# amolchanov86/gym_art

Hardware: AMD Instinct MI355X
Metric: env-steps/sec (whole node) at N=2^20 Hummingbird; achieved HBM GB/s (higher is better)
Workload: dtype f64

## Files before the change

### gym_art_amd/csrc/gaq.hip

```cpp
#include "gaq_host.hpp"

#define GAQ_X(FEAT) extern template __global__ GAQ_STEP_SIG(FEAT)
GAQ_STEP_ALL(GAQ_X)
#undef GAQ_X
#define GAQ_X(FEAT) extern template __global__ GAQ_ROLL_SIG(FEAT)
GAQ_ROLL_ALL(GAQ_X)
#undef GAQ_X

namespace {

using namespace gaqk;

__global__ __launch_bounds__(kBlock) void episode_kernel(int64_t n, const float* __restrict__ reward,
                                                          const uint8_t* __restrict__ done, float* __restrict__ ep_ret,
                                                          uint32_t* __restrict__ ep_len, double* __restrict__ acc) {
  const int64_t i = (int64_t)blockIdx.x * kBlock + threadIdx.x;
  float ret = 0.0f; uint32_t len = 0; bool fin = false;
  if (i < n) {
    ret = ep_ret[i] + reward[i];
    len = ep_len[i] + 1u;
    fin = done[i] != 0;
    ep_ret[i] = fin ? 0.0f : ret;
    ep_len[i] = fin ? 0u : len;
  }
  double c = fin ? 1.0 : 0.0, sr = fin ? (double)ret : 0.0, sl = fin ? (double)len : 0.0, sq = fin ? (double)ret * ret : 0.0;
  if (__ballot(fin)) {
#pragma unroll
    for (int o = 32; o > 0; o >>= 1) { c += __shfl_down(c, o); sr += __shfl_down(sr, o); sl += __shfl_down(sl, o); sq += __shfl_down(sq, o); }
    if ((threadIdx.x & 63) == 0) { atomicAdd(acc + 0, c); atomicAdd(acc + 1, sr); atomicAdd(acc + 2, sl); atomicAdd(acc + 3, sq); }
  }
}

__global__ __launch_bounds__(kBlock) void pack_rows_kernel(int64_t n, int D, const float* __restrict__ obs,
                                                            const float* __restrict__ reward, const uint8_t* __restrict__ done,
                                                            float* __restrict__ rows) {
  const int W = D + 2;
  const int64_t total = n * W;
  for (int64_t k = (int64_t)blockIdx.x * kBlock + threadIdx.x; k < total; k += (int64_t)gridDim.x * kBlock) {
    const int64_t i = k / W;
    const int c = (int)(k - i * W);
    rows[k] = c < D ? obs[i * D + c] : c == D ? reward[i] : (float)done[i];
  }
}

__global__ __launch_bounds__(kBlock) void clear_dynamics_kernel(DevPtrs p, const int64_t* __restrict__ idx, int64_t first, int64_t count) {
  const int64_t k = (int64_t)blockIdx.x * kBlock + threadIdx.x;
  if (k >= count) return;
  const int64_t i = idx ? idx[k] : first + k;
  p.ctr[i] &= 0xFFFFu;
  float* ou = p.ou + (i / kTile) * (4 * kTile) + (i % kTile);
#pragma unroll
  for (int j = 0; j < 4; ++j) ou[j * kTile] = 0.0f;
}

__global__ __launch_bounds__(kBlock) void checksum_kernel(const uint32_t* __restrict__ w, int64_t n, uint64_t* __restrict__ out) {
  uint64_t acc = 0;
  for (int64_t i = (int64_t)blockIdx.x * kBlock + threadIdx.x; i < n; i += (int64_t)gridDim.x * kBlock) {
    uint64_t x = ((uint64_t)w[i] << 32) ^ (uint64_t)i * 0x9E3779B97F4A7C15ull;
    x ^= x >> 29; x *= 0xBF58476D1CE4E5B9ull; x ^= x >> 32;
    acc += x;
  }
#pragma unroll
  for (int o = 32; o > 0; o >>= 1) acc += __shfl_down(acc, o);
  if ((threadIdx.x & 63) == 0) atomicAdd(reinterpret_cast<unsigned long long*>(out), (unsigned long long)acc);
}

__device__ __forceinline__ uint32_t* pfull_of(const DevPtrs& p) { return p.traj + 3 * p.ntiles * kTile; }

__device__ __forceinline__ void write_model_planes(const DevPtrs& p, double dt, int64_t i, const gaq::DerivedModel& dm, bool staged = false) {
  double* tp = staged ? p.par_next + i * (int64_t)kPar
                      : const_cast<double*>(p.par) + (i / kTile) * (int64_t)(kPar * kTile) + (i % kTile);
  const int stride = staged ? 1 : kTile;
  auto P = [&](int plane) -> double& { return tp[plane * stride]; };
  P(PP_MASS) = dm.mass; P(PP_INV_MASS) = 1.0 / dm.mass;
#pragma unroll
  for (int j = 0; j < 3; ++j) { P(PP_INERTIA + j) = dm.inertia[j]; P(PP_INV_INERTIA + j) = 1.0 / dm.inertia[j]; }
#pragma unroll
  for (int j = 0; j < 4; ++j) {
    P(PP_THRUST_MAX + j) = dm.thrust_max[j]; P(PP_TORQUE_MAX + j) = dm.torque_max[j];
    P(PP_PROP_X + j) = dm.prop_pos[3 * j]; P(PP_PROP_Y + j) = dm.prop_pos[3 * j + 1]; P(PP_PROP_Z + j) = dm.prop_pos[3 * j + 2];
  }
  P(PP_TAU_UP) = 4 * dt / (dm.damp_time_up + 1e-6); P(PP_TAU_DOWN) = 4 * dt / (dm.damp_time_down + 1e-6);
  P(PP_T_UP) = dm.damp_time_up; P(PP_T_DOWN) = dm.damp_time_down;
  P(PP_LINEARITY) = dm.linearity; P(PP_ARM) = dm.arm; P(PP_VEL_DAMP) = dm.vel_damp; P(PP_DAMP_Q) = dm.damp_omega_quadratic;
  P(PP_C_DRAG) = dm.c_drag; P(PP_C_ROLL) = dm.c_roll;
  if (staged) P(PP_OU_SIGMA) = (double)(float)dm.ou_sigma;
  else reinterpret_cast<float*>(tp - (i % kTile) + PP_OU_SIGMA * kTile)[i % kTile] = (float)dm.ou_sigma;
  P(PP_T2T) = dm.t2t; P(PP_MX) = dm.motor_x; P(PP_MY) = dm.motor_y; P(PP_COMX) = dm.com[0]; P(PP_COMY) = dm.com[1];
  P(PP_COMPACT_OK) = 1.0;
  if (staged) return;
  pfull_of(p)[i] = p.rcount[i];
  p.ctr[i] &= 0xFFFFu;
  float* ou = p.ou + (i / kTile) * (4 * kTile) + (i % kTile);
#pragma unroll
  for (int j = 0; j < 4; ++j) ou[j * kTile] = 0.0f;
}

__global__ __launch_bounds__(kBlock) void rerandomize_kernel(DevPtrs p, StepCfg cfg, Randomizer rz, const uint8_t* __restrict__ sel,
                                                              int mode, double* __restrict__ trees_out, int64_t first, int64_t count) {
  const int64_t k = (int64_t)blockIdx.x * kBlock + threadIdx.x;
  if (mode == 3) {
    if (k >= count) return;
    const int64_t i = first + k;
    const uint32_t rc = p.rcount[i];
    double* row = trees_out + k * (int64_t)kPar;
    if (rc == pfull_of(p)[i]) { row[PP_COMPACT_OK] = -1.0; return; }
    gaq::ParamTree t;
    if (rz.sampler == 2) gaq::random_quad_tree(cfg.seed, cfg.env_offset + (uint64_t)i, rc - 1, t);
    else gaq::perturb_tree(rz.base, rz.ratio, rz.sampler, cfg.seed, cfg.env_offset + (uint64_t)i, rc - 1, t);
    gaq::DerivedModel dm;
    gaq::derive_tree(t, dm, rz.sampler == 2);
    DevPtrs q = p;
    q.par_next = trees_out - first * (int64_t)kPar;
    write_model_planes(q, cfg.dt, i, dm, true);
    return;
  }
  if (trees_out) {
    if (k >= count) return;
    const int64_t i = first + k;
    gaq::ParamTree t;
    const uint32_t rc = p.rcount[i];
    if (rc == 0) { t = rz.base; }
    else if (rz.sampler == 2) { gaq::random_quad_tree(cfg.seed, cfg.env_offset + (uint64_t)i, rc - 1, t); }
    else { gaq::perturb_tree(rz.base, rz.ratio, rz.sampler, cfg.seed, cfg.env_offset + (uint64_t)i, rc - 1, t); }
    for (int j = 0; j < gaq::TL_COUNT; ++j) trees_out[k * gaq::TL_COUNT + j] = t.v[j];
    return;
  }
  if (mode == 0) {
    const int64_t i = k;
    if (i >= p.n) return;
    const uint32_t promoted = p.rz_flag[i];
    if (!promoted) return;
    if (promoted > 1u) atomicAdd(p.rz_overrun, promoted - 1u);
    gaq::ParamTree t;
    const uint32_t rc = p.rcount[i];
    if (rz.sampler == 2) gaq::random_quad_tree(cfg.seed, cfg.env_offset + (uint64_t)i, rc, t);
    else gaq::perturb_tree(rz.base, rz.ratio, rz.sampler, cfg.seed, cfg.env_offset + (uint64_t)i, rc, t);
    gaq::DerivedModel dm;
    gaq::derive_tree(t, dm, rz.sampler == 2);
    write_model_planes(p, cfg.dt, i, dm, true);
    p.rz_flag[i] = 0;
    return;
  }
  const int64_t i = k;
  if (i >= p.n) return;
  if (mode == 2 || mode == 4) {
    const uint32_t rc = p.rcount[i];
    if (mode == 4 && rc == pfull_of(p)[i]) return;
    gaq::ParamTree t;
    if (rc == 0) { t = rz.base; if (rz.sampler == 2) { pfull_of(p)[i] = 0u; return; } }
    else if (rz.sampler == 2) gaq::random_quad_tree(cfg.seed, cfg.env_offset + (uint64_t)i, rc - 1, t);
    else gaq::perturb_tree(rz.base, rz.ratio, rz.sampler, cfg.seed, cfg.env_offset + (uint64_t)i, rc - 1, t);
    gaq::DerivedModel dm;
    gaq::derive_tree(t, dm, rz.sampler == 2);
    const uint32_t keep = p.ctr[i];
    float ou[4];
    float* op = p.ou + (i / kTile) * (4 * kTile) + (i % kTile);
    for (int j = 0; j < 4; ++j) ou[j] = op[j * kTile];
    write_model_planes(p, cfg.dt, i, dm);
    p.ctr[i] = keep;
    for (int j = 0; j < 4; ++j) op[j * kTile] = ou[j];
    if (p.rz_every > 0) p.rz_flag[i] = 1u;
    return;
  }
  if (!(sel == nullptr || sel[i] != 0)) return;
  const uint32_t rc = p.rcount[i];
  p.rcount[i] = rc + 1u;
  gaq::ParamTree t;
  if (rz.sampler == 2) gaq::random_quad_tree(cfg.seed, cfg.env_offset + (uint64_t)i, rc, t);
  else gaq::perturb_tree(rz.base, rz.ratio, rz.sampler, cfg.seed, cfg.env_offset + (uint64_t)i, rc, t);
  gaq::DerivedModel dm;
  gaq::derive_tree(t, dm, rz.sampler == 2);
  write_model_planes(p, cfg.dt, i, dm);
  if (p.rz_every > 0) p.rz_flag[i] = 1u;
}

__global__ __launch_bounds__(kBlock) void jinv_kernel(DevPtrs p, StepCfg cfg, Model<double> um, const uint8_t* __restrict__ done) {
  const int64_t i = (int64_t)blockIdx.x * kBlock + threadIdx.x;
  if (i >= p.n || !p.jinv) return;
  if (done && !done[i]) return;
  Model<double> m;
  load_model<gaq::F_PER_ENV>(p, cfg, i / kTile, (uint32_t)(i % kTile), um, m);
  double J[4][8];
  const double ccw[4] = {-1, 1, -1, 1};
  for (int c = 0; c < 4; ++c) {
    J[0][c] = m.thrust_max[c] * m.inv_mass;
    J[1][c] = m.inv_inertia[0] * (m.thrust_max[c] * m.prop_y[c]);
    J[2][c] = m.inv_inertia[1] * (m.thrust_max[c] * -m.prop_x[c]);
    J[3][c] = m.inv_inertia[2] * (m.torque_max[c] * ccw[c]);
    for (int r = 0; r < 4; ++r) J[r][4 + c] = (r == c) ? 1.0 : 0.0;
  }
  for (int col = 0; col < 4; ++col) {
    int piv = col;
    for (int r = col + 1; r < 4; ++r) if (fabs(J[r][col]) > fabs(J[piv][col])) piv = r;
    for (int c = 0; c < 8; ++c) { const double t = J[col][c]; J[col][c] = J[piv][c]; J[piv][c] = t; }
    const double inv = 1.0 / J[col][col];
    for (int c = 0; c < 8; ++c) J[col][c] *= inv;
    for (int r = 0; r < 4; ++r) if (r != col) {
      const double f = J[r][col];
      for (int c = 0; c < 8; ++c) J[r][c] -= f * J[col][c];
    }
  }
  double* out = const_cast<double*>(p.jinv) + i * 16;
  for (int r = 0; r < 4; ++r) for (int c = 0; c < 4; ++c) out[4 * r + c] = J[r][4 + c];
}

__global__ __launch_bounds__(kBlock) void derive_trees_kernel(DevPtrs p, StepCfg cfg, const double* __restrict__ trees, int by_density,
                                                               int64_t first, int64_t count) {
  const int64_t k = (int64_t)blockIdx.x * kBlock + threadIdx.x;
  if (k >= count) return;
  gaq::ParamTree t;
  for (int j = 0; j < gaq::TL_COUNT; ++j) t.v[j] = trees[k * gaq::TL_COUNT + j];
  gaq::DerivedModel dm;
  gaq::derive_tree(t, dm, by_density != 0);
  write_model_planes(p, cfg.dt, first + k, dm);
}

__global__ __launch_bounds__(kBlock) void hbm_copy_kernel(const u32x4* __restrict__ src, u32x4* __restrict__ dst, size_t n16) {
  size_t i = (size_t)blockIdx.x * kBlock + threadIdx.x;
  const size_t stride = (size_t)gridDim.x * kBlock;
  for (; i < n16; i += stride) dst[i] = src[i];
}

__global__ void bump_kernel(uint64_t* ctr, uint64_t inc) { *ctr += inc; }
__global__ void fold_counter_kernel(uint64_t* ctr) {
  uint64_t sum = 0;
  for (int k = 0; k < kCtrSlots; ++k) { sum += ctr[k * kCtrStride]; ctr[k * kCtrStride] = 0; }
  ctr[0] = sum;
}

struct TileDirect {
  const DevPtrs& p; int64_t tile; uint32_t lane;
  __device__ __forceinline__ double ld64(const double* arr, int planes, int plane) const {
    auto r = __builtin_amdgcn_make_buffer_rsrc(const_cast<double*>(arr + tile * planes * kTile), 0, planes * kTile * 8, 0x00020000);
    return __builtin_bit_cast(double, __builtin_amdgcn_raw_buffer_load_b64(r, lane * 8u, plane * (kTile * 8), 0));
  }
  __device__ __forceinline__ void st64(double* arr, int planes, int plane, double v) const {
    auto r = __builtin_amdgcn_make_buffer_rsrc(arr + tile * planes * kTile, 0, planes * kTile * 8, 0x00020000);
    __builtin_amdgcn_raw_buffer_store_b64(__builtin_bit_cast(u32x2, v), r, lane * 8u, plane * (kTile * 8), 0);
  }
  __device__ __forceinline__ float ld32(const float* arr, int plane) const {
    auto r = __builtin_amdgcn_make_buffer_rsrc(const_cast<float*>(arr + tile * 4 * kTile), 0, kGrpBytes, 0x00020000);
    return __builtin_bit_cast(float, __builtin_amdgcn_raw_buffer_load_b32(r, lane * 4u, plane * (kTile * 4), 0));
  }
  __device__ __forceinline__ void st32(float* arr, int plane, float v) const {
    auto r = __builtin_amdgcn_make_buffer_rsrc(arr + tile * 4 * kTile, 0, kGrpBytes, 0x00020000);
    __builtin_amdgcn_raw_buffer_store_b32(__builtin_bit_cast(unsigned int, v), r, lane * 4u, plane * (kTile * 4), 0);
  }
};

__global__ __launch_bounds__(kBlock) void reset_kernel(DevPtrs p, StepCfg cfg, Model<double> um, const uint8_t* __restrict__ mask,
                                                        int do_reset, float* obs, int alias, uint64_t key_offset, float* hi_out) {
  extern __shared__ __attribute__((aligned(16))) char smem[];
  const int wave = __builtin_amdgcn_readfirstlane(threadIdx.x >> 6);
  const uint32_t lane = threadIdx.x & 63u;
  if (p.step_ctr) cfg.step_index = step_counter_peek(p, lane);
  cfg.step_index += key_offset;
  const int64_t tile = (int64_t)blockIdx.x * (kBlock / kTile) + wave;
  if (tile >= p.ntiles) return;
  const int D = cfg.obs_dim;
  char* rows = smem + wave * (kTile * D * 4);
  const int64_t i = tile * kTile + lane;
  const TileDirect t{p, tile, lane};
  if (i < p.n) {
    EnvState<double> s;
#pragma unroll
    for (int j = 0; j < 3; ++j) { s.goal[j] = (double)t.ld32(p.goal, j); s.gyro_bias[j] = t.ld32(p.gyro, j); }
    if (alias) {
      double v[18];
#pragma unroll
      for (int k = 0; k < 18; ++k) v[k] = lo_decode(alias, p.obs_in, p.lo, i, k);
#pragma unroll
      for (int j = 0; j < 3; ++j) { s.pos[j] = v[j] + s.goal[j]; s.vel[j] = v[3 + j]; s.omega[j] = v[15 + j]; }
#pragma unroll
      for (int j = 0; j < 9; ++j) s.rot[j] = v[6 + j];
    } else {
#pragma unroll
      for (int j = 0; j < 3; ++j) { s.pos[j] = t.ld64(p.core, kCorePlanes, j); s.vel[j] = t.ld64(p.core, kCorePlanes, 3 + j);
                                    s.omega[j] = t.ld64(p.core, kCorePlanes, 15 + j); }
#pragma unroll
      for (int j = 0; j < 9; ++j) s.rot[j] = t.ld64(p.core, kCorePlanes, 6 + j);
    }
#pragma unroll
    for (int j = 0; j < 4; ++j) { s.rot_damp[j] = t.ld64(p.lag, kLagPlanes, j); s.cmds_damp[j] = t.ld32(p.cmds, j);
                                  s.ou[j] = t.ld32(p.ou, j); s.act_prev[j] = t.ld32(p.actp, j); }
    const uint32_t cw = p.ctr[i];
    s.tick = cw & 0xFFFFu; s.svd_ctr = cw >> 16;
    float acc[3] = {0.0f, 0.0f, 9.81f};
    float hist[4] = {s.act_prev[0], s.act_prev[1], s.act_prev[2], s.act_prev[3]};
    if (do_reset && (mask == nullptr || mask[i])) {
      gaq::reset_env<double, gaq::F_GENERIC>(s, cfg, cfg.env_offset + (uint64_t)i, cfg.step_index);
#pragma unroll
      for (int j = 0; j < 3; ++j) t.st32(p.goal, j, (float)s.goal[j]);
      if (!alias) {
#pragma unroll
        for (int j = 0; j < 3; ++j) { t.st64(p.core, kCorePlanes, j, s.pos[j]); t.st64(p.core, kCorePlanes, 3 + j, s.vel[j]);
                                      t.st64(p.core, kCorePlanes, 15 + j, s.omega[j]); }
#pragma unroll
        for (int j = 0; j < 9; ++j) t.st64(p.core, kCorePlanes, 6 + j, s.rot[j]);
      }
#pragma unroll
      for (int j = 0; j < 4; ++j) { t.st64(p.lag, kLagPlanes, j, s.rot_damp[j]); t.st32(p.cmds, j, s.cmds_damp[j]);
                                    t.st32(p.actp, j, s.act_prev[j]); }
      p.ctr[i] = (s.tick & 0xFFFFu) | (s.svd_ctr << 16);
      hist[0] = hist[1] = hist[2] = hist[3] = 0.0f;
    }
    float hi18[18];
#pragma unroll
    for (int k = 0; k < 18; ++k) hi18[k] = 0.0f;
    if (alias) {
      double v[18];
#pragma unroll
      for (int j = 0; j < 3; ++j) { v[j] = s.pos[j] - s.goal[j]; v[3 + j] = s.vel[j]; v[15 + j] = s.omega[j]; }
#pragma unroll
      for (int j = 0; j < 9; ++j) v[6 + j] = s.rot[j];
#pragma unroll
      for (int k = 0; k < 18; ++k) {
        if (alias == 2) { hi18[k] = (float)v[k]; }
        else { lo_encode(alias, p.lo, i, k, v[k]); hi18[k] = split_hi(v[k]); }
      }
      if (hi_out) {
#pragma unroll
        for (int k = 0; k < 18; ++k) hi_out[i * 18 + k] = hi18[k];
      }
    }
    if (obs) {
      float* row = reinterpret_cast<float*>(rows) + lane * D;
      if (alias && !hi_out) {
#pragma unroll
        for (int k = 0; k < 18; ++k) row[k] = hi18[k];
      } else {
        const float* sz = p.sense_in;
        const int64_t n = p.n;
        double t2w = 0.0, t2t = 0.0;
        if (cfg.obs_flags & (gaq::OBS_APPEND_T2W | gaq::OBS_APPEND_T2T)) {
          double th[4], tq0 = um.torque_max[0], im = um.inv_mass;
#pragma unroll
          for (int j = 0; j < 4; ++j) th[j] = um.thrust_max[j];
          if (p.par) {
#pragma unroll
            for (int j = 0; j < 4; ++j) th[j] = t.ld64(p.par, kPar, PP_THRUST_MAX + j);
            tq0 = t.ld64(p.par, kPar, PP_TORQUE_MAX); im = t.ld64(p.par, kPar, PP_INV_MASS);
          }
          t2w = (((th[0] + th[1]) + th[2]) + th[3]) * im / 9.81; t2t = tq0 / th[0];
        }
        gaq::pack_obs<double, gaq::F_GENERIC | gaq::F_DIAG>(s, cfg, acc, hist, [&](int k, float v, int) { row[k] = v; },
                                            cfg.env_offset + (uint64_t)i, cfg.step_index, 1, WaveSwarm{lane, cfg.swarm.agents},
                                            [&](int c, int slot, int j) { return sz ? sz[((int64_t)(c * 12 + slot) * 3 + j) * n + i] : 0.0f; }, t2w, t2t);
        if (cfg.gyro_bias && (!do_reset || mask == nullptr || mask[i])) {
#pragma unroll
          for (int j = 0; j < 3; ++j) t.st32(p.gyro, j, s.gyro_bias[j]);
        }
      }
    }
  }
  if (obs) {
    wave_lds_fence();
    flush_obs(obs, p.n, D, tile, rows, lane);
  }
}

__global__ __launch_bounds__(kBlock) void export_kernel(DevPtrs p, int alias, double* __restrict__ out, float* __restrict__ aux_out = nullptr) {
  const int64_t i = (int64_t)blockIdx.x * kBlock + threadIdx.x;
  if (i >= p.n) return;
  if (aux_out) {
    for (int k = 0; k < gaq::AUX_WORDS; ++k) aux_out[i * gaq::AUX_WORDS + k] = p.aux[i * gaq::AUX_WORDS + k];
  }
  const int64_t n = p.n;
  const int64_t tile = i / kTile;
  const int lane = (int)(i % kTile);
  auto grp = [&](const float* a, int plane) { return (double)a[tile * (4 * kTile) + plane * kTile + lane]; };
  for (int k = 0; k < 3; ++k) out[(34 + k) * n + i] = grp(p.goal, k);
  if (alias) {
    for (int k = 0; k < 18; ++k)
      out[(int64_t)k * n + i] = lo_decode(alias, p.obs_in, p.lo, i, k) + (k < 3 ? grp(p.goal, k) : 0.0);
  } else {
    for (int k = 0; k < kCorePlanes; ++k) out[(int64_t)k * n + i] = p.core[tile * (kCorePlanes * kTile) + k * kTile + lane];
  }
  for (int j = 0; j < 4; ++j) {
    out[(18 + j) * n + i] = p.lag[tile * (kLagPlanes * kTile) + j * kTile + lane];
    out[(22 + j) * n + i] = grp(p.cmds, j);
    out[(26 + j) * n + i] = grp(p.ou, j);
    out[(30 + j) * n + i] = grp(p.actp, j);
  }
  const uint32_t c = p.ctr[i];
  out[37 * n + i] = (double)(c & 0xFFFFu);
  out[38 * n + i] = (double)(c >> 16);
  for (int k = 0; k < 3; ++k) out[(39 + k) * n + i] = grp(p.gyro, k);
}

thread_local std::string g_err;

int svd_period_of(double dt) {
  double t = 0.0; int k = 0;
  while (!(t > 0.5)) { t += dt; ++k; if (k > 1000000) break; }
  return k;
}

}

int fail(int code, const std::string& msg) { g_err = msg; return code; }
int env_override(const char* name) { const char* v = getenv(name); return v ? (v[0] == '1' ? 1 : 0) : -1; }
LaunchRecord& launch_record() { static LaunchRecord r; return r; }

namespace {

void derive_model(const gaq_model& g, double dt, Model<double>& m) {
  m.mass = g.mass; m.inv_mass = 1.0 / g.mass;
  for (int j = 0; j < 3; ++j) { m.inertia[j] = g.inertia[j]; m.inv_inertia[j] = 1.0 / g.inertia[j]; }
  for (int j = 0; j < 4; ++j) {
    m.thrust_max[j] = g.thrust_max[j]; m.torque_max[j] = g.torque_max[j];
    m.prop_x[j] = g.prop_pos[3 * j]; m.prop_y[j] = g.prop_pos[3 * j + 1]; m.prop_z[j] = g.prop_pos[3 * j + 2];
  }
  m.tau_up = 4 * dt / (g.damp_time_up + 1e-6);
  m.tau_down = 4 * dt / (g.damp_time_down + 1e-6);
  m.linearity = g.linearity; m.arm = g.arm; m.vel_damp = g.vel_damp; m.damp_omega_q = g.damp_omega_quadratic;
  m.c_drag = g.c_drag; m.c_roll = g.c_roll; m.ou_sigma = (float)g.ou_sigma;
  m.jinv = nullptr;
}

bool inverse_jacobian(const gaq_model& g, double out[16]) {
  double J[4][8];
  const double ccw[4] = {-1, 1, -1, 1};
  for (int c = 0; c < 4; ++c) {
    J[0][c] = g.thrust_max[c] / g.mass;
    J[1][c] = (1.0 / g.inertia[0]) * (g.thrust_max[c] * g.prop_pos[3 * c + 1]);
    J[2][c] = (1.0 / g.inertia[1]) * (g.thrust_max[c] * -g.prop_pos[3 * c]);
    J[3][c] = (1.0 / g.inertia[2]) * (g.torque_max[c] * ccw[c]);
    for (int r = 0; r < 4; ++r) J[r][4 + c] = (r == c) ? 1.0 : 0.0;
  }
  for (int col = 0; col < 4; ++col) {
    int piv = col;
    for (int r = col + 1; r < 4; ++r) if (std::fabs(J[r][col]) > std::fabs(J[piv][col])) piv = r;
    if (std::fabs(J[piv][col]) < 1e-300) return false;
    for (int c = 0; c < 8; ++c) std::swap(J[col][c], J[piv][c]);
    const double inv = 1.0 / J[col][col];
    for (int c = 0; c < 8; ++c) J[col][c] *= inv;
    for (int r = 0; r < 4; ++r) if (r != col) {
      const double f = J[r][col];
      for (int c = 0; c < 8; ++c) J[r][c] -= f * J[col][c];
    }
  }
  for (int r = 0; r < 4; ++r) for (int c = 0; c < 4; ++c) out[4 * r + c] = J[r][4 + c];
  return true;
}

int check_model(const gaq_model& g) {
  if (!(g.mass > 0) || !(g.inertia[0] > 0) || !(g.inertia[1] > 0) || !(g.inertia[2] > 0))
    return fail(GAQ_ERR_INVALID, "model: mass and inertia must be positive");
  if (g.damp_time_up < 0 || g.damp_time_down < 0) return fail(GAQ_ERR_INVALID, "model: negative motor time constant");
  return GAQ_OK;
}

bool find_construction(const Model<double>& m, double hint[5]) {
  auto same = [](double a, double b) { return std::memcmp(&a, &b, sizeof(double)) == 0 || (a == 0.0 && b == 0.0); };
  auto around = [](double v, double out[3]) { out[0] = v; out[1] = std::nextafter(v, -INFINITY); out[2] = std::nextafter(v, INFINITY); };
  bool ok = false;
  if (m.thrust_max[0] != 0.0) {
    double cand[3]; around(m.torque_max[0] / m.thrust_max[0], cand);
    for (double t : cand) {
      bool all = true;
      for (int j = 0; j < 4; ++j) all = all && same(t * m.thrust_max[j], m.torque_max[j]);
      if (all) { hint[0] = t; ok = true; break; }
    }
  }
  if (!ok) return false;
  const double sx[4] = {1.0, -1.0, -1.0, 1.0}, sy[4] = {-1.0, -1.0, 1.0, 1.0};
  auto axis = [&](const double p[4], const double sgn[4], double& mo, double& co) {
    double a = 0, b = 0;
    for (int j = 0; j < 4; ++j) (sgn[j] > 0 ? a : b) = p[j];
    double mc[3], cc[3]; around((a - b) * 0.5, mc); around(-(a + b) * 0.5, cc);
    for (double mm : mc) for (double c : cc) {
      bool all = true;
      for (int j = 0; j < 4; ++j) all = all && same(sgn[j] * mm - c, p[j]);
      if (all) { mo = mm; co = c; return true; }
    }
    return false;
  };
  return axis(m.prop_x, sx, hint[1], hint[3]) && axis(m.prop_y, sy, hint[2], hint[4]);
}

struct Layout { bool alias, pack, shadow, fp32; };
struct Selection { uint32_t variant; bool generic; int lds_per_wave; };

bool step_instantiated(uint32_t f) {
  switch (f) {
#define GAQ_X(FEAT) case (FEAT):
    GAQ_STEP_ALL(GAQ_X)
#undef GAQ_X
      return true;
    default: return false;
  }
}
bool roll_instantiated(uint32_t f) {
  switch (f) {
#define GAQ_X(FEAT) case (FEAT):
    GAQ_ROLL_ALL(GAQ_X)
#undef GAQ_X
      return true;
    default: return false;
  }
}

const void* step_kernel_ptr(uint32_t f) {
  switch (f) {
#define GAQ_X(FEAT) case (FEAT): return (const void*)&step_kernel<(FEAT)>;
    GAQ_STEP_ALL(GAQ_X)
#undef GAQ_X
    default: return nullptr;
  }
}
uint32_t rollout_variant_of(uint32_t variant, const Layout& L, bool generic) {
  const uint32_t base = variant & ~(gaq::F_PREDRAW | gaq::F_NT | gaq::F_ROWS | gaq::F_CTR);
  if (!L.alias || L.pack || generic || (variant & gaq::F_MELL)) return 0xFFFFFFFFu;
  if ((base >= 16u && base <= 23u) || (variant >= 48u && variant <= 55u)) return base;
  return 0xFFFFFFFFu;
}

uint32_t rows_twin_of(uint32_t variant) { return step_instantiated(variant | gaq::F_ROWS) ? (variant | gaq::F_ROWS) : 0xFFFFFFFFu; }
uint32_t ctr_twin_of(uint32_t variant) { return step_instantiated(variant | gaq::F_CTR) ? (variant | gaq::F_CTR) : 0xFFFFFFFFu; }

int observation_dim(const gaq_config* cfg) {
  int D = (cfg->obs_flags & GAQ_OBS_QUAT) ? 13 : 18;
  if (cfg->obs_flags & GAQ_OBS_APPEND_T2W) D += 1;
  if (cfg->obs_flags & GAQ_OBS_APPEND_T2T) D += 1;
  if (cfg->obs_flags & GAQ_OBS_APPEND_H) D += 1;
  if (cfg->obs_flags & GAQ_OBS_APPEND_ACC) D += 3;
  if (cfg->obs_flags & GAQ_OBS_APPEND_ACT) D += 4;
  if (cfg->swarm.agents > 1) D += 6 * (cfg->swarm.agents - 1);
  return D;
}

int fill_step_cfg(const gaq_config* cfg, StepCfg& sc, int& obs_dim) {
  if (cfg->struct_size != sizeof(gaq_config) || cfg->abi_version != GAQ_ABI_VERSION)
    return fail(GAQ_ERR_INVALID, "gaq_config size/version mismatch (header vs library)");
  if (cfg->num_envs <= 0) return fail(GAQ_ERR_INVALID, "num_envs must be positive");
  if (cfg->num_envs > (int64_t)1 << 27) return fail(GAQ_ERR_INVALID, "num_envs above 2^27 per handle is not supported");
  if (!(cfg->sim_freq > 0) || cfg->sim_steps <= 0) return fail(GAQ_ERR_INVALID, "sim_freq and sim_steps must be positive");
  if (cfg->sim_steps > 64)
    return fail(GAQ_ERR_INVALID, "sim_steps above 64 is not supported (random-stream ids of the sub-steps)");
  if (cfg->ep_len < 0 || cfg->ep_len >= 0xFFFF) return fail(GAQ_ERR_INVALID, "ep_len must be in [0, 65534]");
  if (cfg->control < 0 || cfg->control > 2) return fail(GAQ_ERR_INVALID, "unknown control mode");
  if (cfg->noise < 0 || cfg->noise > 2) return fail(GAQ_ERR_INVALID, "unknown noise mode");
  if (cfg->reward_mode < 0 || cfg->reward_mode > 1) return fail(GAQ_ERR_INVALID, "unknown reward mode");
  if (cfg->obs_flags & ~127) return fail(GAQ_ERR_INVALID, "unknown obs flags");
  if ((cfg->obs_flags & GAQ_OBS_QUAT) && cfg->swarm.agents > 1) return fail(GAQ_ERR_INVALID, "the quaternion observation is not available for swarms");
  if (cfg->swarm.agents > 1) {
    const int a = cfg->swarm.agents;
    if (a > 16 || (a & (a - 1)) != 0) return fail(GAQ_ERR_INVALID, "swarm.agents must be a power of two <= 16");
    if (cfg->num_envs % a != 0 || cfg->env_id_offset % a != 0)
      return fail(GAQ_ERR_INVALID, "num_envs and env_id_offset must be multiples of swarm.agents (whole worlds per handle)");
    if (!(cfg->swarm.prox_dist > 0.0f) || !(cfg->swarm.collision_dist >= 0.0f) || !(cfg->swarm.goal_radius >= 0.0f))
      return fail(GAQ_ERR_INVALID, "swarm distances must be positive");
  }
  const double dt = 1.0 / cfg->sim_freq;
  const int period = svd_period_of(dt);
  if (period >= 0xFFFF) return fail(GAQ_ERR_INVALID, "sim_freq too high for the 16-bit SVD counter");
  if (cfg->sim_freq < 50.0) return fail(GAQ_ERR_INVALID, "sim_freq below 50 Hz is outside the rotation series' range");
  const int D = observation_dim(cfg);
  obs_dim = D;
  std::memset(&sc, 0, sizeof(sc));
  sc.dt = dt; sc.gravity = cfg->gravity;
  sc.room_lo[0] = -cfg->room_size; sc.room_lo[1] = -cfg->room_size; sc.room_lo[2] = 0.0;
  sc.room_hi[0] = cfg->room_size; sc.room_hi[1] = cfg->room_size; sc.room_hi[2] = cfg->room_size;
  sc.goal_default[0] = 0.0; sc.goal_default[1] = 0.0; sc.goal_default[2] = 2.0;
  sc.init_box = 2.0;
  sc.sim_steps = cfg->sim_steps; sc.ep_len = cfg->ep_len; sc.svd_period = period;
  sc.control = cfg->control; sc.noise = cfg->noise; sc.reward_mode = cfg->reward_mode;
  sc.obs_flags = cfg->obs_flags; sc.obs_dim = D;
  static_assert(sizeof(gaq::RewCoeff) == sizeof(gaq_rew_coeff), "reward coefficient layout");
  std::memcpy(&sc.rew, &cfg->rew, sizeof(sc.rew));
  static_assert(sizeof(gaq::SwarmCfg) == sizeof(gaq_swarm), "swarm layout");
  std::memcpy(&sc.swarm, &cfg->swarm, sizeof(sc.swarm));
  if (sc.swarm.agents <= 1) std::memset(&sc.swarm, 0, sizeof(sc.swarm));
  static_assert(sizeof(gaq::SenseNoise) == sizeof(gaq_sense_noise), "sensor noise layout");
  static_assert(gaq::AUX_WORDS == GAQ_AUX_WORDS, "aux row layout");
  std::memcpy(&sc.sense, &cfg->sense, sizeof(sc.sense));
  if (cfg->sense.enabled && cfg->sense.gyro_norm_std != 0.0f) {
    const double tau = cfg->sense.gyro_bias_correlation_time;
    if (!(tau > 0.0)) return fail(GAQ_ERR_INVALID, "gyro_bias_correlation_time must be positive");
    const double sg = (double)cfg->sense.gyro_noise_density / std::sqrt(dt);
    const double sb = std::sqrt(-(sg * sg) * (tau / 2) * (std::exp(-2 * dt / tau) - 1));
    const double pi = std::exp(-dt / tau);
    sc.gyro_bias = 1;
    sc.gyro_pi = (float)pi; sc.gyro_sigma = (float)sb;
    sc.gyro_pi_step = (float)(pi * pi * pi); sc.gyro_sigma_step = (float)(sb * std::sqrt(1.0 + pi * pi + pi * pi * pi * pi));
  }
  sc.need_act_prev = ((cfg->obs_flags & GAQ_OBS_APPEND_ACT) || cfg->rew.action_change != 0.0f) ? 1 : 0;
  sc.resample_goal = cfg->resample_goal ? 1 : 0;
  sc.excite = cfg->excite ? 1 : 0;
  sc.aux = cfg->aux_outputs ? 1 : 0;
  sc.action_f32 = cfg->action_f32 ? 1 : 0;
  sc.sense_input = (cfg->sense_input && (cfg->sense.enabled || (cfg->obs_flags & (GAQ_OBS_APPEND_T2W | GAQ_OBS_APPEND_T2T)))) ? 1 : 0;
  sc.t2w_std = (float)cfg->t2w_std; sc.t2w_min = 1.5f; sc.t2w_max = 10.0f;
  sc.t2t_std = (float)cfg->t2t_std; sc.t2t_min = 0.005f; sc.t2t_max = 1.0f;
  sc.per_env_goal = (sc.resample_goal || sc.excite || sc.swarm.agents > 1) ? 1 : 0;
  sc.auto_reset = cfg->auto_reset ? 1 : 0;
  sc.init_random_state = cfg->init_random_state ? 1 : 0;
  sc.use_acos = (cfg->rew.rot != 0.0f || cfg->rew.attitude != 0.0f) ? 1 : 0;
  sc.seed = cfg->seed; sc.step_index = 0; sc.env_offset = (uint64_t)cfg->env_id_offset;
  return GAQ_OK;
}

bool envx_wanted(const gaq_config& c, const StepCfg& sc) {
  const bool bias_walk = sc.sense.enabled && sc.gyro_bias;
  return (sc.resample_goal || sc.excite || bias_walk) &&
         !((c.per_env_params || c.control == GAQ_CTRL_MELLINGER) && bias_walk);
}
bool auxp_capable(const gaq_config& c, const StepCfg& sc) {
  const bool obs_diag = (c.obs_flags & (GAQ_OBS_QUAT | GAQ_OBS_APPEND_T2W | GAQ_OBS_APPEND_T2T)) != 0;
  return (sc.aux || obs_diag || envx_wanted(c, sc)) && !(c.control == GAQ_CTRL_MELLINGER && c.per_env_params) && c.obs_state_alias != 0 && !c.fp32_state &&
         sc.swarm.agents <= 1 && env_override("GAQ_NO_AUXP") != 1;
}

void generic_tiers(const gaq_config& c, const StepCfg& sc, bool force_generic, bool& generic, bool& heavy, bool& diag) {
  const bool obs_diag = (c.obs_flags & (GAQ_OBS_QUAT | GAQ_OBS_APPEND_T2W | GAQ_OBS_APPEND_T2T)) != 0;
  const bool bias_walk = sc.sense.enabled && sc.gyro_bias;
  const bool mell_packable = (c.obs_flags & ~(GAQ_OBS_BODY_FRAME | GAQ_OBS_APPEND_H | GAQ_OBS_APPEND_ACC | GAQ_OBS_APPEND_ACT)) == 0 &&
                             c.obs_state_alias != 0;
  const bool mell_heads = c.obs_flags == 0 && !c.sense.enabled && !sc.need_act_prev;
  const bool mell_generic = c.control == GAQ_CTRL_MELLINGER && (c.fp32_state || !(mell_heads || mell_packable || auxp_capable(c, sc)));
  const bool swarm_generic = sc.swarm.agents > 1 &&
                             (c.per_env_params || c.control == GAQ_CTRL_MELLINGER || c.obs_state_alias == 0 || c.fp32_state || c.sense.enabled ||
                              (c.obs_flags & ~(GAQ_OBS_BODY_FRAME | GAQ_OBS_APPEND_H | GAQ_OBS_APPEND_ACC | GAQ_OBS_APPEND_ACT)) != 0);
  const bool auxp = auxp_capable(c, sc);
  const bool envx = auxp && envx_wanted(c, sc);
  generic = force_generic || sc.drag || mell_generic || c.noise == GAQ_NOISE_INPUT || ((sc.resample_goal || sc.excite) && !envx) || (sc.aux && !auxp) ||
            sc.sense_input || (obs_diag && !auxp) || (bias_walk && !envx) || swarm_generic;
  heavy = force_generic || sc.drag || c.control == GAQ_CTRL_MELLINGER || c.noise == GAQ_NOISE_INPUT || sc.sense_input ||
          bias_walk || ((sc.aux || obs_diag) && c.per_env_params);
  diag = sc.aux || obs_diag || (heavy && sc.sense_input);
}

Layout decide_layout(const gaq_config& c, const StepCfg& sc, int D, bool generic) {
  Layout L;
  const bool auxp = auxp_capable(c, sc);
  const bool heads_are_obs = D == 18 && !c.sense.enabled && c.obs_flags == 0 && !sc.need_act_prev && !(auxp && (sc.aux || envx_wanted(c, sc)));
  const bool packable = !c.fp32_state &&
                        (c.obs_flags & ~(GAQ_OBS_BODY_FRAME | GAQ_OBS_APPEND_H | GAQ_OBS_APPEND_ACC | GAQ_OBS_APPEND_ACT |
                                         (auxp ? (GAQ_OBS_QUAT | GAQ_OBS_APPEND_T2W | GAQ_OBS_APPEND_T2T) : 0))) == 0;
  L.alias = (c.obs_state_alias != 0 || c.fp32_state != 0) && (heads_are_obs || packable) && !generic;
  L.pack = L.alias && !heads_are_obs;
  L.fp32 = c.fp32_state != 0;
  L.shadow = L.alias && (c.obs_state_alias == 2 || L.pack) && !c.fp32_state;
  return L;
}

Selection select_kernel(const gaq_config& c, const StepCfg& sc, const Layout& L, int obs_dim, bool force_generic, int rz_every,
                        int num_cus, int predraw_env, int nt_env) {
  Selection out;
  bool generic, heavy, diag;
  generic_tiers(c, sc, force_generic, generic, heavy, diag);
  uint32_t f = c.per_env_params ? gaq::F_PER_ENV : 0u;
  if (generic) {
    f |= gaq::F_GENERIC;
    if (!heavy) f |= gaq::F_LITE;
    if (diag) f |= gaq::F_DIAG;
  } else {
    if (sc.motor_lag) f |= gaq::F_LAG;
    if (c.noise == GAQ_NOISE_PHILOX) f |= gaq::F_NOISE;
    if (c.control == GAQ_CTRL_MELLINGER) f |= gaq::F_MELL;
    if (sc.swarm.agents > 1) f |= gaq::F_SWARM;
  }
  if (L.alias && !generic) f |= gaq::F_ALIAS;
  if (L.pack && L.alias && !generic) f |= gaq::F_PACK;
  if (L.pack && L.alias && !generic && auxp_capable(c, sc)) f |= gaq::F_AUXP;
  if ((f & gaq::F_AUXP) && envx_wanted(c, sc)) f |= gaq::F_ENVX | ((sc.sense.enabled && sc.gyro_bias) ? gaq::F_BIAS : 0u);
  if (L.fp32 && L.alias && !generic) f |= gaq::F_FP32;
  if (c.per_env_params && rz_every > 0) f |= gaq::F_RZ;
  if (f == 20u || f == 22u || f == 23u) {
    const int64_t tiles = (c.num_envs + kTile - 1) / kTile;
    const int64_t simds = (int64_t)(num_cus > 0 ? num_cus : 256) * 4;
    bool nt = tiles <= 2 * simds, predraw = tiles > simds;
    if (predraw_env >= 0) predraw = predraw_env != 0;
    if (nt_env >= 0) nt = nt_env != 0;
    if (predraw && sc.sim_steps <= 2) f |= gaq::F_PREDRAW;
    if (nt) f |= gaq::F_NT;
  }
  out.variant = f;
  out.generic = generic;
  const int obs_rows = kTile * obs_dim * 4;
  int lpw;
  if (generic) {
    const int img = tile_image<gaq::F_GENERIC>(sc).total;
    lpw = img > obs_rows ? img : obs_rows;
    if (f & gaq::F_DIAG) {
      const int both = ((obs_rows + 15) & ~15) + kTile * gaq::AUX_WORDS * 4;
      lpw = lpw > both ? lpw : both;
    }
  } else {
    int img = (L.fp32 ? kRowsLds : L.alias ? kRowsLds + kLoRowsLds : kCoreBytes) +
              (sc.motor_lag ? kLagBytes + kGrpBytes : 0) +
              (c.noise == GAQ_NOISE_PHILOX ? kGrpBytes : 0) +
              ((sc.need_act_prev && (!L.alias || L.pack)) ? kGrpBytes : 0) +
              (sc.swarm.agents > 1 ? kGrpBytes : 0) +
              ((f & gaq::F_ENVX) && sc.per_env_goal ? kGrpBytes : 0) +
              ((f & gaq::F_BIAS) && sc.gyro_bias ? kGrpBytes : 0);
    lpw = img > obs_rows ? img : obs_rows;
    if (f & gaq::F_AUXP) {
      const int both = ((obs_rows + 15) & ~15) + kTile * gaq::AUX_WORDS * 4;
      lpw = lpw > both ? lpw : both;
    }
  }
  out.lds_per_wave = (lpw + 15) & ~15;
  return out;
}

void counter_plan(int64_t ntiles, uint64_t& waves, uint32_t& shift, uint32_t& inc0) {
  const int wpb = kBlock / kTile;
  waves = (uint64_t)((ntiles + wpb - 1) / wpb) * wpb;
  shift = 0;
  while (((uint64_t)1 << shift) < waves) ++shift;
  inc0 = (uint32_t)(((uint64_t)1 << shift) - (waves - 1));
}

void refresh_feature_flags(gaq_env* e) {
  StepCfg& sc = e->sc;
  sc.motor_lag = e->any_lag ? 1 : 0;
  sc.drag = e->any_drag ? 1 : 0;
  const Layout L{e->alias, e->pack, e->shadow, e->fp32};
  const Selection sel = select_kernel(e->cfg, sc, L, e->obs_dim, e->force_generic, e->d.rz_every, e->num_cus,
                                      env_override("GAQ_PREDRAW"), env_override("GAQ_NT"));
  e->variant = (int)sel.variant;
  e->needs_generic = sel.generic;
  e->lds_per_wave = sel.lds_per_wave;
}

int alias_mode(const gaq_env* e) { return e->fp32 ? 2 : !e->alias ? 0 : e->lomix ? 3 : 1; }

int record_alias_rows(gaq_env* e, hipStream_t st) {
  if (!e->check_alias || e->shadow) return GAQ_OK;
  HIP_TRY(hipMemsetAsync(e->alias_sum_dev, 0, sizeof(uint64_t), st));
  const int64_t words = e->d.n * 18;
  hipLaunchKernelGGL(checksum_kernel, dim3(1024), dim3(kBlock), 0, st, reinterpret_cast<const uint32_t*>(e->last_obs), words, e->alias_sum_dev);
  HIP_TRY(hipGetLastError());
  HIP_TRY(hipMemcpyAsync(&e->alias_sum, e->alias_sum_dev, sizeof(uint64_t), hipMemcpyDeviceToHost, st));
  HIP_TRY(hipStreamSynchronize(st));
  e->alias_sum_valid = true;
  return GAQ_OK;
}
int verify_alias_rows(gaq_env* e, hipStream_t st) {
  if (!e->check_alias || e->shadow || !e->alias_sum_valid) return GAQ_OK;
  uint64_t now = 0;
  HIP_TRY(hipMemsetAsync(e->alias_sum_dev, 0, sizeof(uint64_t), st));
  const int64_t words = e->d.n * 18;
  hipLaunchKernelGGL(checksum_kernel, dim3(1024), dim3(kBlock), 0, st, reinterpret_cast<const uint32_t*>(e->last_obs), words, e->alias_sum_dev);
  HIP_TRY(hipGetLastError());
  HIP_TRY(hipMemcpyAsync(&now, e->alias_sum_dev, sizeof(uint64_t), hipMemcpyDeviceToHost, st));
  HIP_TRY(hipStreamSynchronize(st));
  if (now != e->alias_sum)
    return fail(GAQ_ERR_STATE, "obs_state_alias: the observation tensor returned by the previous step / reset was modified before "
                               "this call -- it is the integrator state's fp32 head (include/gaq.h gaq_config.obs_state_alias); "
                               "copy it before editing, or create the handle with obs_state_alias = 2 (library-owned heads)");
  return GAQ_OK;
}

int launch_refill(gaq_env* e, hipStream_t st) {
  const dim3 grid((unsigned)((e->d.n + kBlock - 1) / kBlock)), block(kBlock);
  hipLaunchKernelGGL(rerandomize_kernel, grid, block, 0, st, e->d, e->sc, e->rz, (const uint8_t*)nullptr, 0, (double*)nullptr,
                     (int64_t)0, (int64_t)0);
  HIP_TRY(hipGetLastError());
  e->rz_since_refill = 0; e->rz_refill_now = false;
  return GAQ_OK;
}

int launch_jinv(gaq_env* e, hipStream_t st, const uint8_t* done) {
  if (!e->d.jinv || !e->dev_params) return GAQ_OK;
  const dim3 grid((unsigned)((e->d.n + kBlock - 1) / kBlock)), block(kBlock);
  hipLaunchKernelGGL(jinv_kernel, grid, block, 0, st, e->d, e->sc, e->um, done);
  HIP_TRY(hipGetLastError());
  return GAQ_OK;
}

uint32_t launch_variant_of(const gaq_env* e) {
  const uint32_t v = (uint32_t)e->variant;
  if (e->d.rows_out && rows_twin_of(v) != 0xFFFFFFFFu) return rows_twin_of(v);
  if (e->d.step_ctr && ctr_twin_of(v) != 0xFFFFFFFFu) return ctr_twin_of(v);
  return v;
}

}

int launch_step(gaq_env* e, const float* actions, float* obs, float* reward, uint8_t* done, hipStream_t st) {
  e->info_valid = false;
  if ((reinterpret_cast<uintptr_t>(actions) & 15) != 0) return fail(GAQ_ERR_INVALID, "actions must be 16-byte aligned");
  if ((reinterpret_cast<uintptr_t>(obs) & 15) != 0) return fail(GAQ_ERR_INVALID, "obs must be 16-byte aligned");
  if (e->sc.noise == gaq::NOISE_INPUT) {
    if (!e->noise_next) return fail(GAQ_ERR_STATE, "GAQ_NOISE_INPUT: call gaq_set_noise_input_dev before each step");
    e->d.noise_in = e->noise_next;
    e->noise_next = nullptr;
  }
  if (e->sc.sense_input) {
    if (!e->sense_next) return fail(GAQ_ERR_STATE, "sense_input: call gaq_set_sense_input_dev before each step");
    e->d.sense_in = e->sense_next;
    e->sense_next = nullptr;
  }
  const int tiles_per_block = kBlock / kTile;
  const dim3 grid((unsigned)((e->d.ntiles + tiles_per_block - 1) / tiles_per_block)), block(kBlock);
  const size_t lds = (size_t)e->lds_per_wave * tiles_per_block;
  const int lpw = e->lds_per_wave;
  const float* caller_obs = obs;
  if (e->alias) {
    if (e->needs_generic) return fail(GAQ_ERR_STATE, "obs_state_alias: parameters now need the generic kernel (rotor drag); "
                                                     "create the handle without obs_state_alias");
    e->d.obs_in = e->last_obs;
    if (int rc = verify_alias_rows(e, st)) return rc;
    e->d.obs_copy = nullptr;
    if (e->shadow) {
      if (obs != e->own_obs) e->d.obs_copy = obs;
      obs = e->own_obs;
    }
  }
  if (lds > 65536 && e->lds_raised_for != e->variant) {
    const void* fn = step_kernel_ptr((uint32_t)e->variant);
    if (!fn || lds > 160 * 1024) return fail(GAQ_ERR_INVALID, "observation rows too large for the CU's LDS");
    HIP_TRY(hipFuncSetAttribute(fn, hipFuncAttributeMaxDynamicSharedMemorySize, (int)lds));
    e->lds_raised_for = e->variant;
  }
  const uint32_t launch_variant = launch_variant_of(e);
  if (e->d.rz_every > 0 && (launch_variant & gaq::F_RZ) != 0) {
    const bool hot_only = e->sc.compact_params != 0 && e->sc.zero_damp != 0 && (launch_variant & gaq::F_FP32) == 0;
    if (hot_only) e->cold_stale = true;
    else if (e->cold_stale) {
      const dim3 g1((unsigned)((e->d.n + kBlock - 1) / kBlock));
      hipLaunchKernelGGL(rerandomize_kernel, g1, block, 0, st, e->d, e->sc, e->rz, (const uint8_t*)nullptr, 4, (double*)nullptr, (int64_t)0, (int64_t)0);
      HIP_TRY(hipGetLastError());
      e->rz_refill_now = true;
      e->cold_stale = false;
    }
  }
  if (e->d.rz_every > 0 && e->rz_refill_now) { if (int rc = launch_refill(e, st)) return rc; }
  const bool self_counting = (launch_variant & gaq::F_CTR) != 0;
  if (e->d.step_ctr && !self_counting) {
    bool capturing = false;
    hipStreamCaptureStatus cs = hipStreamCaptureStatusNone;
    if (hipStreamIsCapturing(st, &cs) == hipSuccess) capturing = cs == hipStreamCaptureStatusActive; else (void)hipGetLastError();
    if (e->ctr_spread || capturing) {
      hipLaunchKernelGGL(fold_counter_kernel, dim3(1), dim3(1), 0, st, e->d.step_ctr);
      HIP_TRY(hipGetLastError());
      if (!capturing) e->ctr_spread = false;
    }
  }
  if (launch_variant != e->noted_step) { launch_record().note(0, launch_variant); e->noted_step = launch_variant; }
#define GAQ_LAUNCH(FEAT) \
  hipLaunchKernelGGL(step_kernel<(FEAT)>, grid, block, lds, st, e->d, e->sc, e->um, actions, obs, reward, done, lpw)
  switch (launch_variant) {
// ... 91 lines not shown
  HIP_TRY(hipGetLastError());
  if (caller_obs) e->cur_obs = caller_obs;
  if (e->alias) {
    e->last_obs = e->pack ? e->own_obs : obs;
    if (e->shadow && !e->pack && caller_obs != obs)
      HIP_TRY(hipMemcpyAsync(caller_obs, obs, sizeof(float) * (size_t)e->d.n * 18, hipMemcpyDeviceToDevice, st));
    if (int rc = record_alias_rows(e, st)) return rc;
  }
  return GAQ_OK;
}

int read_step_counter(gaq_env* e, uint64_t* step) {
  std::vector<uint64_t> w((size_t)kCtrSlots * kCtrStride);
  HIP_TRY(hipMemcpy(w.data(), e->step_ctr_mem, w.size() * sizeof(uint64_t), hipMemcpyDeviceToHost));
  uint64_t sum = 0;
  for (int k = 0; k < kCtrSlots; ++k) sum += w[k * kCtrStride];
  *step = sum >> e->d.ctr_shift;
  return GAQ_OK;
}
int write_step_counter(gaq_env* e, uint64_t step) {
  std::vector<uint64_t> w((size_t)kCtrSlots * kCtrStride, 0);
  w[0] = step << e->d.ctr_shift;
  HIP_TRY(hipMemcpy(e->step_ctr_mem, w.data(), w.size() * sizeof(uint64_t), hipMemcpyHostToDevice));
  e->ctr_spread = false;
  return GAQ_OK;
}

}

int sync_handle(gaq_env* e) {
  HIP_TRY(hipStreamSynchronize(e->stream));
  if (e->user_stream_used) HIP_TRY(hipStreamSynchronize(e->user_stream));
  return GAQ_OK;
}

int check_overrun(gaq_env* e) {
  if (!e->d.rz_overrun) return GAQ_OK;
  uint32_t o = 0;
  HIP_TRY(hipMemcpy(&o, e->d.rz_overrun, sizeof(uint32_t), hipMemcpyDeviceToHost));
  if (o) return fail(GAQ_ERR_STATE, "internal: an env was re-randomised before its staged parameter planes were refilled");
  return GAQ_OK;
}

namespace {

struct Scratch {
  void* p = nullptr;
  ~Scratch() { if (p) (void)hipFree(p); }
  int alloc(size_t bytes) {
    hipError_t e = hipMalloc(&p, bytes ? bytes : 16);
    return e == hipSuccess ? 0 : fail(GAQ_ERR_DEVICE, std::string("hipMalloc: ") + hipGetErrorString(e));
  }
};

inline size_t tidx(int64_t i, int planes, int plane) {
  return (size_t)(i / kTile) * planes * kTile + (size_t)plane * kTile + (size_t)(i % kTile);
}

}

extern "C" {

int gaq_abi_version(void) { return GAQ_ABI_VERSION; }
const char* gaq_last_error(void) { return g_err.c_str(); }

int gaq_num_devices(void) {
  int n = 0;
  if (hipGetDeviceCount(&n) != hipSuccess) return 0;
  return n;
}

int gaq_create(const gaq_config* cfg, gaq_env** out) {
  if (!cfg || !out) return fail(GAQ_ERR_INVALID, "null argument");
  StepCfg sc0;
  int D = 18;
  if (int rc = fill_step_cfg(cfg, sc0, D)) return rc;
  if (!cfg->per_env_params && check_model(cfg->model) != GAQ_OK) return GAQ_ERR_INVALID;
  int ndev = gaq_num_devices();
  if (ndev <= 0) return fail(GAQ_ERR_DEVICE, "no HIP device visible: libgaq has no CPU fallback");
  if (cfg->device < 0 || cfg->device >= ndev) return fail(GAQ_ERR_INVALID, "device ordinal out of range");
  HIP_TRY(hipSetDevice(cfg->device));
  hipDeviceProp_t prop;
  HIP_TRY(hipGetDeviceProperties(&prop, cfg->device));

  gaq_env* e = new (std::nothrow) gaq_env();
  if (!e) return fail(GAQ_ERR_DEVICE, "out of host memory");
  e->cfg = *cfg;
  e->obs_dim = D;
  e->num_cus = prop.multiProcessorCount > 0 ? prop.multiProcessorCount : 256;
  StepCfg& sc = e->sc;
  sc = sc0;
  const double dt = sc.dt;

  if (!cfg->per_env_params) {
    derive_model(cfg->model, dt, e->um);
    e->um.jinv = nullptr;
    e->any_lag = !(e->um.tau_up >= 1.0 && e->um.tau_down >= 1.0);
    e->any_drag = (cfg->model.c_drag != 0.0 || cfg->model.c_roll != 0.0);
    if (cfg->control == GAQ_CTRL_MELLINGER && !inverse_jacobian(cfg->model, sc.jinv)) {
      delete e;
      return fail(GAQ_ERR_INVALID, "singular quadrotor jacobian");
    }
  } else {
    std::memset(&e->um, 0, sizeof(e->um));
    e->any_lag = true;
    e->any_drag = false;
  }
  { const char* nf = getenv("GAQ_NO_FUSED"); if (nf && nf[0] == '1') e->fused_rollout = false; }
  { const char* fg = getenv("GAQ_FORCE_GENERIC"); if (fg && fg[0] == '1') e->force_generic = true; }
  e->lomix = cfg->per_env_params != 0 || e->any_lag;
  {
    sc.motor_lag = e->any_lag ? 1 : 0; sc.drag = e->any_drag ? 1 : 0;
    bool generic, heavy, diag;
    generic_tiers(*cfg, sc, e->force_generic, generic, heavy, diag);
    const Layout L = decide_layout(*cfg, sc, D, generic);
    e->alias = L.alias; e->pack = L.pack; e->fp32 = L.fp32; e->shadow = L.shadow;
  }
  { const char* ca = getenv("GAQ_CHECK_ALIAS"); e->check_alias = ca && ca[0] == '1'; }
  {
    const char* ab = getenv("GAQ_ABLATE");
    sc.ablate = ab ? atoi(ab) : 0;
    if (sc.ablate != 0 && !kDiagBuild) {
      delete e;
      return fail(GAQ_ERR_INVALID, "GAQ_ABLATE is set but this libgaq is not a measurement build (make EXTRA=-DGAQ_DIAG_BUILD OUT=...): "
                                   "the ablations skip parts of the step and give wrong physics; unset the variable");
    }
    if (sc.ablate != 0) fprintf(stderr, "libgaq: GAQ_ABLATE=%d in a measurement build -- results are WRONG by construction, only timings mean anything\n", sc.ablate);
  }
  refresh_feature_flags(e);
  if (e->fp32 && !e->alias) {
    delete e;
    return fail(GAQ_ERR_INVALID, "fp32_state needs the specialised kernels (18-word world-frame obs, RawControl, default reward terms)");
  }
  if (!step_instantiated((uint32_t)e->variant)) {
    delete e;
    return fail(GAQ_ERR_STATE, "internal: no kernel instantiation for this feature mask");
  }

  DevPtrs& d = e->d;
  std::memset(&d, 0, sizeof(d));
  d.n = cfg->num_envs;
  d.ntiles = (cfg->num_envs + kTile - 1) / kTile;
  {
    uint64_t waves;
    counter_plan(d.ntiles, waves, d.ctr_shift, d.ctr_inc0);
  }
  const size_t nt = (size_t)d.ntiles;
  hipError_t he = hipSuccess;
  auto alloc0 = [&](void** p, size_t bytes) {
    if (he != hipSuccess) return;
    he = hipMalloc(p, bytes);
    if (he == hipSuccess) he = hipMemset(*p, 0, bytes);
  };
  if (e->alias) {
    if (!e->fp32) alloc0((void**)&d.lo, nt * (e->lomix ? (size_t)kMixRowsBytes : (size_t)kLoRowsBytes));
    alloc0((void**)&e->own_obs, nt * kRowsBytes);
  } else {
    alloc0((void**)&d.core, nt * kCoreBytes);
  }
  alloc0((void**)&d.lag, nt * kLagBytes);
  alloc0((void**)&d.ou, nt * kGrpBytes);
  alloc0((void**)&d.cmds, nt * kGrpBytes);
  alloc0((void**)&d.actp, nt * kGrpBytes);
  alloc0((void**)&d.goal, nt * kGrpBytes);
  alloc0((void**)&d.gyro, nt * kGrpBytes);
  alloc0((void**)&e->step_ctr_mem, sizeof(uint64_t) * kCtrSlots * kCtrStride);
  alloc0((void**)&e->alias_sum_dev, sizeof(uint64_t));
  alloc0((void**)&d.ctr, nt * kTile * sizeof(uint32_t));
  alloc0((void**)&d.done_count, sizeof(uint32_t) * 2);
  alloc0((void**)&d.nan_count, sizeof(uint32_t));
  if (cfg->compact_done) alloc0((void**)&d.done_list, nt * kTile * sizeof(uint32_t));
  if (cfg->aux_outputs) alloc0((void**)&d.aux, nt * kTile * gaq::AUX_WORDS * sizeof(float));
  if (cfg->per_env_params) {
    double* par = nullptr;
    double* jinv_dev = nullptr;
    alloc0((void**)&par, nt * kParBytes);
    if (cfg->control == GAQ_CTRL_MELLINGER) alloc0((void**)&jinv_dev, nt * kTile * 16 * sizeof(double));
    d.par = par;
    d.jinv = jinv_dev;
    alloc0((void**)&d.traj, 4 * nt * kTile * sizeof(uint32_t));
    d.rcount = d.traj ? d.traj + nt * kTile : nullptr;
    d.rz_flag = d.traj ? d.traj + 2 * nt * kTile : nullptr;
    e->host_par.assign(nt * kPar * kTile, 1.0);
    for (size_t t = 0; t < nt; ++t)
      for (int pl : {(int)PP_VEL_DAMP, (int)PP_DAMP_Q, (int)PP_C_DRAG, (int)PP_C_ROLL, (int)PP_COMX, (int)PP_COMY, (int)PP_OU_SIGMA})
        std::fill_n(e->host_par.begin() + (t * kPar + pl) * kTile, kTile, 0.0);
    e->pflags.assign((size_t)cfg->num_envs, 0);
  }
  if (he == hipSuccess) he = hipStreamCreateWithFlags(&e->stream, hipStreamNonBlocking);
  if (he == hipSuccess) he = hipEventCreate(&e->ev0);
  if (he == hipSuccess) he = hipEventCreate(&e->ev1);
  if (he != hipSuccess) {
    std::string msg = std::string("device allocation failed: ") + hipGetErrorString(he);
    gaq_destroy(e);
    return fail(GAQ_ERR_DEVICE, msg);
  }
  auto init_state = [&]() -> int {
    std::vector<float> goal(nt * 4 * kTile, 0.0f);
    for (int64_t i = 0; i < d.ntiles * kTile; ++i) {
      goal[tidx(i, 4, 2)] = 2.0f;
      if (sc.swarm.agents > 1) {
        const float ang = 6.2831853071795864769f * (float)(((uint64_t)cfg->env_id_offset + (uint64_t)i) % (uint64_t)sc.swarm.agents) /
                          (float)sc.swarm.agents;
        goal[tidx(i, 4, 0)] = sc.swarm.goal_radius * cosf(ang);
        goal[tidx(i, 4, 1)] = sc.swarm.goal_radius * sinf(ang);
      }
    }
    HIP_TRY(hipMemcpy(d.goal, goal.data(), goal.size() * sizeof(float), hipMemcpyHostToDevice));
    if (e->alias) {
      std::vector<float> rows(nt * kTile * 18, 0.0f);
      for (int64_t i = 0; i < d.ntiles * kTile; ++i) {
        rows[i * 18 + 0] = -goal[tidx(i, 4, 0)]; rows[i * 18 + 1] = -goal[tidx(i, 4, 1)];
        rows[i * 18 + 2] = -2.0f;
        for (int j : {6, 10, 14}) rows[i * 18 + j] = 1.0f;
      }
      HIP_TRY(hipMemcpy(e->own_obs, rows.data(), rows.size() * sizeof(float), hipMemcpyHostToDevice));
      e->last_obs = e->own_obs;
    } else {
      std::vector<double> core(nt * kCorePlanes * kTile, 0.0);
      for (int64_t i = 0; i < d.ntiles * kTile; ++i)
        for (int j : {6, 10, 14}) core[tidx(i, kCorePlanes, j)] = 1.0;
      HIP_TRY(hipMemcpy(d.core, core.data(), core.size() * sizeof(double), hipMemcpyHostToDevice));
    }
    if (cfg->per_env_params)
      HIP_TRY(hipMemcpy(const_cast<double*>(d.par), e->host_par.data(), e->host_par.size() * sizeof(double), hipMemcpyHostToDevice));
    return GAQ_OK;
  };
  if (int rc = init_state()) { gaq_destroy(e); return rc; }
  *out = e;
  return GAQ_OK;
}

int gaq_destroy(gaq_env* e) {
  if (!e) return GAQ_OK;
  (void)hipSetDevice(e->cfg.device);
  if (e->stream) (void)hipStreamSynchronize(e->stream);
  (void)hipDeviceSynchronize();
  (void)hipFree(e->d.core); (void)hipFree(e->d.lo); (void)hipFree(e->own_obs); (void)hipFree(e->d.lag); (void)hipFree(e->d.ou); (void)hipFree(e->d.cmds);
  (void)hipFree(e->d.actp); (void)hipFree(e->d.goal); (void)hipFree(e->d.gyro); (void)hipFree(e->step_ctr_mem); if (e->info_pin) (void)hipHostFree(e->info_pin); (void)hipFree(e->alias_sum_dev); (void)hipFree(e->d.ctr);
  (void)hipFree(e->d.done_count); (void)hipFree(e->d.nan_count); (void)hipFree(e->d.done_list);
  (void)hipFree(e->d.ep_ret); (void)hipFree(e->d.ep_len); (void)hipFree(e->d.ep_acc); (void)hipFree(e->d.aux);
  (void)hipFree(const_cast<double*>(e->d.par)); (void)hipFree(const_cast<double*>(e->d.jinv));
  (void)hipFree(e->d.traj); (void)hipFree(e->d.rz_overrun);
  (void)hipFree(e->stage_dev); (void)hipFree(e->export_dev);
  if (e->stage_pin) (void)hipHostFree(e->stage_pin);
  if (e->ev0) (void)hipEventDestroy(e->ev0);
  if (e->ev1) (void)hipEventDestroy(e->ev1);
  if (e->stream) (void)hipStreamDestroy(e->stream);
  delete e;
  return GAQ_OK;
}

int gaq_is_diag_build(void) { return kDiagBuild ? 1 : 0; }

int gaq_plan(const gaq_config* cfg, int32_t motor_lag, int32_t rotor_drag, int32_t randomize_every, int32_t num_cus, gaq_plan_info* out) {
  if (!cfg || !out) return fail(GAQ_ERR_INVALID, "null argument");
  StepCfg sc;
  int D = 18;
  if (int rc = fill_step_cfg(cfg, sc, D)) return rc;
  bool lag = motor_lag > 0, drag = rotor_drag > 0;
  if (!cfg->per_env_params) {
    if (check_model(cfg->model) != GAQ_OK) return GAQ_ERR_INVALID;
    Model<double> um;
    derive_model(cfg->model, sc.dt, um);
    if (motor_lag < 0) lag = !(um.tau_up >= 1.0 && um.tau_down >= 1.0);
    if (rotor_drag < 0) drag = (cfg->model.c_drag != 0.0 || cfg->model.c_roll != 0.0);
  } else {
    if (motor_lag < 0) lag = true;
    if (rotor_drag < 0) drag = false;
  }
  sc.motor_lag = lag ? 1 : 0; sc.drag = drag ? 1 : 0;
  const bool force_generic = env_override("GAQ_FORCE_GENERIC") == 1;
  bool generic, heavy, diag;
  generic_tiers(*cfg, sc, force_generic, generic, heavy, diag);
  StepCfg sc_create = sc;
  if (cfg->per_env_params) { sc_create.drag = 0; }
  bool g0, h0, d0;
  generic_tiers(*cfg, sc_create, force_generic, g0, h0, d0);
  const Layout L = decide_layout(*cfg, sc_create, D, g0);
  const int rz = (cfg->per_env_params && randomize_every > 0) ? randomize_every : 0;
  const Selection sel = select_kernel(*cfg, sc, L, D, force_generic, rz, num_cus, env_override("GAQ_PREDRAW"), env_override("GAQ_NT"));
  out->obs_dim = D;
  out->state_layout = !L.alias ? 0 : L.shadow ? 2 : 1;
  out->fp32 = (L.fp32 && L.alias) ? 1 : 0;
  out->step_variant = (int32_t)sel.variant;
  out->step_instantiated = step_instantiated(sel.variant) ? 1 : 0;
  out->launchable = (out->step_instantiated && !(L.alias && sel.generic) && !(L.fp32 && !L.alias)) ? 1 : 0;
  const uint32_t rv = (rz > 0) ? 0xFFFFFFFFu : rollout_variant_of(sel.variant, L, sel.generic);
  out->rollout_variant = rv == 0xFFFFFFFFu ? -1 : (int32_t)rv;
  out->rollout_instantiated = rv == 0xFFFFFFFFu ? 0 : (roll_instantiated(rv) ? 1 : 0);
  out->lds_per_wave = sel.lds_per_wave;
  const uint32_t rt = rows_twin_of(sel.variant), ct = ctr_twin_of(sel.variant);
  out->rows_variant = rt == 0xFFFFFFFFu ? -1 : (int32_t)rt;
  out->ctr_variant = ct == 0xFFFFFFFFu ? -1 : (int32_t)ct;
  {
    uint64_t waves; uint32_t sh, inc0;
    counter_plan((cfg->num_envs + kTile - 1) / kTile, waves, sh, inc0);
    out->ctr_waves = (int32_t)waves; out->ctr_shift = (int32_t)sh; out->ctr_inc0 = (int32_t)inc0;
  }
  return GAQ_OK;
}

int gaq_kernel_variant(const gaq_env* e) { return e ? e->variant : GAQ_ERR_INVALID; }
int gaq_launch_variant(const gaq_env* e) { return e ? (int)launch_variant_of(e) : GAQ_ERR_INVALID; }
int gaq_launched_variants(int kind, uint32_t* out, int capacity) {
  if (kind < 0 || kind > 2 || capacity < 0 || (capacity > 0 && !out)) return GAQ_ERR_INVALID;
  LaunchRecord& r = launch_record();
  std::lock_guard<std::mutex> g(r.mu);
  int k = 0;
  for (uint32_t f : r.seen[kind]) { if (k < capacity) out[k] = f; ++k; }
  return k;
}
int gaq_obs_dim(const gaq_env* e) { return e ? e->obs_dim : GAQ_ERR_INVALID; }
int gaq_obs_is_state(const gaq_env* e) { return (e && e->alias && !e->shadow) ? 1 : 0; }
int gaq_state_layout(const gaq_env* e) { return !e ? GAQ_ERR_INVALID : !e->alias ? 0 : e->shadow ? 2 : 1; }
int64_t gaq_num_envs(const gaq_env* e) { return e ? e->d.n : GAQ_ERR_INVALID; }

static void set_env_flags(gaq_env* e, int64_t i, uint8_t nf) {
  const uint8_t of = e->pflags[(size_t)i];
  e->cnt_lag += (nf & 1) - (of & 1); e->cnt_drag += ((nf >> 1) & 1) - ((of >> 1) & 1);
  e->cnt_noncompact += ((nf >> 2) & 1) - ((of >> 2) & 1); e->cnt_damp += ((nf >> 3) & 1) - ((of >> 3) & 1);
  e->pflags[(size_t)i] = nf;
}
static void flags_from_counts(gaq_env* e) {
  e->any_lag = e->cnt_lag > 0; e->any_drag = e->cnt_drag > 0;
  e->sc.compact_params = (e->cnt_noncompact == 0 && !getenv("GAQ_NO_COMPACT")) ? 1 : 0;
  e->sc.zero_damp = (e->cnt_damp == 0 && !getenv("GAQ_NO_COMPACT")) ? 1 : 0;
  refresh_feature_flags(e);
}
static uint8_t tree_flags(const gaq_quad_params& t, double dt) {
  const double tu = 4 * dt / (t.motor[9] + 1e-6), td = 4 * dt / (t.motor[10] + 1e-6);
  return (uint8_t)((!(tu >= 1.0 && td >= 1.0) ? 1 : 0) | ((t.motor[7] != 0.0 || t.motor[8] != 0.0) ? 2 : 0) |
                   ((t.damp[0] != 0.0 || t.damp[1] != 0.0) ? 8 : 0));
}

static int set_params_impl(gaq_env* e, const gaq_model* models, const int64_t* idx, int64_t first, int64_t count) {
  if (!e || !models) return fail(GAQ_ERR_INVALID, "null argument");
  e->info_valid = false;
  if (!e->cfg.per_env_params) return fail(GAQ_ERR_STATE, "handle was created with per_env_params = 0");
  if (e->dev_params) return fail(GAQ_ERR_STATE, "this handle's parameters are managed on the device (gaq_set_randomizer / "
                                                "gaq_set_param_trees): gaq_set_params is not available");
  if (count < 0) return fail(GAQ_ERR_INVALID, "negative count");
  if (count == 0) return GAQ_OK;
  auto env_of = [&](int64_t k) { return idx ? idx[k] : first + k; };
  int64_t lo = e->d.n, hi = -1;
  for (int64_t k = 0; k < count; ++k) {
    const int64_t i = env_of(k);
    if (i < 0 || i >= e->d.n) return fail(GAQ_ERR_INVALID, "env index out of bounds");
    lo = i < lo ? i : lo; hi = i > hi ? i : hi;
  }
  HIP_TRY(hipSetDevice(e->cfg.device));
  double* hp = e->host_par.data();
  std::vector<double> ji(e->d.jinv ? (size_t)count * 16 : 0);
  for (int64_t k = 0; k < count; ++k) {
    if (check_model(models[k]) != GAQ_OK) return GAQ_ERR_INVALID;
    if (e->d.jinv && !inverse_jacobian(models[k], ji.data() + (size_t)k * 16)) return fail(GAQ_ERR_INVALID, "singular quadrotor jacobian");
  }
  for (int64_t k = 0; k < count; ++k) {
    Model<double> m;
    derive_model(models[k], e->sc.dt, m);
    const int64_t i = env_of(k);
    auto P = [&](int plane) -> double& { return hp[tidx(i, kPar, plane)]; };
    P(PP_MASS) = m.mass; P(PP_INV_MASS) = m.inv_mass;
    for (int j = 0; j < 3; ++j) { P(PP_INERTIA + j) = m.inertia[j]; P(PP_INV_INERTIA + j) = m.inv_inertia[j]; }
    for (int j = 0; j < 4; ++j) {
      P(PP_THRUST_MAX + j) = m.thrust_max[j]; P(PP_TORQUE_MAX + j) = m.torque_max[j];
      P(PP_PROP_X + j) = m.prop_x[j]; P(PP_PROP_Y + j) = m.prop_y[j]; P(PP_PROP_Z + j) = m.prop_z[j];
    }
    P(PP_TAU_UP) = m.tau_up; P(PP_TAU_DOWN) = m.tau_down; P(PP_LINEARITY) = m.linearity;
    P(PP_T_UP) = models[k].damp_time_up; P(PP_T_DOWN) = models[k].damp_time_down;
    P(PP_ARM) = m.arm; P(PP_VEL_DAMP) = m.vel_damp; P(PP_DAMP_Q) = m.damp_omega_q;
    P(PP_C_DRAG) = m.c_drag; P(PP_C_ROLL) = m.c_roll;
    reinterpret_cast<float*>(hp + tidx(i - i % kTile, kPar, PP_OU_SIGMA))[i % kTile] = (float)models[k].ou_sigma;
    double hint[5] = {0, 0, 0, 0, 0};
    const bool compact_ok = find_construction(m, hint);
    P(PP_COMPACT_OK) = compact_ok ? 1.0 : 0.0;
    for (int j = 0; j < 5; ++j) P(PP_T2T + j) = hint[j];
    set_env_flags(e, i, (uint8_t)((!(m.tau_up >= 1.0 && m.tau_down >= 1.0) ? 1 : 0) | ((m.c_drag != 0.0 || m.c_roll != 0.0) ? 2 : 0) |
                                  (!compact_ok ? 4 : 0) | ((m.vel_damp != 0.0 || m.damp_omega_q != 0.0) ? 8 : 0)));
  }
  HIP_TRY(hipStreamSynchronize(e->stream));
  if (int rc_ = sync_handle(e)) return rc_;
  if (e->d.jinv) {
    if (!idx) {
      HIP_TRY(hipMemcpy(const_cast<double*>(e->d.jinv) + (size_t)first * 16, ji.data(), ji.size() * sizeof(double), hipMemcpyHostToDevice));
    } else {
      for (int64_t k = 0; k < count; ++k)
        HIP_TRY(hipMemcpy(const_cast<double*>(e->d.jinv) + (size_t)idx[k] * 16, ji.data() + (size_t)k * 16, 16 * sizeof(double), hipMemcpyHostToDevice));
    }
  }
  {
    std::vector<int64_t> tiles((size_t)count);
// ... 314 lines not shown
  }
  char* dv = e->stage_dev;
  char* pin = e->stage_pin;
  if (pin && e->stage_map) {
    char* mp = e->stage_map;
    const bool heads_in_obs = e->alias && !e->pack && !e->shadow;
    float* obs_arg = heads_in_obs ? e->own_obs : reinterpret_cast<float*>(mp + e->off_obs);
    std::memcpy(pin, actions, 16 * n);
    int rc = gaq_step_dev(e, reinterpret_cast<const float*>(mp), obs_arg, reinterpret_cast<float*>(mp + e->off_rew),
                          reinterpret_cast<uint8_t*>(mp + e->off_done), e->stream);
    if (rc) return rc;
    if (heads_in_obs) HIP_TRY(hipMemcpyAsync(pin + e->off_obs, e->own_obs, 4 * D * n, hipMemcpyDeviceToHost, e->stream));
    if (e->d.aux) {
      const size_t sbytes = sizeof(double) * GAQ_STATE_PLANES * n, abytes = sizeof(float) * gaq::AUX_WORDS * n;
      if (!e->info_pin) {
        HIP_TRY(hipHostMalloc((void**)&e->info_pin, sbytes + abytes, hipHostMallocMapped));
        void* dp = nullptr;
        if (hipHostGetDevicePointer(&dp, e->info_pin, 0) == hipSuccess && dp) e->info_map = static_cast<char*>(dp);
        else (void)hipGetLastError();
      }
      if (e->alias) e->d.obs_in = e->last_obs;
      const dim3 grid((unsigned)((n + kBlock - 1) / kBlock)), block(kBlock);
      if (e->info_map) {
        hipLaunchKernelGGL(export_kernel, grid, block, 0, e->stream, e->d, alias_mode(e), reinterpret_cast<double*>(e->info_map),
                           reinterpret_cast<float*>(e->info_map + sbytes));
        HIP_TRY(hipGetLastError());
      } else {
        if (!e->export_dev) HIP_TRY(hipMalloc((void**)&e->export_dev, sbytes));
        hipLaunchKernelGGL(export_kernel, grid, block, 0, e->stream, e->d, alias_mode(e), e->export_dev, (float*)nullptr);
        HIP_TRY(hipGetLastError());
        HIP_TRY(hipMemcpyAsync(e->info_pin, e->export_dev, sbytes, hipMemcpyDeviceToHost, e->stream));
        HIP_TRY(hipMemcpyAsync(e->info_pin + sbytes, e->d.aux, abytes, hipMemcpyDeviceToHost, e->stream));
      }
    }
    HIP_TRY(hipStreamSynchronize(e->stream));
    e->info_valid = e->d.aux != nullptr;
    std::memcpy(reward, pin + e->off_rew, 4 * n);
    std::memcpy(done, pin + e->off_done, n);
    std::memcpy(obs, pin + e->off_obs, 4 * D * n);
    if (int rc_ = check_overrun(e)) return rc_;
    for (size_t i = 0; i < n; ++i) {
      if (!std::isfinite(reward[i])) {
        HIP_TRY(hipMemset(e->d.nan_count, 0, sizeof(uint32_t)));
        return fail(GAQ_ERR_NAN, "QuadEnv: reward is Nan");
      }
    }
    return GAQ_OK;
  }
  float* dev_obs = (e->alias && !e->pack) ? e->own_obs : reinterpret_cast<float*>(dv + e->off_obs);
  if (pin) std::memcpy(pin, actions, 16 * n);
  HIP_TRY(hipMemcpyAsync(dv, pin ? (const void*)pin : (const void*)actions, 16 * n, hipMemcpyHostToDevice, e->stream));
  int rc = gaq_step_dev(e, reinterpret_cast<const float*>(dv), dev_obs, reinterpret_cast<float*>(dv + e->off_rew),
                        reinterpret_cast<uint8_t*>(dv + e->off_done), e->stream);
  if (rc) return rc;
  if (pin) {
    if (e->alias && !e->pack) {
      HIP_TRY(hipMemcpyAsync(pin + e->off_rew, dv + e->off_rew, e->off_obs - e->off_rew, hipMemcpyDeviceToHost, e->stream));
      HIP_TRY(hipMemcpyAsync(pin + e->off_obs, dev_obs, 4 * D * n, hipMemcpyDeviceToHost, e->stream));
    } else {
      HIP_TRY(hipMemcpyAsync(pin + e->off_rew, dv + e->off_rew, e->stage_bytes - e->off_rew, hipMemcpyDeviceToHost, e->stream));
    }
    if (e->d.aux) {
      const size_t sbytes = sizeof(double) * GAQ_STATE_PLANES * n, abytes = sizeof(float) * gaq::AUX_WORDS * n;
      if (!e->info_pin) HIP_TRY(hipHostMalloc((void**)&e->info_pin, sbytes + abytes, hipHostMallocDefault));
      if (!e->export_dev) HIP_TRY(hipMalloc((void**)&e->export_dev, sbytes));
      if (e->alias) e->d.obs_in = e->last_obs;
      const dim3 grid((unsigned)((n + kBlock - 1) / kBlock)), block(kBlock);
      hipLaunchKernelGGL(export_kernel, grid, block, 0, e->stream, e->d, alias_mode(e), e->export_dev, (float*)nullptr);
      HIP_TRY(hipGetLastError());
      HIP_TRY(hipMemcpyAsync(e->info_pin, e->export_dev, sbytes, hipMemcpyDeviceToHost, e->stream));
      HIP_TRY(hipMemcpyAsync(e->info_pin + sbytes, e->d.aux, abytes, hipMemcpyDeviceToHost, e->stream));
    }
    HIP_TRY(hipStreamSynchronize(e->stream));
    e->info_valid = e->d.aux != nullptr;
    std::memcpy(reward, pin + e->off_rew, 4 * n);
    std::memcpy(done, pin + e->off_done, n);
    std::memcpy(obs, pin + e->off_obs, 4 * D * n);
  } else {
    HIP_TRY(hipMemcpyAsync(obs, dev_obs, 4 * D * n, hipMemcpyDeviceToHost, e->stream));
    HIP_TRY(hipMemcpyAsync(reward, dv + e->off_rew, 4 * n, hipMemcpyDeviceToHost, e->stream));
    HIP_TRY(hipMemcpyAsync(done, dv + e->off_done, n, hipMemcpyDeviceToHost, e->stream));
    HIP_TRY(hipStreamSynchronize(e->stream));
  }
  if (int rc_ = check_overrun(e)) return rc_;
  for (size_t i = 0; i < n; ++i) {
    if (!std::isfinite(reward[i])) {
      HIP_TRY(hipMemset(e->d.nan_count, 0, sizeof(uint32_t)));
      return fail(GAQ_ERR_NAN, "QuadEnv: reward is Nan");
    }
  }
  return GAQ_OK;
}

int gaq_set_noise_input_dev(gaq_env* e, const float* normals_dev) {
  if (!e || !normals_dev) return fail(GAQ_ERR_INVALID, "null argument");
  if (e->sc.noise != gaq::NOISE_INPUT) return fail(GAQ_ERR_STATE, "handle was not created with GAQ_NOISE_INPUT");
  e->noise_next = normals_dev;
  return GAQ_OK;
}

int gaq_set_sense_input_dev(gaq_env* e, const float* draws_dev) {
  if (!e || !draws_dev) return fail(GAQ_ERR_INVALID, "null argument");
  if (!e->sc.sense_input) return fail(GAQ_ERR_STATE, "handle was not created with sense_input (and sensor noise or a t2w / t2t observation)");
  e->sense_next = draws_dev;
  return GAQ_OK;
}

int gaq_set_action_dtype(gaq_env* e, int32_t is_float32) {
  if (!e) return fail(GAQ_ERR_INVALID, "null handle");
  e->sc.action_f32 = is_float32 ? 1 : 0;
  return GAQ_OK;
}

int gaq_get_aux(gaq_env* e, float* host_out) {
  if (!e || !host_out) return fail(GAQ_ERR_INVALID, "null argument");
  if (!e->d.aux) return fail(GAQ_ERR_STATE, "handle was created with aux_outputs = 0");
  if (e->info_valid) {
    std::memcpy(host_out, e->info_pin + sizeof(double) * GAQ_STATE_PLANES * (size_t)e->d.n, sizeof(float) * (size_t)e->d.n * gaq::AUX_WORDS);
    return GAQ_OK;
  }
  HIP_TRY(hipSetDevice(e->cfg.device));
  if (int rc_ = sync_handle(e)) return rc_;
  HIP_TRY(hipMemcpy(host_out, e->d.aux, sizeof(float) * (size_t)e->d.n * gaq::AUX_WORDS, hipMemcpyDeviceToHost));
  return GAQ_OK;
}

int gaq_get_state(gaq_env* e, double* hp) {
  if (!e || !hp) return fail(GAQ_ERR_INVALID, "null argument");
  if (e->info_valid) { std::memcpy(hp, e->info_pin, sizeof(double) * GAQ_STATE_PLANES * (size_t)e->d.n); return GAQ_OK; }
  HIP_TRY(hipSetDevice(e->cfg.device));
  if (int rc_ = sync_handle(e)) return rc_;
  const size_t n = (size_t)e->d.n;
  const size_t bytes = sizeof(double) * GAQ_STATE_PLANES * n;
  if (!e->export_dev) HIP_TRY(hipMalloc((void**)&e->export_dev, bytes));
  if (e->alias) e->d.obs_in = e->last_obs;
  const dim3 grid((unsigned)((n + kBlock - 1) / kBlock)), block(kBlock);
  hipLaunchKernelGGL(export_kernel, grid, block, 0, e->stream, e->d, alias_mode(e), e->export_dev, (float*)nullptr);
  HIP_TRY(hipGetLastError());
  HIP_TRY(hipMemcpyAsync(hp, e->export_dev, bytes, hipMemcpyDeviceToHost, e->stream));
  HIP_TRY(hipStreamSynchronize(e->stream));
  return GAQ_OK;
}

int gaq_set_state(gaq_env* e, const double* hp) {
  if (!e || !hp) return fail(GAQ_ERR_INVALID, "null argument");
  e->info_valid = false;
  e->cur_obs = nullptr;
  HIP_TRY(hipSetDevice(e->cfg.device));
  HIP_TRY(hipStreamSynchronize(e->stream));
  if (int rc_ = sync_handle(e)) return rc_;
  const int64_t n = e->d.n;
  const size_t nt = (size_t)e->d.ntiles;
  std::vector<double> core(nt * kCorePlanes * kTile, 0.0), lag(nt * kLagPlanes * kTile, 0.0);
  std::vector<float> ou(nt * 4 * kTile, 0.f), cmds(nt * 4 * kTile, 0.f), actp(nt * 4 * kTile, 0.f), goal(nt * 4 * kTile, 0.f),
      gyro(nt * 4 * kTile, 0.f);
  std::vector<uint32_t> c(nt * kTile, 0u);
  for (int64_t i = n; i < (int64_t)(nt * kTile); ++i) { for (int j : {6, 10, 14}) core[tidx(i, kCorePlanes, j)] = 1.0; }
  for (int64_t i = 0; i < n; ++i) {
    for (int pl = 0; pl < kCorePlanes; ++pl) core[tidx(i, kCorePlanes, pl)] = hp[(size_t)pl * n + i];
    for (int j = 0; j < 4; ++j) {
      lag[tidx(i, kLagPlanes, j)] = hp[(size_t)(18 + j) * n + i];
      cmds[tidx(i, 4, j)] = (float)hp[(size_t)(22 + j) * n + i];
      ou[tidx(i, 4, j)] = (float)hp[(size_t)(26 + j) * n + i];
      actp[tidx(i, 4, j)] = (float)hp[(size_t)(30 + j) * n + i];
    }
    for (int j = 0; j < 3; ++j) goal[tidx(i, 4, j)] = (float)hp[(size_t)(34 + j) * n + i];
    for (int j = 0; j < 3; ++j) gyro[tidx(i, 4, j)] = (float)hp[(size_t)(39 + j) * n + i];
    const double t = hp[(size_t)37 * n + i], s = hp[(size_t)38 * n + i];
    if (!(t >= 0 && t <= 65535 && s >= 0 && s <= 65535)) return fail(GAQ_ERR_INVALID, "tick / SVD counter out of range");
    c[i] = ((uint32_t)t & 0xFFFFu) | ((uint32_t)s << 16);
  }
  if (e->alias) {
    std::vector<float> hi(nt * kTile * 18, 0.0f);
    const int mode = alias_mode(e);
    std::vector<unsigned char> lo(nt * (size_t)(e->lomix ? kMixRowsBytes : kLoRowsBytes), 0);
    for (int64_t i = 0; i < n; ++i)
      for (int k = 0; k < 18; ++k) {
        const double v = core[tidx(i, kCorePlanes, k)] - (k < 3 ? (double)goal[tidx(i, 4, k)] : 0.0);
        hi[i * 18 + k] = e->fp32 ? (float)v : split_hi(v);
        lo_encode(mode, lo.data(), i, k, v);
      }
    HIP_TRY(hipMemcpy(e->own_obs, hi.data(), hi.size() * 4, hipMemcpyHostToDevice));
    if (!e->fp32) HIP_TRY(hipMemcpy(e->d.lo, lo.data(), lo.size(), hipMemcpyHostToDevice));
    e->last_obs = e->own_obs;
  } else {
    HIP_TRY(hipMemcpy(e->d.core, core.data(), core.size() * 8, hipMemcpyHostToDevice));
  }
  HIP_TRY(hipMemcpy(e->d.lag, lag.data(), lag.size() * 8, hipMemcpyHostToDevice));
  HIP_TRY(hipMemcpy(e->d.ou, ou.data(), ou.size() * 4, hipMemcpyHostToDevice));
  HIP_TRY(hipMemcpy(e->d.cmds, cmds.data(), cmds.size() * 4, hipMemcpyHostToDevice));
  HIP_TRY(hipMemcpy(e->d.actp, actp.data(), actp.size() * 4, hipMemcpyHostToDevice));
  HIP_TRY(hipMemcpy(e->d.goal, goal.data(), goal.size() * 4, hipMemcpyHostToDevice));
  HIP_TRY(hipMemcpy(e->d.gyro, gyro.data(), gyro.size() * 4, hipMemcpyHostToDevice));
  HIP_TRY(hipMemcpy(e->d.ctr, c.data(), c.size() * 4, hipMemcpyHostToDevice));
  e->rz_refill_now = true;
  return GAQ_OK;
}

int gaq_done_list(gaq_env* e, uint32_t* idx_out, int64_t capacity, int64_t* count_out) {
  if (!e || !count_out) return fail(GAQ_ERR_INVALID, "null argument");
  if (!e->d.done_list) return fail(GAQ_ERR_STATE, "handle was created with compact_done = 0");
  HIP_TRY(hipSetDevice(e->cfg.device));
  HIP_TRY(hipStreamSynchronize(e->stream));
  if (int rc_ = sync_handle(e)) return rc_;
  uint64_t step = e->sc.step_index;
  if (e->d.step_ctr) { if (int rc_ = read_step_counter(e, &step)) return rc_; }
  if (step == 0) { *count_out = 0; return GAQ_OK; }
  uint32_t cnt = 0;
  HIP_TRY(hipMemcpy(&cnt, e->d.done_count + ((step - 1) & 1), sizeof(uint32_t), hipMemcpyDeviceToHost));
  *count_out = cnt;
  if (idx_out && cnt) {
    const int64_t m = cnt < capacity ? cnt : capacity;
    HIP_TRY(hipMemcpy(idx_out, e->d.done_list, sizeof(uint32_t) * m, hipMemcpyDeviceToHost));
  }
  return GAQ_OK;
}

int gaq_pack_rows_dev(gaq_env* e, const float* obs, const float* reward, const uint8_t* done, float* rows, void* stream) {
  if (!e || !obs || !reward || !done || !rows) return fail(GAQ_ERR_INVALID, "null argument");
  HIP_TRY(hipSetDevice(e->cfg.device));
  e->user_stream = (hipStream_t)stream; e->user_stream_used = true;
  const int64_t total = e->d.n * (e->obs_dim + 2);
  int64_t blocks = (total + kBlock - 1) / kBlock;
  if (blocks > 16384) blocks = 16384;
  hipLaunchKernelGGL(pack_rows_kernel, dim3((unsigned)blocks), dim3(kBlock), 0, (hipStream_t)stream, e->d.n, e->obs_dim, obs, reward,
                     done, rows);
  HIP_TRY(hipGetLastError());
  return GAQ_OK;
}

int gaq_set_packed_rows_dev(gaq_env* e, float* rows_dev) {
  if (!e) return fail(GAQ_ERR_INVALID, "null handle");
  if (rows_dev && (reinterpret_cast<uintptr_t>(rows_dev) & 15) != 0) return fail(GAQ_ERR_INVALID, "rows must be 16-byte aligned");
  e->d.rows_out = rows_dev;
  return GAQ_OK;
}

int gaq_nan_count(gaq_env* e, int64_t* count_out) {
  if (!e || !count_out) return fail(GAQ_ERR_INVALID, "null argument");
  HIP_TRY(hipSetDevice(e->cfg.device));
  HIP_TRY(hipStreamSynchronize(e->stream));
  if (int rc_ = sync_handle(e)) return rc_;
  uint32_t c = 0;
  HIP_TRY(hipMemcpy(&c, e->d.nan_count, sizeof(uint32_t), hipMemcpyDeviceToHost));
  HIP_TRY(hipMemset(e->d.nan_count, 0, sizeof(uint32_t)));
  *count_out = c;
  return check_overrun(e);
}

int gaq_set_terminal_obs_dev(gaq_env* e, float* term_obs_dev) {
  if (!e) return fail(GAQ_ERR_INVALID, "null handle");
  e->d.term_obs = term_obs_dev;
  return GAQ_OK;
}

int gaq_track_episodes(gaq_env* e, int32_t enabled) {
  if (!e) return fail(GAQ_ERR_INVALID, "null handle");
  HIP_TRY(hipSetDevice(e->cfg.device));
  if (int rc_ = sync_handle(e)) return rc_;
  if (enabled && !e->d.ep_ret) {
    const size_t np = (size_t)e->d.ntiles * kTile;
    HIP_TRY(hipMalloc((void**)&e->d.ep_ret, np * sizeof(float)));
    HIP_TRY(hipMalloc((void**)&e->d.ep_len, np * sizeof(uint32_t)));
    HIP_TRY(hipMalloc((void**)&e->d.ep_acc, 4 * sizeof(double)));
    HIP_TRY(hipMemset(e->d.ep_ret, 0, np * sizeof(float)));
    HIP_TRY(hipMemset(e->d.ep_len, 0, np * sizeof(uint32_t)));
    HIP_TRY(hipMemset(e->d.ep_acc, 0, 4 * sizeof(double)));
  } else if (!enabled && e->d.ep_ret) {
    (void)hipFree(e->d.ep_ret); (void)hipFree(e->d.ep_len); (void)hipFree(e->d.ep_acc);
    e->d.ep_ret = nullptr; e->d.ep_len = nullptr; e->d.ep_acc = nullptr;
  }
  return GAQ_OK;
}

int gaq_episode_stats(gaq_env* e, int64_t* episodes, double* return_sum, double* length_sum, double* return_sqsum, int32_t clear) {
  if (!e || !episodes || !return_sum || !length_sum || !return_sqsum) return fail(GAQ_ERR_INVALID, "null argument");
  if (!e->d.ep_acc) return fail(GAQ_ERR_STATE, "episode tracking is off (gaq_track_episodes)");
  HIP_TRY(hipSetDevice(e->cfg.device));
  if (int rc_ = sync_handle(e)) return rc_;
  double a[4];
  HIP_TRY(hipMemcpy(a, e->d.ep_acc, sizeof(a), hipMemcpyDeviceToHost));
  if (clear) HIP_TRY(hipMemset(e->d.ep_acc, 0, sizeof(a)));
  *episodes = (int64_t)(a[0] + 0.5); *return_sum = a[1]; *length_sum = a[2]; *return_sqsum = a[3];
  return GAQ_OK;
}

int gaq_get_counters(gaq_env* e, gaq_counters* out, uint32_t* episodes_out, uint32_t* resamples_out) {
  if (!e || !out) return fail(GAQ_ERR_INVALID, "null argument");
  HIP_TRY(hipSetDevice(e->cfg.device));
  if (int rc_ = sync_handle(e)) return rc_;
  if (int rc_ = check_overrun(e)) return rc_;
  out->step_index = e->sc.step_index;
  if (e->d.step_ctr) { if (int rc_ = read_step_counter(e, &out->step_index)) return rc_; }
  out->reset_calls = e->reset_calls;
  if ((episodes_out || resamples_out) && !e->d.traj) return fail(GAQ_ERR_STATE, "handle was created with per_env_params = 0: no per-env counts");
  const size_t bytes = sizeof(uint32_t) * (size_t)e->d.n;
  if (episodes_out) HIP_TRY(hipMemcpy(episodes_out, e->d.traj, bytes, hipMemcpyDeviceToHost));
  if (resamples_out) HIP_TRY(hipMemcpy(resamples_out, e->d.rcount, bytes, hipMemcpyDeviceToHost));
  return GAQ_OK;
}

int gaq_set_counters(gaq_env* e, const gaq_counters* in, const uint32_t* episodes, const uint32_t* resamples) {
  if (!e || !in) return fail(GAQ_ERR_INVALID, "null argument");
  if ((episodes || resamples) && !e->d.traj) return fail(GAQ_ERR_STATE, "handle was created with per_env_params = 0: no per-env counts");
  HIP_TRY(hipSetDevice(e->cfg.device));
  if (int rc_ = sync_handle(e)) return rc_;
  e->info_valid = false;
  e->sc.step_index = in->step_index;
  e->reset_calls = in->reset_calls;
  if (e->d.step_ctr) { if (int rc_ = write_step_counter(e, in->step_index)) return rc_; }
  HIP_TRY(hipMemset(e->d.done_count, 0, sizeof(uint32_t) * 2));
  const size_t bytes = sizeof(uint32_t) * (size_t)e->d.n;
  if (episodes) HIP_TRY(hipMemcpy(e->d.traj, episodes, bytes, hipMemcpyHostToDevice));
  if (resamples) {
    HIP_TRY(hipMemcpy(e->d.rcount, resamples, bytes, hipMemcpyHostToDevice));
    if (e->rz_on) {
      const dim3 grid((unsigned)((e->d.n + kBlock - 1) / kBlock)), block(kBlock);
      hipLaunchKernelGGL(rerandomize_kernel, grid, block, 0, e->stream, e->d, e->sc, e->rz, (const uint8_t*)nullptr, 2, (double*)nullptr,
                         (int64_t)0, (int64_t)0);
      HIP_TRY(hipGetLastError());
      if (int rc = launch_jinv(e, e->stream, nullptr)) return rc;
      if (e->d.rz_every > 0) { if (int rc = launch_refill(e, e->stream)) return rc; }
      HIP_TRY(hipStreamSynchronize(e->stream));
      e->cold_stale = false;
    }
  }
  e->rz_refill_now = true;
  return GAQ_OK;
}

int gaq_set_graph_safe(gaq_env* e, int32_t enabled) {
  if (!e) return fail(GAQ_ERR_INVALID, "null handle");
  HIP_TRY(hipSetDevice(e->cfg.device));
  if (int rc_ = sync_handle(e)) return rc_;
  if (enabled && !e->d.step_ctr) {
    if (int rc_ = write_step_counter(e, e->sc.step_index)) return rc_;
    e->d.step_ctr = e->step_ctr_mem;
  } else if (!enabled && e->d.step_ctr) {
    uint64_t v = 0;
    if (int rc_ = read_step_counter(e, &v)) return rc_;
    e->sc.step_index = v;
    e->d.step_ctr = nullptr;
  }
  return GAQ_OK;
}

int gaq_set_timing(gaq_env* e, int32_t enabled) {
// ... 38 lines not shown
```

### gym_art_amd/csrc/gaq_kernels.hpp

```cpp
#pragma once

#include <hip/hip_runtime.h>

#include <cstddef>
#include <cstdint>

#include "../../include/gaq.h"
#include "quad_core.hpp"
#include "quad_params_dev.hpp"

namespace gaqk {

#ifndef GAQ_LD_AUX
#define GAQ_LD_AUX 0
#endif
#ifndef GAQ_ST_AUX
#define GAQ_ST_AUX 0
#endif
#ifndef GAQ_ACT_AUX
#define GAQ_ACT_AUX 0
#endif
template <uint32_t F> constexpr int kLdAux = (F & gaq::F_NT) ? 2 : GAQ_LD_AUX;
template <uint32_t F> constexpr int kStAux = (F & gaq::F_NT) ? 2 : GAQ_ST_AUX;
#ifndef GAQ_COPY_AUX
#define GAQ_COPY_AUX 2
#endif
template <uint32_t F> constexpr int kCopyAux = (F & gaq::F_NT) ? 2 : GAQ_COPY_AUX;
#ifdef GAQ_DIAG_BUILD
constexpr bool kDiagBuild = true;
#else
constexpr bool kDiagBuild = false;
#endif
__host__ __device__ __forceinline__ bool ablated(const gaq::StepCfg& cfg, int bit) { return kDiagBuild && (cfg.ablate & bit) != 0; }
constexpr int kBlock = 256;
constexpr int kTile = 64;
constexpr int kCorePlanes = 18;
constexpr int kLagPlanes = 4;
constexpr int kCoreBytes = kCorePlanes * kTile * 8;
constexpr int kLagBytes = kLagPlanes * kTile * 8;
constexpr int kGrpBytes = 4 * kTile * 4;
constexpr int kRowBytes = 18 * 4;
constexpr int kRowsBytes = kTile * kRowBytes;
constexpr int kRowsLds = 5 * 1024;
constexpr int kLoRowBytes = 18 * 2;
constexpr int kLoRowsBytes = kTile * kLoRowBytes;
constexpr int kLoRowsLds = 3 * 1024;
constexpr int kMixRowWords = 11;
constexpr int kMixRowBytes = kMixRowWords * 4;
constexpr int kMixRowsBytes = kTile * kMixRowBytes;
template <uint32_t F> constexpr bool kLoMix = (F & (gaq::F_PER_ENV | gaq::F_LAG)) != 0;
constexpr int kPar = 45;
constexpr int kParBytes = kPar * kTile * 8;
constexpr int kHotPlanes = 19;
constexpr int kParNextSkew = 544;
enum ParPlane { PP_MASS = 0, PP_INV_MASS = 1, PP_INERTIA = 2, PP_INV_INERTIA = 5, PP_THRUST_MAX = 8, PP_TORQUE_MAX = 12,
                PP_PROP_X = 16, PP_PROP_Y = 20, PP_PROP_Z = 24, PP_TAU_UP = 28, PP_TAU_DOWN = 29, PP_LINEARITY = 30,
                PP_ARM = 31, PP_VEL_DAMP = 32, PP_DAMP_Q = 33, PP_C_DRAG = 34, PP_C_ROLL = 35, PP_OU_SIGMA = 36,
                PP_T2T = 37, PP_MX = 38, PP_MY = 39, PP_COMX = 40, PP_COMY = 41, PP_COMPACT_OK = 42,
                PP_T_UP = 43, PP_T_DOWN = 44 };

struct DevPtrs {
  double* core;
  void* lo;
  const float* obs_in;
  float* obs_copy;
  float* hi_final;
  double* lag;
  float* ou;
  float* cmds;
  float* actp;
  float* goal;
  float* gyro;
  uint32_t* ctr;
  const double* par;
  const double* jinv;
  const float* noise_in;
  const float* sense_in;
  float* aux;
  uint32_t* done_list;
  uint32_t* done_count;
  uint32_t* nan_count;
  float* term_obs;
  float* ep_ret;
  uint32_t* ep_len;
  double* ep_acc;
  uint64_t* step_ctr;
  uint32_t ctr_shift;
  uint32_t ctr_inc0;
  float* rows_out;
  uint32_t* rcount;
  uint32_t* traj;
  double* par_next;
  uint32_t* rz_flag;
  uint32_t* rz_overrun;
  int32_t rz_every;
  int64_t n, ntiles;
};

using gaq::EnvState;
using gaq::Model;
using gaq::StepCfg;

template <uint32_t F> struct RealOf { using type = double; };
#define GAQ_REAL_FP32(FEAT) template <> struct RealOf<(FEAT)> { using type = float; };
GAQ_REAL_FP32(48u) GAQ_REAL_FP32(49u) GAQ_REAL_FP32(50u) GAQ_REAL_FP32(51u) GAQ_REAL_FP32(52u) GAQ_REAL_FP32(53u) GAQ_REAL_FP32(54u) GAQ_REAL_FP32(55u)
#undef GAQ_REAL_FP32
template <uint32_t F> using Real = typename RealOf<F>::type;

typedef unsigned int u32x2 __attribute__((ext_vector_type(2)));
typedef unsigned int u32x4 __attribute__((ext_vector_type(4)));
typedef __attribute__((address_space(3))) void lds_void;

struct TileImage { int lo, lag, ou, cmds, actp, goal, gyro, total; };

template <uint32_t F>
__host__ __device__ __forceinline__ TileImage tile_image(const StepCfg& cfg) {
  TileImage t;
  t.lo = kRowsLds;
  int o = (F & gaq::F_FP32) ? kRowsLds : (F & gaq::F_ALIAS) ? kRowsLds + kLoRowsLds : kCoreBytes;
  t.lag = o;  if (gaq::has_lag<F>(cfg)) o += kLagBytes;
  t.ou = o;   if (gaq::noise_mode<F>(cfg) != gaq::NOISE_OFF) o += kGrpBytes;
  t.cmds = o; if (gaq::has_lag<F>(cfg)) o += kGrpBytes;
  t.actp = o; if (gaq::has_act_prev<F>(cfg)) o += kGrpBytes;
  t.goal = o; if (gaq::has_env_goal<F>(cfg)) o += kGrpBytes;
  t.gyro = o; if (gaq::has_gyro_bias<F>(cfg)) o += kGrpBytes;
  t.total = o;
  return t;
}

template <int PIECES, int AUX = GAQ_LD_AUX>
__device__ __forceinline__ void dma_in(const void* g, char* l, uint32_t lane) {
  auto r = __builtin_amdgcn_make_buffer_rsrc(const_cast<void*>(g), 0, PIECES * 1024, 0x00020000);
#pragma unroll
  for (int k = 0; k < PIECES; ++k)
    __builtin_amdgcn_raw_ptr_buffer_load_lds(r, (lds_void*)(l + k * 1024), 16, lane * 16u, k * 1024, 0, AUX);
}
template <int PIECES, int AUX = GAQ_ST_AUX>
__device__ __forceinline__ void copy_out(void* g, const char* l, uint32_t lane) {
  auto r = __builtin_amdgcn_make_buffer_rsrc(g, 0, PIECES * 1024, 0x00020000);
#pragma unroll
  for (int k = 0; k < PIECES; ++k) {
    const u32x4 v = *reinterpret_cast<const u32x4*>(l + k * 1024 + lane * 16u);
    __builtin_amdgcn_raw_buffer_store_b128(v, r, lane * 16u, k * 1024, AUX);
  }
}

#ifndef GAQ_RTZ_HEADS
#define GAQ_RTZ_HEADS 1
#endif
__device__ __forceinline__ void heads9_rtz(const double* v, float* h) {
  asm volatile(
      "s_setreg_imm32_b32 hwreg(HW_REG_MODE, 0, 2), 3\n\t"
      "v_cvt_f32_f64 %0, %9\n\tv_cvt_f32_f64 %1, %10\n\tv_cvt_f32_f64 %2, %11\n\tv_cvt_f32_f64 %3, %12\n\tv_cvt_f32_f64 %4, %13\n\t"
      "v_cvt_f32_f64 %5, %14\n\tv_cvt_f32_f64 %6, %15\n\tv_cvt_f32_f64 %7, %16\n\tv_cvt_f32_f64 %8, %17\n\t"
      "s_setreg_imm32_b32 hwreg(HW_REG_MODE, 0, 2), 0"
      : "=&v"(h[0]), "=&v"(h[1]), "=&v"(h[2]), "=&v"(h[3]), "=&v"(h[4]), "=&v"(h[5]), "=&v"(h[6]), "=&v"(h[7]), "=&v"(h[8])
      : "v"(v[0]), "v"(v[1]), "v"(v[2]), "v"(v[3]), "v"(v[4]), "v"(v[5]), "v"(v[6]), "v"(v[7]), "v"(v[8]));
}
template <bool RTZ>
__device__ __forceinline__ void heads18(const double* v, float* h) {
  if constexpr (RTZ && GAQ_RTZ_HEADS) {
    heads9_rtz(v, h); heads9_rtz(v + 9, h + 9);
  } else {
#pragma unroll
    for (int k = 0; k < 18; ++k) h[k] = gaq::split_hi(v[k]);
  }
}

using gaq::split_decode; using gaq::split_hi; using gaq::split_lo; using gaq::split_decode32; using gaq::split_lo32;

__host__ __device__ __forceinline__ double lo_decode(int mode, const float* hi, const void* lo, int64_t i, int k) {
  const float h = hi[i * 18 + k];
  if (mode == 2) return (double)h;
  if (mode == 3) {
    const uint32_t* row = reinterpret_cast<const uint32_t*>(lo) + i * kMixRowWords;
    if (k >= 15) return split_decode32(h, row[8 + (k - 15)]);
    return split_decode(h, row[k >> 1] >> ((k & 1) * 16));
  }
  return split_decode(h, (uint32_t)reinterpret_cast<const uint16_t*>(lo)[i * 18 + k]);
}
__host__ __device__ __forceinline__ void lo_encode(int mode, void* lo, int64_t i, int k, double v) {
  if (mode == 3) {
    uint32_t* row = reinterpret_cast<uint32_t*>(lo) + i * kMixRowWords;
    if (k >= 15) row[8 + (k - 15)] = split_lo32(v);
    else reinterpret_cast<uint16_t*>(row)[k] = (uint16_t)split_lo(v);
  } else if (mode == 1) {
    reinterpret_cast<uint16_t*>(lo)[i * 18 + k] = (uint16_t)split_lo(v);
  }
}

template <int PIECES, int AUX = GAQ_LD_AUX>
__device__ __forceinline__ void dma_in_rows(const void* g, char* l, uint32_t lane, uint32_t nbytes) {
  auto r = __builtin_amdgcn_make_buffer_rsrc(const_cast<void*>(g), 0, (int)nbytes, 0x00020000);
#pragma unroll
  for (int k = 0; k < PIECES; ++k)
    __builtin_amdgcn_raw_ptr_buffer_load_lds(r, (lds_void*)(l + k * 1024), 16, lane * 16u, k * 1024, 0, AUX);
}
template <int PIECES, int TILE_BYTES, int AUX = GAQ_ST_AUX>
__device__ __forceinline__ void copy_out_rows(void* g, const char* l, uint32_t lane, uint32_t nbytes) {
  auto r = __builtin_amdgcn_make_buffer_rsrc(g, 0, (int)nbytes, 0x00020000);
#pragma unroll
  for (int k = 0; k < PIECES; ++k) {
    const uint32_t off = k * 1024 + lane * 16u;
    if (off < (uint32_t)TILE_BYTES) {
      const u32x4 v = *reinterpret_cast<const u32x4*>(l + off);
      __builtin_amdgcn_raw_buffer_store_b128(v, r, off, 0, AUX);
    }
  }
}

template <uint32_t F>
__device__ __forceinline__ void stage_in(const DevPtrs& p, const StepCfg& cfg, int64_t tile, char* buf, uint32_t lane) {
  const TileImage im = tile_image<F>(cfg);
  if constexpr ((F & gaq::F_ALIAS) != 0) {
    const int64_t first = tile * kTile;
    const uint32_t live = (uint32_t)((p.n - first) < kTile ? (p.n - first) : kTile);
    dma_in_rows<5, kLdAux<F>>(p.obs_in + first * 18, buf, lane, live * kRowBytes);
    if constexpr ((F & gaq::F_FP32) == 0)
      {
        if constexpr (kLoMix<F>) dma_in_rows<3, kLdAux<F>>(reinterpret_cast<const uint32_t*>(p.lo) + first * kMixRowWords, buf + kRowsLds, lane, kMixRowsBytes);
        else dma_in_rows<3, kLdAux<F>>(reinterpret_cast<const int16_t*>(p.lo) + first * 18, buf + kRowsLds, lane, kLoRowsBytes);
      }
  } else {
    dma_in<9, kLdAux<F>>(p.core + tile * (kCorePlanes * kTile), buf, lane);
  }
  if (gaq::has_lag<F>(cfg)) {
    dma_in<2, kLdAux<F>>(p.lag + tile * (kLagPlanes * kTile), buf + im.lag, lane);
    dma_in<1, kLdAux<F>>(p.cmds + tile * (4 * kTile), buf + im.cmds, lane);
  }
  if (gaq::noise_mode<F>(cfg) != gaq::NOISE_OFF) dma_in<1, kLdAux<F>>(p.ou + tile * (4 * kTile), buf + im.ou, lane);
  if (gaq::has_act_prev<F>(cfg)) dma_in<1, kLdAux<F>>(p.actp + tile * (4 * kTile), buf + im.actp, lane);
  if (gaq::has_env_goal<F>(cfg)) dma_in<1, kLdAux<F>>(p.goal + tile * (4 * kTile), buf + im.goal, lane);
  if (gaq::has_gyro_bias<F>(cfg)) dma_in<1, kLdAux<F>>(p.gyro + tile * (4 * kTile), buf + im.gyro, lane);
}

template <uint32_t F>
__device__ __forceinline__ void read_image(const StepCfg& cfg, const char* buf, uint32_t lane, EnvState<Real<F>>& s) {
  using T = Real<F>;
  const TileImage im = tile_image<F>(cfg);
  if constexpr ((F & gaq::F_FP32) != 0) {
    const float2* h = reinterpret_cast<const float2*>(buf + lane * kRowBytes);
    float v[18];
#pragma unroll
    for (int k = 0; k < 9; ++k) { const float2 a = h[k]; v[2 * k] = a.x; v[2 * k + 1] = a.y; }
#pragma unroll
    for (int j = 0; j < 3; ++j) { s.pos[j] = v[j] + (float)cfg.goal_default[j]; s.vel[j] = v[3 + j]; s.omega[j] = v[15 + j]; }
#pragma unroll
    for (int j = 0; j < 9; ++j) s.rot[j] = v[6 + j];
  } else if constexpr ((F & gaq::F_ALIAS) != 0) {
    const float2* h = reinterpret_cast<const float2*>(buf + lane * kRowBytes);
    double gl[3] = {cfg.goal_default[0], cfg.goal_default[1], cfg.goal_default[2]};
    if constexpr ((F & (gaq::F_SWARM | gaq::F_ENVX)) != 0) {
      if (gaq::has_env_goal<F>(cfg)) {
        const float* g = reinterpret_cast<const float*>(buf + im.goal) + lane;
#pragma unroll
        for (int j = 0; j < 3; ++j) gl[j] = (double)g[j * kTile];
      }
    }
    double v[18];
    if constexpr (kLoMix<F>) {
      const uint32_t* q = reinterpret_cast<const uint32_t*>(buf + kRowsLds + lane * kMixRowBytes);
      float hv[18];
#pragma unroll
      for (int k = 0; k < 9; ++k) { const float2 a = h[k]; hv[2 * k] = a.x; hv[2 * k + 1] = a.y; }
#pragma unroll
      for (int k = 0; k < 8; ++k) {
        const uint32_t w = q[k];
        v[2 * k] = split_decode(hv[2 * k], w);
        if (2 * k + 1 < 15) v[2 * k + 1] = split_decode(hv[2 * k + 1], w >> 16);
      }
#pragma unroll
      for (int j = 0; j < 3; ++j) v[15 + j] = split_decode32(hv[15 + j], q[8 + j]);
    } else {
      const uint32_t* q = reinterpret_cast<const uint32_t*>(buf + kRowsLds + lane * kLoRowBytes);
#pragma unroll
      for (int k = 0; k < 9; ++k) {
        const float2 a = h[k];
        const uint32_t w = q[k];
        v[2 * k] = split_decode(a.x, w);
        v[2 * k + 1] = split_decode(a.y, w >> 16);
      }
    }
#pragma unroll
    for (int j = 0; j < 3; ++j) { s.pos[j] = v[j] + gl[j]; s.vel[j] = v[3 + j]; s.omega[j] = v[15 + j]; }
#pragma unroll
    for (int j = 0; j < 9; ++j) s.rot[j] = v[6 + j];
  } else {
    const double* c = reinterpret_cast<const double*>(buf) + lane;
#pragma unroll
    for (int j = 0; j < 3; ++j) s.pos[j] = c[(0 + j) * kTile];
#pragma unroll
    for (int j = 0; j < 3; ++j) s.vel[j] = c[(3 + j) * kTile];
#pragma unroll
    for (int j = 0; j < 9; ++j) s.rot[j] = c[(6 + j) * kTile];
#pragma unroll
    for (int j = 0; j < 3; ++j) s.omega[j] = c[(15 + j) * kTile];
  }
#pragma unroll
  for (int j = 0; j < 4; ++j) { s.rot_damp[j] = T(0); s.cmds_damp[j] = 0.0f; s.ou[j] = 0.0f; s.act_prev[j] = 0.0f; }
#pragma unroll
  for (int j = 0; j < 3; ++j) { s.goal[j] = T(cfg.goal_default[j]); s.gyro_bias[j] = 0.0f; }
  if (gaq::has_gyro_bias<F>(cfg)) {
    const float* g = reinterpret_cast<const float*>(buf + im.gyro) + lane;
#pragma unroll
    for (int j = 0; j < 3; ++j) s.gyro_bias[j] = g[j * kTile];
  }
  if (gaq::has_lag<F>(cfg)) {
    const double* l = reinterpret_cast<const double*>(buf + im.lag) + lane;
    const float* m = reinterpret_cast<const float*>(buf + im.cmds) + lane;
#pragma unroll
    for (int j = 0; j < 4; ++j) { s.rot_damp[j] = T(l[j * kTile]); s.cmds_damp[j] = m[j * kTile]; }
  }
  if (gaq::noise_mode<F>(cfg) != gaq::NOISE_OFF) {
    const float* o = reinterpret_cast<const float*>(buf + im.ou) + lane;
#pragma unroll
    for (int j = 0; j < 4; ++j) s.ou[j] = o[j * kTile];
  }
  if (gaq::has_act_prev<F>(cfg)) {
    const float* a = reinterpret_cast<const float*>(buf + im.actp) + lane;
#pragma unroll
    for (int j = 0; j < 4; ++j) s.act_prev[j] = a[j * kTile];
  }
  if (gaq::has_env_goal<F>(cfg)) {
    const float* g = reinterpret_cast<const float*>(buf + im.goal) + lane;
#pragma unroll
    for (int j = 0; j < 3; ++j) s.goal[j] = T(g[j * kTile]);
  }
}

template <uint32_t F>
__device__ __forceinline__ void write_image(const StepCfg& cfg, char* buf, uint32_t lane, const EnvState<Real<F>>& s) {
  const TileImage im = tile_image<F>(cfg);
  if constexpr ((F & gaq::F_FP32) != 0) {
    float v[18];
#pragma unroll
    for (int j = 0; j < 3; ++j) { v[j] = s.pos[j] - (float)cfg.goal_default[j]; v[3 + j] = s.vel[j]; v[15 + j] = s.omega[j]; }
#pragma unroll
    for (int j = 0; j < 9; ++j) v[6 + j] = s.rot[j];
    float2* h = reinterpret_cast<float2*>(buf + lane * kRowBytes);
#pragma unroll
    for (int k = 0; k < 9; ++k) h[k] = make_float2(v[2 * k], v[2 * k + 1]);
  } else if constexpr ((F & gaq::F_ALIAS) != 0) {
    double v[18];
#pragma unroll
    for (int j = 0; j < 3; ++j) {
      if constexpr ((F & (gaq::F_SWARM | gaq::F_ENVX)) != 0) v[j] = s.pos[j] - s.goal[j]; else v[j] = s.pos[j] - cfg.goal_default[j];
      v[3 + j] = s.vel[j]; v[15 + j] = s.omega[j];
    }
#pragma unroll
    for (int j = 0; j < 9; ++j) v[6 + j] = s.rot[j];
    float2* h = reinterpret_cast<float2*>(buf + lane * kRowBytes);
    float hv[18];
    heads18<gaq::kHeadsAreObs<F>>(v, hv);
    if constexpr (kLoMix<F>) {
      uint32_t* q = reinterpret_cast<uint32_t*>(buf + kRowsLds + lane * kMixRowBytes);
#pragma unroll
      for (int k = 0; k < 9; ++k) h[k] = make_float2(hv[2 * k], hv[2 * k + 1]);
#pragma unroll
      for (int k = 0; k < 8; ++k) q[k] = split_lo(v[2 * k]) | ((2 * k + 1 < 15) ? (split_lo(v[2 * k + 1]) << 16) : 0u);
#pragma unroll
      for (int j = 0; j < 3; ++j) q[8 + j] = split_lo32(v[15 + j]);
    } else {
      uint32_t* q = reinterpret_cast<uint32_t*>(buf + kRowsLds + lane * kLoRowBytes);
#pragma unroll
      for (int k = 0; k < 9; ++k) {
        h[k] = make_float2(hv[2 * k], hv[2 * k + 1]);
        q[k] = split_lo(v[2 * k]) | (split_lo(v[2 * k + 1]) << 16);
      }
    }
  } else {
    double* c = reinterpret_cast<double*>(buf) + lane;
#pragma unroll
    for (int j = 0; j < 3; ++j) c[(0 + j) * kTile] = s.pos[j];
#pragma unroll
    for (int j = 0; j < 3; ++j) c[(3 + j) * kTile] = s.vel[j];
#pragma unroll
    for (int j = 0; j < 9; ++j) c[(6 + j) * kTile] = s.rot[j];
#pragma unroll
    for (int j = 0; j < 3; ++j) c[(15 + j) * kTile] = s.omega[j];
  }
  if (gaq::has_lag<F>(cfg)) {
    double* l = reinterpret_cast<double*>(buf + im.lag) + lane;
    float* m = reinterpret_cast<float*>(buf + im.cmds) + lane;
#pragma unroll
    for (int j = 0; j < 4; ++j) { l[j * kTile] = (double)s.rot_damp[j]; m[j * kTile] = s.cmds_damp[j]; }
  }
  if (gaq::noise_mode<F>(cfg) != gaq::NOISE_OFF) {
    float* o = reinterpret_cast<float*>(buf + im.ou) + lane;
#pragma unroll
    for (int j = 0; j < 4; ++j) o[j * kTile] = s.ou[j];
  }
  if (gaq::has_act_prev<F>(cfg)) {
    float* a = reinterpret_cast<float*>(buf + im.actp) + lane;
#pragma unroll
    for (int j = 0; j < 4; ++j) a[j * kTile] = s.act_prev[j];
  }
  if (gaq::has_env_goal<F>(cfg)) {
    float* g = reinterpret_cast<float*>(buf + im.goal) + lane;
#pragma unroll
    for (int j = 0; j < 3; ++j) g[j * kTile] = (float)s.goal[j];
  }
  if (gaq::has_gyro_bias<F>(cfg)) {
    float* g = reinterpret_cast<float*>(buf + im.gyro) + lane;
#pragma unroll
    for (int j = 0; j < 3; ++j) g[j * kTile] = s.gyro_bias[j];
    g[3 * kTile] = 0.0f;
  }
}

template <uint32_t F>
__device__ __forceinline__ void stage_out(const DevPtrs& p, const StepCfg& cfg, int64_t tile, const char* buf, uint32_t lane,
                                          float* obs) {
  const TileImage im = tile_image<F>(cfg);
  if constexpr ((F & gaq::F_ALIAS) != 0) {
    const int64_t first = tile * kTile;
    const uint32_t live = (uint32_t)((p.n - first) < kTile ? (p.n - first) : kTile);
    copy_out_rows<5, kRowsBytes, kStAux<F>>(obs + first * 18, buf, lane, live * kRowBytes);
    if constexpr ((F & gaq::F_PACK) == 0)
      if (p.obs_copy) copy_out_rows<5, kRowsBytes, kCopyAux<F>>(p.obs_copy + first * 18, buf, lane, live * kRowBytes);
    if constexpr ((F & gaq::F_FP32) == 0)
      {
        if constexpr (kLoMix<F>) copy_out_rows<3, kMixRowsBytes, kStAux<F>>(reinterpret_cast<uint32_t*>(p.lo) + first * kMixRowWords, buf + kRowsLds, lane, kMixRowsBytes);
        else copy_out_rows<3, kLoRowsBytes, kStAux<F>>(reinterpret_cast<int16_t*>(p.lo) + first * 18, buf + kRowsLds, lane, kLoRowsBytes);
      }
  } else {
    copy_out<9, kStAux<F>>(p.core + tile * (kCorePlanes * kTile), buf, lane);
  }
  if (gaq::has_lag<F>(cfg)) {
    copy_out<2, kStAux<F>>(p.lag + tile * (kLagPlanes * kTile), buf + im.lag, lane);
    copy_out<1, kStAux<F>>(p.cmds + tile * (4 * kTile), buf + im.cmds, lane);
  }
  if (gaq::noise_mode<F>(cfg) != gaq::NOISE_OFF) copy_out<1, kStAux<F>>(p.ou + tile * (4 * kTile), buf + im.ou, lane);
  if (gaq::has_act_prev<F>(cfg)) copy_out<1, kStAux<F>>(p.actp + tile * (4 * kTile), buf + im.actp, lane);
  if (gaq::has_env_goal<F>(cfg) && (cfg.resample_goal || cfg.excite))
    copy_out<1, kStAux<F>>(p.goal + tile * (4 * kTile), buf + im.goal, lane);
  if (gaq::has_gyro_bias<F>(cfg)) copy_out<1, kStAux<F>>(p.gyro + tile * (4 * kTile), buf + im.gyro, lane);
}

template <typename T>
__device__ __forceinline__ void convert_model(const Model<double>& a, Model<T>& m) {
  m.mass = T(a.mass); m.inv_mass = T(a.inv_mass);
#pragma unroll
  for (int j = 0; j < 3; ++j) { m.inertia[j] = T(a.inertia[j]); m.inv_inertia[j] = T(a.inv_inertia[j]); }
#pragma unroll
  for (int j = 0; j < 4; ++j) {
    m.thrust_max[j] = T(a.thrust_max[j]); m.torque_max[j] = T(a.torque_max[j]);
    m.prop_x[j] = T(a.prop_x[j]); m.prop_y[j] = T(a.prop_y[j]); m.prop_z[j] = T(a.prop_z[j]);
  }
  m.tau_up = T(a.tau_up); m.tau_down = T(a.tau_down); m.linearity = T(a.linearity); m.arm = T(a.arm);
  m.vel_damp = T(a.vel_damp); m.damp_omega_q = T(a.damp_omega_q); m.c_drag = T(a.c_drag); m.c_roll = T(a.c_roll);
  m.ou_sigma = a.ou_sigma; m.jinv = a.jinv;
}

template <uint32_t F, bool MODEL_IN_VGPRS = false>
__device__ __forceinline__ void load_model(const DevPtrs& p, const StepCfg& cfg, int64_t tile, uint32_t lane,
                                           const Model<double>& um, Model<Real<F>>& m) {
  using T = Real<F>;
  if constexpr ((F & gaq::F_PER_ENV) == 0) {
    if constexpr ((F & gaq::F_FP32) != 0) convert_model(um, m); else m = um;
#ifndef GAQ_VG_EXTRA
#define GAQ_VG_EXTRA 0u
#endif
    if constexpr (((F & gaq::F_NT) != 0 && (F & gaq::F_PREDRAW) == 0 && (F & gaq::F_FP32) == 0) || (MODEL_IN_VGPRS && (F & gaq::F_FP32) == 0) ||
                  ((F & (GAQ_VG_EXTRA)) != 0 && (F & (gaq::F_FP32 | gaq::F_GENERIC)) == 0)) {
#define GAQ_VG(x) asm volatile("" : "+v"(x))
      GAQ_VG(m.inv_mass); GAQ_VG(m.linearity); GAQ_VG(m.vel_damp); GAQ_VG(m.damp_omega_q); GAQ_VG(m.arm);
#pragma unroll
      for (int j = 0; j < 3; ++j) { GAQ_VG(m.inertia[j]); GAQ_VG(m.inv_inertia[j]); }
#pragma unroll
      for (int j = 0; j < 4; ++j) { GAQ_VG(m.thrust_max[j]); GAQ_VG(m.torque_max[j]); GAQ_VG(m.prop_x[j]); GAQ_VG(m.prop_y[j]); }
      if constexpr ((F & gaq::F_LAG) != 0) { GAQ_VG(m.tau_up); GAQ_VG(m.tau_down); }
#undef GAQ_VG
    }
    return;
  }
  auto r = __builtin_amdgcn_make_buffer_rsrc(const_cast<double*>(p.par + tile * (kPar * kTile)), 0, kParBytes, 0x00020000);
  const uint32_t o8 = lane * 8u;
  auto ld = [&](int plane) { return T(__builtin_bit_cast(double, __builtin_amdgcn_raw_buffer_load_b64(r, o8, plane * (kTile * 8), 0))); };
  m.inv_mass = ld(PP_INV_MASS);
  if (cfg.compact_params && (F & gaq::F_FP32) == 0) {
    auto ldd = [&](int plane) { return __builtin_bit_cast(double, __builtin_amdgcn_raw_buffer_load_b64(r, o8, plane * (kTile * 8), 0)); };
    const double t2t = ldd(PP_T2T), mx = ldd(PP_MX), my = ldd(PP_MY), cx = ldd(PP_COMX), cy = ldd(PP_COMY);
    const double sx[4] = {1.0, -1.0, -1.0, 1.0}, sy[4] = {-1.0, -1.0, 1.0, 1.0};
#pragma unroll
    for (int j = 0; j < 3; ++j) { const double in = ldd(PP_INERTIA + j); m.inertia[j] = T(in); m.inv_inertia[j] = T(1.0 / in); }
#pragma unroll
    for (int j = 0; j < 4; ++j) {
      const double th = ldd(PP_THRUST_MAX + j);
      m.thrust_max[j] = T(th); m.torque_max[j] = T(t2t * th);
      m.prop_x[j] = T(sx[j] * mx - cx); m.prop_y[j] = T(sy[j] * my - cy);
    }
  } else {
#pragma unroll
    for (int j = 0; j < 3; ++j) { m.inertia[j] = ld(PP_INERTIA + j); m.inv_inertia[j] = ld(PP_INV_INERTIA + j); }
#pragma unroll
    for (int j = 0; j < 4; ++j) {
      m.thrust_max[j] = ld(PP_THRUST_MAX + j); m.torque_max[j] = ld(PP_TORQUE_MAX + j);
      m.prop_x[j] = ld(PP_PROP_X + j); m.prop_y[j] = ld(PP_PROP_Y + j);
    }
  }
  m.linearity = ld(PP_LINEARITY); m.arm = ld(PP_ARM);
  m.vel_damp = T(0); m.damp_omega_q = T(0);
  if (!cfg.zero_damp) { m.vel_damp = ld(PP_VEL_DAMP); m.damp_omega_q = ld(PP_DAMP_Q); }
  m.tau_up = T(1); m.tau_down = T(1);
  if (gaq::has_lag<F>(cfg)) { m.tau_up = ld(PP_TAU_UP); m.tau_down = ld(PP_TAU_DOWN); }
  m.ou_sigma = 0.0f;
  if (gaq::noise_mode<F>(cfg) != gaq::NOISE_OFF)
    m.ou_sigma = __builtin_bit_cast(float, __builtin_amdgcn_raw_buffer_load_b32(r, lane * 4u, PP_OU_SIGMA * (kTile * 8), 0));
  m.mass = T(0); m.c_drag = T(0); m.c_roll = T(0);
  m.jinv = p.jinv ? p.jinv + (tile * kTile + lane) * 16 : nullptr;
#pragma unroll
  for (int j = 0; j < 4; ++j) m.prop_z[j] = T(0);
  if (((F & gaq::F_GENERIC) != 0) && cfg.drag) {
    m.mass = ld(PP_MASS); m.c_drag = ld(PP_C_DRAG); m.c_roll = ld(PP_C_ROLL);
#pragma unroll
    for (int j = 0; j < 4; ++j) m.prop_z[j] = ld(PP_PROP_Z + j);
  }
}

__device__ __forceinline__ void flush_obs(float* obs, int64_t n, int D, int64_t tile, const char* rows, uint32_t lane) {
  const int64_t first = tile * kTile;
  const int64_t live = (n - first) < kTile ? (n - first) : kTile;
  const uint32_t bytes = (uint32_t)live * D * 4u;
  auto r = __builtin_amdgcn_make_buffer_rsrc(obs + first * D, 0, (int)bytes, 0x00020000);
  const int pieces = (kTile * D * 4 + 1023) / 1024;
  for (int k = 0; k < pieces; ++k) {
    const uint32_t off = k * 1024 + lane * 16u;
    if (off < (uint32_t)(kTile * D * 4)) {
      const u32x4 v = *reinterpret_cast<const u32x4*>(rows + off);
      __builtin_amdgcn_raw_buffer_store_b128(v, r, off, 0, GAQ_ST_AUX);
    }
  }
}

struct WaveSwarm {
  uint32_t lane; int agents;
  __device__ __forceinline__ void neighbour(int j, const float* me, float* o) const {
    const int src = (int)((lane & ~(uint32_t)(agents - 1)) | ((lane + (uint32_t)j) & (uint32_t)(agents - 1)));
#pragma unroll
    for (int k = 0; k < 6; ++k) o[k] = __shfl(me[k], src);
  }
  __device__ __forceinline__ bool any(bool b) const { return __any(b) != 0; }
};

__device__ __forceinline__ void wait_dma() { asm volatile("s_waitcnt vmcnt(0)" ::: "memory"); }
__device__ __forceinline__ void wave_lds_fence() {
  __builtin_amdgcn_fence(__ATOMIC_RELEASE, "wavefront");
  __builtin_amdgcn_wave_barrier();
  __builtin_amdgcn_fence(__ATOMIC_ACQUIRE, "wavefront");
}

constexpr int kCtrSlots = 64;
constexpr int kCtrStride = 544;
__device__ __forceinline__ uint64_t step_counter_read(const DevPtrs& p, uint32_t lane) {
  static_assert(kCtrSlots == kTile, "one counter word per lane");
  return p.step_ctr[lane * kCtrStride];
}
__device__ __forceinline__ uint64_t step_counter_sum(uint64_t c) {
#pragma unroll
  for (int o = 1; o < kCtrSlots; o <<= 1) c += __shfl_xor(c, o);
  const uint32_t lo = __builtin_amdgcn_readfirstlane((uint32_t)c), hi = __builtin_amdgcn_readfirstlane((uint32_t)(c >> 32));
  return ((uint64_t)hi << 32) | lo;
}
__device__ __forceinline__ uint64_t step_counter_checkin(const DevPtrs& p, uint64_t raw, uint32_t lane) {
  const uint64_t c = step_counter_sum(raw);
  const uint32_t gwave = __builtin_amdgcn_readfirstlane(blockIdx.x * (uint32_t)(kBlock / kTile) + (threadIdx.x >> 6));
  if (lane == 0) {
    uint32_t inc = gwave == 0 ? p.ctr_inc0 : 1u;
    uint32_t dep = (uint32_t)c;
    asm volatile("" : "+s"(inc) : "s"(dep));
    (void)__hip_atomic_fetch_add(p.step_ctr + (gwave % (uint32_t)kCtrSlots) * kCtrStride, (uint64_t)inc, __ATOMIC_RELAXED,
                                 __HIP_MEMORY_SCOPE_AGENT);
  }
  return c >> p.ctr_shift;
}
__device__ __forceinline__ uint64_t step_counter_peek(const DevPtrs& p, uint32_t lane) {
  return step_counter_sum(step_counter_read(p, lane)) >> p.ctr_shift;
}

template <int AUX>
__device__ __forceinline__ void flush_packed_rows(float* rows_out, int64_t n, int W, int64_t tile, char* lds, uint32_t lane) {
  const int64_t first = tile * kTile;
  const int64_t live = (n - first) < kTile ? (n - first) : kTile;
  const uint32_t bytes = (uint32_t)live * W * 4u;
  auto r = __builtin_amdgcn_make_buffer_rsrc(rows_out + first * W, 0, (int)bytes, 0x00020000);
  const int pieces = (kTile * W * 4 + 1023) / 1024;
  for (int k = 0; k < pieces; ++k) {
    const uint32_t off = k * 1024 + lane * 16u;
    if (off < (uint32_t)(kTile * W * 4)) {
      const u32x4 v = *reinterpret_cast<const u32x4*>(lds + off);
      __builtin_amdgcn_raw_buffer_store_b128(v, r, off, 0, AUX);
    }
  }
}

__device__ __forceinline__ void store_aux(const DevPtrs& p, int64_t i, const gaq::StepOut& out) {
  if (!p.aux) return;
  float* ax = p.aux + i * gaq::AUX_WORDS;
#pragma unroll
  for (int j = 0; j < 3; ++j) { ax[gaq::AUX_ACC + j] = out.acc_meter[j]; ax[gaq::AUX_OMEGA_DOT + j] = out.omega_dot[j]; ax[gaq::AUX_TORQUE + j] = out.torque[j]; }
#pragma unroll
  for (int j = 0; j < 4; ++j) { ax[gaq::AUX_CTRL + j] = out.ctrl[j]; ax[gaq::AUX_CMDS + j] = out.cmds[j]; }
}

struct KernArgsMirror { DevPtrs p; StepCfg cfg; Model<double> um; };
static_assert(offsetof(KernArgsMirror, um) == sizeof(DevPtrs) + sizeof(StepCfg) && sizeof(DevPtrs) % 8 == 0 && sizeof(StepCfg) % 8 == 0,
              "kernel-argument layout of step_kernel's first three arguments");
typedef __attribute__((address_space(4))) const char karg_char;
__device__ __forceinline__ karg_char* kernarg_model_ptr() {
#if defined(__HIP_DEVICE_COMPILE__)
  return (karg_char*)__builtin_amdgcn_kernarg_segment_ptr() + offsetof(KernArgsMirror, um);
#else
  return nullptr;
#endif
}

template <uint32_t F> constexpr int kStepMinWaves = 1;
#ifndef GAQ_NO_FLOORS
template <> inline constexpr int kStepMinWaves<214036u> = 3;
template <> inline constexpr int kStepMinWaves<82962u> = 3;
#endif
template <uint32_t F>
__global__ __launch_bounds__(kBlock) __attribute__((amdgpu_waves_per_eu(kStepMinWaves<F>))) void step_kernel(DevPtrs p, StepCfg cfg, Model<double> um,
                                                       const float* __restrict__ actions, float* obs,
                                                       float* __restrict__ reward, uint8_t* __restrict__ done,
                                                       int lds_per_wave) {
  constexpr bool G = (F & gaq::F_GENERIC) != 0;
  constexpr bool A = (F & gaq::F_ALIAS) != 0;
  static_assert(!(G && A), "obs/state aliasing exists in the specialised kernels only");
  extern __shared__ __attribute__((aligned(16))) char smem[];
  const int wave = __builtin_amdgcn_readfirstlane(threadIdx.x >> 6);
  const uint32_t lane = threadIdx.x & 63u;
  const int64_t tile = (int64_t)blockIdx.x * (kBlock / kTile) + wave;
  if constexpr ((F & gaq::F_CTR) != 0) {
    if (tile >= p.ntiles) {
      (void)step_counter_checkin(p, step_counter_read(p, lane), lane);
      return;
    }
  } else {
    if (p.step_ctr) cfg.step_index = *p.step_ctr >> p.ctr_shift;
    if (tile >= p.ntiles) return;
  }
  char* buf = smem + wave * lds_per_wave;
  const int64_t i = tile * kTile + lane;
  const bool live = i < p.n;
  const int D = cfg.obs_dim;

  stage_in<F>(p, cfg, tile, buf, lane);
  using T = Real<F>;
  Model<T> m;
  if constexpr (!gaq::kModelMem<F>) load_model<F>(p, cfg, tile, lane, um, m);
  const Model<T>* mp = &m;
  if constexpr (gaq::kModelMem<F>) mp = (const Model<T>*)kernarg_model_ptr();
  float4 a4;
  uint32_t cw;
  {
    auto ra = __builtin_amdgcn_make_buffer_rsrc(const_cast<float*>(actions), 0, (int)(p.n * 16), 0x00020000);
    const u32x4 v = __builtin_amdgcn_raw_buffer_load_b128(ra, (uint32_t)i * 16u, 0, (F & gaq::F_NT) ? 2 : GAQ_ACT_AUX);
    a4 = __builtin_bit_cast(float4, v);
    auto rc = __builtin_amdgcn_make_buffer_rsrc(p.ctr, 0, (int)(p.ntiles * kTile * 4), 0x00020000);
    cw = __builtin_amdgcn_raw_buffer_load_b32(rc, (uint32_t)i * 4u, 0, (F & gaq::F_NT) ? 2 : GAQ_ACT_AUX);
  }
  if constexpr ((F & gaq::F_CTR) != 0) cfg.step_index = step_counter_checkin(p, step_counter_read(p, lane), lane);
  float pre0[4] = {0.0f, 0.0f, 0.0f, 0.0f}, pre1[4] = {0.0f, 0.0f, 0.0f, 0.0f};
  if constexpr ((F & gaq::F_PREDRAW) != 0) {
    const gaq::Philox r0(cfg.seed, cfg.env_offset + (uint64_t)i, cfg.step_index, gaq::RNG_OU0);
    gaq::normals4(r0, pre0);
    if (cfg.sim_steps > 1) { const gaq::Philox r1(cfg.seed, cfg.env_offset + (uint64_t)i, cfg.step_index, gaq::RNG_OU0 + 1u); gaq::normals4(r1, pre1); }
  }
  if constexpr ((F & gaq::F_PREDRAW) != 0) {
    asm volatile("" :: "v"(pre0[0]), "v"(pre0[1]), "v"(pre0[2]), "v"(pre0[3]), "v"(pre1[0]), "v"(pre1[1]), "v"(pre1[2]), "v"(pre1[3]));
  }
  wait_dma();
  EnvState<T> s;
  read_image<F>(cfg, buf, lane, s);
  s.tick = cw & 0xFFFFu;
  s.svd_ctr = cw >> 16;
  wave_lds_fence();

  const float act[4] = {a4.x, a4.y, a4.z, a4.w};
  gaq::StepOut out;
  out.reward = 0.0f; out.done = 0; out.crashed = 0;
  constexpr int kObWords = (F & gaq::F_AUXP) ? 28 : 26;
  float ob[kObWords];
#pragma unroll
  for (int k = 0; k < kObWords; ++k) ob[k] = 0.0f;
  char* rows = buf;
  float* term_row = p.term_obs ? p.term_obs + i * D : nullptr;
#ifndef GAQ_PACK_ROWS_LDS
#define GAQ_PACK_ROWS_LDS 0
#endif
  constexpr bool kObsRowsInLds = G || (F & gaq::F_SWARM) != 0 || (F & gaq::F_AUXP) != 0 ||
                                 (GAQ_PACK_ROWS_LDS && (F & gaq::F_PACK) != 0 && (F & gaq::F_ALIAS) != 0);
  constexpr bool kAuxRowsInLds = gaq::kAuxIsRow<F>;
  const int aux_off = (kTile * D * 4 + 15) & ~15;
  if (live && !ablated(cfg, 1)) {
    if constexpr ((F & gaq::F_SWARM) != 0) {
      float* row = reinterpret_cast<float*>(rows) + lane * D;
      gaq::env_step<T, F>(s, *mp, cfg, act, cfg.env_offset + (uint64_t)i, [&](int, int) { return 0.0f; }, out,
                          [&](int k, float v, int) { row[k] = v; }, term_row, WaveSwarm{lane, cfg.swarm.agents});
    } else if constexpr (G) {
      const float* nz = p.noise_in;
      const int64_t n = p.n;
      float* row = reinterpret_cast<float*>(rows) + lane * D;
      if constexpr (kAuxRowsInLds) out.aux_row = reinterpret_cast<float*>(rows + aux_off) + lane * gaq::AUX_WORDS;
      const float* sz = p.sense_in;
      gaq::env_step<T, F>(s, *mp, cfg, act, cfg.env_offset + (uint64_t)i,
                               [&](int k, int c) { return nz[((int64_t)k * 4 + c) * n + i]; }, out,
                               [&](int k, float v, int) { row[k] = v; }, term_row, WaveSwarm{lane, cfg.swarm.agents},
                               [&](int c, int slot, int j) { return sz ? sz[((int64_t)(c * 12 + slot) * 3 + j) * n + i] : 0.0f; });
      if constexpr (gaq::kAux<F> && !kAuxRowsInLds) store_aux(p, i, out);
    } else if constexpr (gaq::kHeadsAreObs<F>) {
      gaq::env_step<T, F>(s, *mp, cfg, act, cfg.env_offset + (uint64_t)i, [&](int k, int c) { return k == 0 ? pre0[c] : pre1[c]; }, out,
                          [&](int, float, int) {}, term_row);
    } else if constexpr (kObsRowsInLds) {
      float* row = reinterpret_cast<float*>(rows) + lane * D;
      if constexpr (kAuxRowsInLds) out.aux_row = reinterpret_cast<float*>(rows + aux_off) + lane * gaq::AUX_WORDS;
      gaq::env_step<T, F>(s, *mp, cfg, act, cfg.env_offset + (uint64_t)i, [&](int, int) { return 0.0f; }, out,
                          [&](int k, float v, int) { row[k] = v; }, term_row);
      if constexpr (gaq::kAux<F> && !kAuxRowsInLds) store_aux(p, i, out);
    } else {
      gaq::env_step<T, F>(s, *mp, cfg, act, cfg.env_offset + (uint64_t)i, [&](int, int) { return 0.0f; }, out,
                          [&](int k, float v, int slot) { if (slot < 0) ob[k] = v; else ob[18 + slot] = v; }, term_row);
      if constexpr (gaq::kAux<F>) store_aux(p, i, out);
    }
  }
  bool promote = false;
  if constexpr ((F & gaq::F_RZ) != 0) {
    if (p.rz_every > 0 && live && out.done && !ablated(cfg, 4)) {
      auto rt = __builtin_amdgcn_make_buffer_rsrc(p.traj, 0, (int)(p.ntiles * (3 * kTile * 4)), 0x00020000);
      const int third = (int)(p.ntiles * (kTile * 4));
      bool due = true;
      if (p.rz_every > 1) {
        const uint32_t tr = __builtin_amdgcn_raw_buffer_load_b32(rt, (uint32_t)i * 4u, 0, 0) + 1u;
        __builtin_amdgcn_raw_buffer_store_b32(tr, rt, (uint32_t)i * 4u, 0, 0);
        due = ((tr + 1u) % (uint32_t)p.rz_every) == 0u;
      }
      if (due) {
        promote = true;
        (void)__builtin_amdgcn_raw_ptr_buffer_atomic_add_i32(1, rt, (uint32_t)i * 4u, third, 0);
        (void)__builtin_amdgcn_raw_ptr_buffer_atomic_add_i32(1, rt, (uint32_t)i * 4u, 2 * third, 0);
        s.svd_ctr = 0;
#pragma unroll
        for (int j = 0; j < 4; ++j) s.ou[j] = 0.0f;
      }
    }
  }
  if constexpr (kObsRowsInLds) {
    wave_lds_fence();
    if constexpr (A) flush_obs(p.obs_copy, p.n, D, tile, rows, lane);
    else flush_obs(obs, p.n, D, tile, rows, lane);
    if constexpr (kAuxRowsInLds) { if (p.aux) flush_obs(p.aux, p.n, gaq::AUX_WORDS, tile, rows + aux_off, lane); }
    wave_lds_fence();
  }
  write_image<F>(cfg, buf, lane, s);
  wave_lds_fence();
  stage_out<F>(p, cfg, tile, buf, lane, obs);
  {
    auto rc = __builtin_amdgcn_make_buffer_rsrc(p.ctr, 0, (int)(p.ntiles * kTile * 4), 0x00020000);
    __builtin_amdgcn_raw_buffer_store_b32((s.tick & 0xFFFFu) | (s.svd_ctr << 16), rc, (uint32_t)i * 4u, 0, kStAux<F>);
  }
  if (live) {
    reward[i] = out.reward;
    done[i] = out.done;
    if (!isfinite(out.reward)) atomicAdd(p.nan_count, 1u);
  }
  if constexpr (!gaq::kHeadsAreObs<F> && !kObsRowsInLds) {
    float* obs_rows_out = obs;
    if constexpr (A) obs_rows_out = p.obs_copy;
    wave_lds_fence();
    float* row = reinterpret_cast<float*>(rows) + lane * D;
    if (D == 18) {
#pragma unroll
      for (int k = 0; k < 18; k += 2) *reinterpret_cast<float2*>(row + k) = make_float2(ob[k], ob[k + 1]);
    } else {
      int k = 18;
      bool quat = false;
      if constexpr ((F & gaq::F_AUXP) != 0) quat = (cfg.obs_flags & gaq::OBS_QUAT) != 0;
      if (quat) {
#pragma unroll
        for (int j = 0; j < 13; ++j) row[j] = ob[j];
        k = 13;
      } else {
#pragma unroll
        for (int j = 0; j < 18; ++j) row[j] = ob[j];
      }
      if (cfg.obs_flags & gaq::OBS_APPEND_H) row[k++] = ob[18];
      if (cfg.obs_flags & gaq::OBS_APPEND_ACC) { row[k] = ob[19]; row[k + 1] = ob[20]; row[k + 2] = ob[21]; k += 3; }
      if (cfg.obs_flags & gaq::OBS_APPEND_ACT) { row[k] = ob[22]; row[k + 1] = ob[23]; row[k + 2] = ob[24]; row[k + 3] = ob[25]; k += 4; }
      if constexpr ((F & gaq::F_AUXP) != 0) {
        if (cfg.obs_flags & gaq::OBS_APPEND_T2W) row[k++] = ob[26];
        if (cfg.obs_flags & gaq::OBS_APPEND_T2T) row[k++] = ob[27];
      }
    }
    wave_lds_fence();
    flush_obs(obs_rows_out, p.n, D, tile, rows, lane);
  }

  if constexpr ((F & gaq::F_ROWS) != 0) {
    static_assert(gaq::kHeadsAreObs<F> && (F & gaq::F_FP32) == 0, "fused packed rows: alias kernels whose observation is the heads");
    float hv[18];
    const float2* h = reinterpret_cast<const float2*>(buf + lane * kRowBytes);
#pragma unroll
    for (int k = 0; k < 9; ++k) { const float2 a = h[k]; hv[2 * k] = a.x; hv[2 * k + 1] = a.y; }
    wave_lds_fence();
    float* row = reinterpret_cast<float*>(buf) + lane * 20;
#pragma unroll
    for (int k = 0; k < 18; k += 2) *reinterpret_cast<float2*>(row + k) = make_float2(hv[k], hv[k + 1]);
    *reinterpret_cast<float2*>(row + 18) = make_float2(out.reward, (float)out.done);
    wave_lds_fence();
    flush_packed_rows<kStAux<F>>(p.rows_out, p.n, 20, tile, buf, lane);
  }

  if constexpr ((F & gaq::F_RZ) != 0) {
    unsigned long long pm = __ballot(promote);
    if (pm && !ablated(cfg, 2)) {
      double* cur = const_cast<double*>(p.par) + tile * (int64_t)(kPar * kTile);
      const double* rows = p.par + p.ntiles * (int64_t)(kPar * kTile) + kParNextSkew + tile * (int64_t)(kPar * kTile);
      const bool hot_only = cfg.compact_params != 0 && cfg.zero_damp != 0 && (F & gaq::F_FP32) == 0;
      const int pl = hot_only ? (int)lane + ((int)lane < 4 ? 1 : (int)lane < 9 ? 4 : (int)lane < 13 ? 19 : 23) : (int)lane;
      static_assert(PP_INV_MASS == 1 && PP_INERTIA == 2 && PP_THRUST_MAX == 8 && PP_TORQUE_MAX == 12 && PP_TAU_UP == 28 && PP_TAU_DOWN == 29 &&
                    PP_LINEARITY == 30 && PP_ARM == 31 && PP_OU_SIGMA == 36 && PP_T2T == 37 && PP_COMY == 41, "hot planes of a promotion");
      const bool mine = hot_only ? (int)lane < kHotPlanes : (int)lane < kPar;
      while (pm) {
        const int L = __ffsll((long long)pm) - 1;
        pm &= pm - 1ull;
        if (mine) {
          const double v = rows[L * kPar + pl];
          if (pl == PP_OU_SIGMA) reinterpret_cast<float*>(cur + PP_OU_SIGMA * kTile)[L] = (float)v;
          else cur[pl * kTile + L] = v;
        }
      }
    }
  }
  if (p.done_list) {
    const bool is_done = live && out.done;
    uint32_t* cnt = p.done_count + (cfg.step_index & 1);
    if (i == 0) p.done_count[(cfg.step_index + 1) & 1] = 0;
    const unsigned long long mask = __ballot(is_done);
    if (mask) {
      const int leader = __ffsll((long long)mask) - 1;
      uint32_t base = 0;
      if ((int)lane == leader) base = atomicAdd(cnt, (uint32_t)__popcll(mask));
      base = __shfl(base, leader);
      if (is_done) p.done_list[base + __popcll(mask & ((1ull << lane) - 1ull))] = (uint32_t)i;
    }
  }
}

constexpr int kPolMaxHidden = 3;
constexpr int kPolMaxWidth = 128;
constexpr int kPolChunk = 16;
struct PolicyDev {
  const float* w;
  int32_t in_dim, n_hidden, hidden_act, out_tanh;
  int32_t width[kPolMaxHidden];
  int32_t off[kPolMaxHidden + 1];
  int32_t explore;
  float std4[4];
  int32_t scratch_bytes;
};
typedef __attribute__((address_space(4))) const float kconst_float;
__device__ __forceinline__ kconst_float* as_const(const float* p) { return (kconst_float*)(uintptr_t)p; }
__device__ __forceinline__ float pol_act(int act, float v) { return act == 0 ? tanhf(v) : fmaxf(v, 0.0f); }

__device__ __forceinline__ void policy_out_tail(const PolicyDev& P, uint64_t seed, uint64_t env, uint64_t step, float out[4]) {
  if (P.out_tanh) {
#pragma unroll
    for (int o = 0; o < 4; ++o) out[o] = tanhf(out[o]);
  }
  if (P.explore) {
    float z[4];
    const gaq::Philox r(seed, env, step, gaq::RNG_POLICY);
    gaq::normals4(r, z);
#pragma unroll
    for (int o = 0; o < 4; ++o) out[o] = __builtin_fmaf(P.std4[o], z[o], out[o]);
  }
}

__device__ __forceinline__ void policy_eval(const PolicyDev& P, const float* x, float* scratch, uint32_t lane, uint64_t seed,
                                            uint64_t env, uint64_t step, float out[4]) {
  const int nh = P.n_hidden;
  kconst_float* wo = as_const(P.w + P.off[nh]);
  const int last_w = P.width[nh - 1];
#pragma unroll
  for (int o = 0; o < 4; ++o) out[o] = wo[last_w * 4 + o];
  int in = P.in_dim;
  const float* hin = nullptr;
  int sc_off = 0;
#pragma unroll 1
  for (int l = 0; l < nh; ++l) {
    const int width = P.width[l];
    kconst_float* wl = as_const(P.w + P.off[l]);
    kconst_float* bl = wl + width * in;
    const bool last = l == nh - 1;
    float* hout = scratch + sc_off * kTile;
#pragma unroll 1
    for (int c = 0; c < width; c += kPolChunk) {
      float acc[kPolChunk];
#pragma unroll
      for (int j = 0; j < kPolChunk; ++j) acc[j] = bl[c + j];
      kconst_float* wc = wl + c * in;
      auto fold = [&](float v, int k) {
#pragma unroll
        for (int j = 0; j < kPolChunk; ++j) acc[j] = __builtin_fmaf(wc[k * kPolChunk + j], v, acc[j]);
      };
      if (hin) {
#pragma unroll 2
        for (int k = 0; k < in; ++k) fold(hin[k * kTile + lane], k);
      } else {
#pragma unroll 2
        for (int k = 0; k < in; ++k) fold(x[k], k);
      }
#pragma unroll
      for (int j = 0; j < kPolChunk; ++j) acc[j] = pol_act(P.hidden_act, acc[j]);
      if (last) {
#pragma unroll
        for (int j = 0; j < kPolChunk; ++j) {
#pragma unroll
          for (int o = 0; o < 4; ++o) out[o] = __builtin_fmaf(wo[(c + j) * 4 + o], acc[j], out[o]);
        }
      } else {
#pragma unroll
        for (int j = 0; j < kPolChunk; ++j) hout[(c + j) * kTile + lane] = acc[j];
      }
    }
    if (!last) { wave_lds_fence(); hin = hout; sc_off += width; in = width; }
  }
  policy_out_tail(P, seed, env, step, out);
  wave_lds_fence();
}

template <uint32_t F> constexpr int kRollMinWaves = 1;
template <uint32_t F>
__global__ __launch_bounds__(kBlock) __attribute__((amdgpu_waves_per_eu(kRollMinWaves<F>))) void rollout_kernel(DevPtrs p, StepCfg cfg, Model<double> um, int T,
                                                          const float* __restrict__ actions, float* obs,
                                                          float* __restrict__ reward, uint8_t* __restrict__ done,
                                                          int lds_per_wave) {
  static_assert((F & gaq::F_ALIAS) != 0 && (F & gaq::F_GENERIC) == 0, "fused rollout: alias layout only");
  extern __shared__ __attribute__((aligned(16))) char smem[];
  const int wave = __builtin_amdgcn_readfirstlane(threadIdx.x >> 6);
  const uint32_t lane = threadIdx.x & 63u;
  if (p.step_ctr) cfg.step_index = step_counter_peek(p, lane);
  const int64_t tile = (int64_t)blockIdx.x * (kBlock / kTile) + wave;
  if (tile >= p.ntiles) return;
  char* buf = smem + wave * lds_per_wave;
  const int64_t i = tile * kTile + lane;
  const bool live = i < p.n;
  const int64_t first = tile * kTile;
  const uint32_t nlive = (uint32_t)((p.n - first) < kTile ? (p.n - first) : kTile);
  const TileImage im = tile_image<F>(cfg);

  stage_in<F>(p, cfg, tile, buf, lane);
  using RT = Real<F>;
  Model<RT> m;
  load_model<F, true>(p, cfg, tile, lane, um, m);
  auto rc = __builtin_amdgcn_make_buffer_rsrc(p.ctr, 0, (int)(p.ntiles * kTile * 4), 0x00020000);
  const uint32_t cw = __builtin_amdgcn_raw_buffer_load_b32(rc, (uint32_t)i * 4u, 0, 0);
  auto load_action = [&](int t) {
    auto ra = __builtin_amdgcn_make_buffer_rsrc(const_cast<float*>(actions + ((int64_t)t * p.n + first) * 4), 0,
                                                (int)(nlive * 16u), 0x00020000);
    return __builtin_amdgcn_raw_buffer_load_b128(ra, lane * 16u, 0, 0);
  };
  u32x4 a_next = load_action(0);
  wait_dma();
  EnvState<RT> s;
  read_image<F>(cfg, buf, lane, s);
  s.tick = cw & 0xFFFFu;
  s.svd_ctr = cw >> 16;
  wave_lds_fence();
  StepCfg c = cfg;
  for (int t = 0; t < T; ++t) {
    const float4 a4 = __builtin_bit_cast(float4, a_next);
    if (t + 1 < T) a_next = load_action(t + 1);
    const float act[4] = {a4.x, a4.y, a4.z, a4.w};
    gaq::StepOut out;
    out.reward = 0.0f; out.done = 0; out.crashed = 0;
    float* term_row = p.term_obs ? p.term_obs + i * 18 : nullptr;
    if (live)
      gaq::env_step<RT, F>(s, m, c, act, c.env_offset + (uint64_t)i, [&](int, int) { return 0.0f; }, out,
                          [&](int, float, int) {}, term_row);
    {
      RT v[18];
#pragma unroll
      for (int j = 0; j < 3; ++j) { v[j] = s.pos[j] - RT(cfg.goal_default[j]); v[3 + j] = s.vel[j]; v[15 + j] = s.omega[j]; }
#pragma unroll
      for (int j = 0; j < 9; ++j) v[6 + j] = s.rot[j];
      float2* h = reinterpret_cast<float2*>(buf + lane * kRowBytes);
      if constexpr ((F & gaq::F_FP32) != 0) {
#pragma unroll
        for (int k = 0; k < 9; ++k) h[k] = make_float2((float)v[2 * k], (float)v[2 * k + 1]);
#pragma unroll
        for (int j = 0; j < 3; ++j) s.pos[j] = RT((float)v[j]) + RT(cfg.goal_default[j]);
      } else {
        double vd[18];
#pragma unroll
        for (int k = 0; k < 18; ++k) vd[k] = (double)v[k];
        float hv[18];
        heads18<true>(vd, hv);
#pragma unroll
        for (int k = 0; k < 9; ++k) h[k] = make_float2(hv[2 * k], hv[2 * k + 1]);
      }
    }
    wave_lds_fence();
    const int64_t slot = (int64_t)t * p.n;
    copy_out_rows<5, kRowsBytes>(obs + (slot + first) * 18, buf, lane, nlive * kRowBytes);
    if (live) {
      reward[slot + i] = out.reward;
      done[slot + i] = out.done;
      if (!isfinite(out.reward)) atomicAdd(p.nan_count, 1u);
    }
    wave_lds_fence();
    c.step_index += 1;
  }
  write_image<F>(cfg, buf, lane, s);
  wave_lds_fence();
  if (p.hi_final) copy_out_rows<5, kRowsBytes>(p.hi_final + first * 18, buf, lane, nlive * kRowBytes);
  if constexpr ((F & gaq::F_FP32) == 0) {
    if constexpr (kLoMix<F>) copy_out_rows<3, kMixRowsBytes>(reinterpret_cast<uint32_t*>(p.lo) + first * kMixRowWords, buf + im.lo, lane, kMixRowsBytes);
    else copy_out_rows<3, kLoRowsBytes>(reinterpret_cast<int16_t*>(p.lo) + first * 18, buf + im.lo, lane, kLoRowsBytes);
  }
  if (gaq::has_lag<F>(cfg)) {
    copy_out<2>(p.lag + tile * (kLagPlanes * kTile), buf + im.lag, lane);
    copy_out<1>(p.cmds + tile * (4 * kTile), buf + im.cmds, lane);
  }
  if (gaq::noise_mode<F>(cfg) != gaq::NOISE_OFF) copy_out<1>(p.ou + tile * (4 * kTile), buf + im.ou, lane);
  __builtin_amdgcn_raw_buffer_store_b32((s.tick & 0xFFFFu) | (s.svd_ctr << 16), rc, (uint32_t)i * 4u, 0, 0);
}

template <uint32_t F>
__device__ __forceinline__ void policy_rollout_body(const DevPtrs& p, StepCfg cfg, const Model<double>& um, int T, float* obs,
                                                    float* __restrict__ reward, uint8_t* __restrict__ done, char* buf, int64_t tile,
                                                    uint32_t lane, const PolicyDev* pol, float* pol_scratch, float* __restrict__ act_out) {
  const int64_t i = tile * kTile + lane;
  const bool live = i < p.n;
  const int64_t first = tile * kTile;
  const uint32_t nlive = (uint32_t)((p.n - first) < kTile ? (p.n - first) : kTile);
  const TileImage im = tile_image<F>(cfg);

  stage_in<F>(p, cfg, tile, buf, lane);
  using RT = Real<F>;
  Model<RT> m;
  load_model<F, true>(p, cfg, tile, lane, um, m);
  auto rc = __builtin_amdgcn_make_buffer_rsrc(p.ctr, 0, (int)(p.ntiles * kTile * 4), 0x00020000);
  const uint32_t cw = __builtin_amdgcn_raw_buffer_load_b32(rc, (uint32_t)i * 4u, 0, 0);
  wait_dma();
  EnvState<RT> s;
  read_image<F>(cfg, buf, lane, s);
  s.tick = cw & 0xFFFFu;
  s.svd_ctr = cw >> 16;
  wave_lds_fence();
  StepCfg c = cfg;
  for (int t = 0; t < T; ++t) {
    float act[4];
    policy_eval(*pol, reinterpret_cast<const float*>(buf + lane * kRowBytes), pol_scratch, lane, c.seed, c.env_offset + (uint64_t)i,
                c.step_index, act);
    if (act_out && live) {
      const u32x4 v = __builtin_bit_cast(u32x4, make_float4(act[0], act[1], act[2], act[3]));
      auto ro = __builtin_amdgcn_make_buffer_rsrc(act_out + ((int64_t)t * p.n + first) * 4, 0, (int)(nlive * 16u), 0x00020000);
      __builtin_amdgcn_raw_buffer_store_b128(v, ro, lane * 16u, 0, 0);
    }
    gaq::StepOut out;
    out.reward = 0.0f; out.done = 0; out.crashed = 0;
    float* term_row = p.term_obs ? p.term_obs + i * 18 : nullptr;
    if (live)
      gaq::env_step<RT, F>(s, m, c, act, c.env_offset + (uint64_t)i, [&](int, int) { return 0.0f; }, out,
                          [&](int, float, int) {}, term_row);
    {
      RT v[18];
#pragma unroll
      for (int j = 0; j < 3; ++j) { v[j] = s.pos[j] - RT(cfg.goal_default[j]); v[3 + j] = s.vel[j]; v[15 + j] = s.omega[j]; }
#pragma unroll
      for (int j = 0; j < 9; ++j) v[6 + j] = s.rot[j];
      float2* h = reinterpret_cast<float2*>(buf + lane * kRowBytes);
      if constexpr ((F & gaq::F_FP32) != 0) {
#pragma unroll
        for (int k = 0; k < 9; ++k) h[k] = make_float2((float)v[2 * k], (float)v[2 * k + 1]);
#pragma unroll
        for (int j = 0; j < 3; ++j) s.pos[j] = RT((float)v[j]) + RT(cfg.goal_default[j]);
      } else {
        double vd[18];
#pragma unroll
        for (int k = 0; k < 18; ++k) vd[k] = (double)v[k];
        float hv[18];
        heads18<true>(vd, hv);
#pragma unroll
        for (int k = 0; k < 9; ++k) h[k] = make_float2(hv[2 * k], hv[2 * k + 1]);
      }
    }
    wave_lds_fence();
    const int64_t slot = (int64_t)t * p.n;
    copy_out_rows<5, kRowsBytes>(obs + (slot + first) * 18, buf, lane, nlive * kRowBytes);
    if (live) {
      reward[slot + i] = out.reward;
      done[slot + i] = out.done;
      if (!isfinite(out.reward)) atomicAdd(p.nan_count, 1u);
    }
    wave_lds_fence();
    c.step_index += 1;
  }
  write_image<F>(cfg, buf, lane, s);
  wave_lds_fence();
  if (p.hi_final) copy_out_rows<5, kRowsBytes>(p.hi_final + first * 18, buf, lane, nlive * kRowBytes);
  if constexpr ((F & gaq::F_FP32) == 0) {
    if constexpr (kLoMix<F>) copy_out_rows<3, kMixRowsBytes>(reinterpret_cast<uint32_t*>(p.lo) + first * kMixRowWords, buf + im.lo, lane, kMixRowsBytes);
    else copy_out_rows<3, kLoRowsBytes>(reinterpret_cast<int16_t*>(p.lo) + first * 18, buf + im.lo, lane, kLoRowsBytes);
  }
  if (gaq::has_lag<F>(cfg)) {
    copy_out<2>(p.lag + tile * (kLagPlanes * kTile), buf + im.lag, lane);
    copy_out<1>(p.cmds + tile * (4 * kTile), buf + im.cmds, lane);
  }
  if (gaq::noise_mode<F>(cfg) != gaq::NOISE_OFF) copy_out<1>(p.ou + tile * (4 * kTile), buf + im.ou, lane);
  __builtin_amdgcn_raw_buffer_store_b32((s.tick & 0xFFFFu) | (s.svd_ctr << 16), rc, (uint32_t)i * 4u, 0, 0);
}

constexpr int kPolBlock = kTile;
template <uint32_t F>
__global__ __launch_bounds__(kPolBlock) void policy_rollout_kernel(DevPtrs p, StepCfg cfg, Model<double> um, int T, PolicyDev pol,
                                                                   float* __restrict__ act_out, float* obs, float* __restrict__ reward,
                                                                   uint8_t* __restrict__ done, int lds_per_wave) {
  static_assert((F & gaq::F_ALIAS) != 0 && (F & gaq::F_GENERIC) == 0, "fused rollout: alias layout only");
  extern __shared__ __attribute__((aligned(16))) char smem[];
  const uint32_t lane = threadIdx.x & 63u;
  if (p.step_ctr) cfg.step_index = step_counter_peek(p, lane);
  const int64_t tile = (int64_t)blockIdx.x;
  if (tile >= p.ntiles) return;
  float* scratch = reinterpret_cast<float*>(smem + ((lds_per_wave + 15) & ~15));
  policy_rollout_body<F>(p, cfg, um, T, obs, reward, done, smem, tile, lane, &pol, scratch, act_out);
}

}

#define GAQ_STEP_PART0(X) X(8u) X(1u) X(3u) X(16u) X(48u) X(2049u) X(2065u) X(3089u) X(2097u) X(4116u) X(8468u) X(16384u) X(33808u) X(197648u) X(459792u) X(197649u) X(199697u) X(16385u) X(16401u) X(18433u) X(18449u)
#define GAQ_STEP_PART1(X) X(9u) X(0u) X(2u) X(17u) X(49u) X(2051u) X(2067u) X(3091u) X(4244u) X(4372u) X(8470u) X(16386u) X(33810u) X(17424u) X(197650u) X(459794u) X(197651u) X(199699u) X(16387u) X(16403u) X(18435u) X(18451u)
#define GAQ_STEP_PART2(X) X(72u) X(2057u) X(4u) X(18u) X(50u) X(2053u) X(2069u) X(3093u) X(4500u) X(4118u) X(8471u) X(16388u) X(33812u) X(66578u) X(66583u) X(68625u) X(16389u) X(16405u) X(18437u) X(18453u)
#define GAQ_STEP_PART3(X) X(73u) X(2121u) X(5u) X(19u) X(51u) X(2055u) X(2071u) X(3095u) X(4246u) X(4374u) X(8596u) X(16390u) X(33814u) X(17426u) X(197652u) X(459796u) X(197653u) X(199701u) X(16391u) X(16407u) X(18439u) X(18455u)
#define GAQ_STEP_PART4(X) X(520u) X(6u) X(20u) X(52u) X(1040u) X(1041u) X(148u) X(276u) X(2099u) X(4502u) X(16400u) X(16402u) X(66576u) X(66581u) X(68627u) X(17425u) X(82960u) X(214032u) X(19473u)
#define GAQ_STEP_PART5(X) X(521u) X(7u) X(21u) X(53u) X(1042u) X(1043u) X(150u) X(278u) X(2101u) X(4119u) X(8598u) X(584u) X(17428u) X(197654u) X(459798u) X(197655u) X(199703u) X(17427u) X(82962u) X(214034u) X(19475u)
#define GAQ_STEP_PART6(X) X(2569u) X(22u) X(54u) X(1044u) X(1045u) X(151u) X(279u) X(404u) X(2103u) X(4247u) X(16404u) X(66580u) X(66577u) X(68631u) X(17429u) X(82964u) X(214036u) X(19477u)
#define GAQ_STEP_PART7(X) X(23u) X(55u) X(1046u) X(1047u) X(406u) X(407u) X(4375u) X(4503u) X(8599u) X(16406u) X(17430u) X(66582u) X(66579u) X(68629u) X(17431u) X(82966u) X(214038u) X(19479u)
#define GAQ_STEP_ALL(X) GAQ_STEP_PART0(X) GAQ_STEP_PART1(X) GAQ_STEP_PART2(X) GAQ_STEP_PART3(X) GAQ_STEP_PART4(X) GAQ_STEP_PART5(X) \
                        GAQ_STEP_PART6(X) GAQ_STEP_PART7(X)
#define GAQ_ROLL_PART0(X) X(16u) X(48u)
#define GAQ_ROLL_PART1(X) X(17u) X(49u)
#define GAQ_ROLL_PART2(X) X(18u) X(50u)
#define GAQ_ROLL_PART3(X) X(19u) X(51u)
#define GAQ_ROLL_PART4(X) X(20u) X(52u)
#define GAQ_ROLL_PART5(X) X(21u) X(53u)
#define GAQ_ROLL_PART6(X) X(22u) X(54u)
#define GAQ_ROLL_PART7(X) X(23u) X(55u)
#define GAQ_ROLL_ALL(X) GAQ_ROLL_PART0(X) GAQ_ROLL_PART1(X) GAQ_ROLL_PART2(X) GAQ_ROLL_PART3(X) GAQ_ROLL_PART4(X) GAQ_ROLL_PART5(X) \
                        GAQ_ROLL_PART6(X) GAQ_ROLL_PART7(X)
#define GAQ_STEP_SIG(FEAT) \
  void gaqk::step_kernel<(FEAT)>(gaqk::DevPtrs, gaq::StepCfg, gaq::Model<double>, const float*, float*, float*, uint8_t*, int);
#define GAQ_PROLL_PART0(X) X(16u) X(48u)
#define GAQ_PROLL_PART1(X) X(17u) X(49u)
#define GAQ_PROLL_PART2(X) X(18u) X(50u)
#define GAQ_PROLL_PART3(X) X(19u) X(51u)
#define GAQ_PROLL_PART4(X) X(20u) X(52u)
#define GAQ_PROLL_PART5(X) X(21u) X(53u)
#define GAQ_PROLL_PART6(X) X(22u) X(54u)
#define GAQ_PROLL_PART7(X) X(23u) X(55u)
#define GAQ_PROLL_ALL(X) GAQ_PROLL_PART0(X) GAQ_PROLL_PART1(X) GAQ_PROLL_PART2(X) GAQ_PROLL_PART3(X) GAQ_PROLL_PART4(X) GAQ_PROLL_PART5(X) \
                         GAQ_PROLL_PART6(X) GAQ_PROLL_PART7(X)
#define GAQ_PROLL_SIG(FEAT) \
  void gaqk::policy_rollout_kernel<(FEAT)>(gaqk::DevPtrs, gaq::StepCfg, gaq::Model<double>, int, gaqk::PolicyDev, float*, float*, float*, uint8_t*, int);
#define GAQ_ROLL_SIG(FEAT) \
  void gaqk::rollout_kernel<(FEAT)>(gaqk::DevPtrs, gaq::StepCfg, gaq::Model<double>, int, const float*, float*, float*, uint8_t*, int);
```

Baseline: 21.45 billion.

## Interleave lo-rows, OU noise and tick counters into one per-tile side buffer

Merges the separate per-tile arrays for low-order split bits, OU noise state and the tick/SVD counter word into one contiguous 'side' region per tile. Kernels now stage it into LDS with a single span DMA and write it back with one span store, replacing the scattered per-lane counter load/store and separate lo/ou copies. The aim is fewer, larger, more contiguous HBM transactions per tile. In exchange the LDS image layout and offsets change, a slack region is added to the LDS budget (possibly hurting occupancy), and all host pack/unpack and reset paths move to the new stride-based addressing.

```diff
diff --git a/gym_art_amd/csrc/gaq.hip b/gym_art_amd/csrc/gaq.hip
--- a/gym_art_amd/csrc/gaq.hip
+++ b/gym_art_amd/csrc/gaq.hip
@@ -47,8 +47,8 @@
   const int64_t k = (int64_t)blockIdx.x * kBlock + threadIdx.x;
   if (k >= count) return;
   const int64_t i = idx ? idx[k] : first + k;
-  p.ctr[i] &= 0xFFFFu;
-  float* ou = p.ou + (i / kTile) * (4 * kTile) + (i % kTile);
+  side_ctr(p.side, p.side_stride, i / kTile)[i % kTile] &= 0xFFFFu;
+  float* ou = side_ou(p.side, p.side_stride, i / kTile) + (i % kTile);
 #pragma unroll
   for (int j = 0; j < 4; ++j) ou[j * kTile] = 0.0f;
 }
@@ -90,8 +90,8 @@
   P(PP_COMPACT_OK) = 1.0;
   if (staged) return;
   pfull_of(p)[i] = p.rcount[i];
-  p.ctr[i] &= 0xFFFFu;
-  float* ou = p.ou + (i / kTile) * (4 * kTile) + (i % kTile);
+  side_ctr(p.side, p.side_stride, i / kTile)[i % kTile] &= 0xFFFFu;
+  float* ou = side_ou(p.side, p.side_stride, i / kTile) + (i % kTile);
 #pragma unroll
   for (int j = 0; j < 4; ++j) ou[j * kTile] = 0.0f;
 }
@@ -153,12 +153,13 @@
     else gaq::perturb_tree(rz.base, rz.ratio, rz.sampler, cfg.seed, cfg.env_offset + (uint64_t)i, rc - 1, t);
     gaq::DerivedModel dm;
     gaq::derive_tree(t, dm, rz.sampler == 2);
-    const uint32_t keep = p.ctr[i];
+    uint32_t* cp = side_ctr(p.side, p.side_stride, i / kTile) + (i % kTile);
+    const uint32_t keep = *cp;
     float ou[4];
-    float* op = p.ou + (i / kTile) * (4 * kTile) + (i % kTile);
+    float* op = side_ou(p.side, p.side_stride, i / kTile) + (i % kTile);
     for (int j = 0; j < 4; ++j) ou[j] = op[j * kTile];
     write_model_planes(p, cfg.dt, i, dm);
-    p.ctr[i] = keep;
+    *cp = keep;
     for (int j = 0; j < 4; ++j) op[j * kTile] = ou[j];
     if (p.rz_every > 0) p.rz_flag[i] = 1u;
     return;
@@ -269,7 +270,7 @@
     if (alias) {
       double v[18];
 #pragma unroll
-      for (int k = 0; k < 18; ++k) v[k] = lo_decode(alias, p.obs_in, p.lo, i, k);
+      for (int k = 0; k < 18; ++k) v[k] = lo_decode(alias, p.obs_in, p.side, p.side_stride, i, k);
 #pragma unroll
       for (int j = 0; j < 3; ++j) { s.pos[j] = v[j] + s.goal[j]; s.vel[j] = v[3 + j]; s.omega[j] = v[15 + j]; }
 #pragma unroll
@@ -283,8 +284,9 @@
     }
 #pragma unroll
     for (int j = 0; j < 4; ++j) { s.rot_damp[j] = t.ld64(p.lag, kLagPlanes, j); s.cmds_damp[j] = t.ld32(p.cmds, j);
-                                  s.ou[j] = t.ld32(p.ou, j); s.act_prev[j] = t.ld32(p.actp, j); }
-    const uint32_t cw = p.ctr[i];
+                                  s.ou[j] = side_ou(p.side, p.side_stride, tile)[j * kTile + lane]; s.act_prev[j] = t.ld32(p.actp, j); }
+    uint32_t* cp = side_ctr(p.side, p.side_stride, tile) + lane;
+    const uint32_t cw = *cp;
     s.tick = cw & 0xFFFFu; s.svd_ctr = cw >> 16;
     float acc[3] = {0.0f, 0.0f, 9.81f};
     float hist[4] = {s.act_prev[0], s.act_prev[1], s.act_prev[2], s.act_prev[3]};
@@ -302,7 +304,7 @@
 #pragma unroll
       for (int j = 0; j < 4; ++j) { t.st64(p.lag, kLagPlanes, j, s.rot_damp[j]); t.st32(p.cmds, j, s.cmds_damp[j]);
                                     t.st32(p.actp, j, s.act_prev[j]); }
-      p.ctr[i] = (s.tick & 0xFFFFu) | (s.svd_ctr << 16);
+      *cp = (s.tick & 0xFFFFu) | (s.svd_ctr << 16);
       hist[0] = hist[1] = hist[2] = hist[3] = 0.0f;
     }
     float hi18[18];
@@ -317,7 +319,7 @@
 #pragma unroll
       for (int k = 0; k < 18; ++k) {
         if (alias == 2) { hi18[k] = (float)v[k]; }
-        else { lo_encode(alias, p.lo, i, k, v[k]); hi18[k] = split_hi(v[k]); }
+        else { lo_encode(alias, p.side, p.side_stride, i, k, v[k]); hi18[k] = split_hi(v[k]); }
       }
       if (hi_out) {
 #pragma unroll
@@ -373,17 +375,17 @@
   for (int k = 0; k < 3; ++k) out[(34 + k) * n + i] = grp(p.goal, k);
   if (alias) {
     for (int k = 0; k < 18; ++k)
-      out[(int64_t)k * n + i] = lo_decode(alias, p.obs_in, p.lo, i, k) + (k < 3 ? grp(p.goal, k) : 0.0);
+      out[(int64_t)k * n + i] = lo_decode(alias, p.obs_in, p.side, p.side_stride, i, k) + (k < 3 ? grp(p.goal, k) : 0.0);
   } else {
     for (int k = 0; k < kCorePlanes; ++k) out[(int64_t)k * n + i] = p.core[tile * (kCorePlanes * kTile) + k * kTile + lane];
   }
   for (int j = 0; j < 4; ++j) {
     out[(18 + j) * n + i] = p.lag[tile * (kLagPlanes * kTile) + j * kTile + lane];
     out[(22 + j) * n + i] = grp(p.cmds, j);
-    out[(26 + j) * n + i] = grp(p.ou, j);
+    out[(26 + j) * n + i] = (double)side_ou(p.side, p.side_stride, tile)[j * kTile + lane];
     out[(30 + j) * n + i] = grp(p.actp, j);
   }
-  const uint32_t c = p.ctr[i];
+  const uint32_t c = side_ctr(p.side, p.side_stride, tile)[lane];
   out[37 * n + i] = (double)(c & 0xFFFFu);
   out[38 * n + i] = (double)(c >> 16);
   for (int k = 0; k < 3; ++k) out[(39 + k) * n + i] = grp(p.gyro, k);
@@ -689,9 +691,8 @@
       lpw = lpw > both ? lpw : both;
     }
   } else {
-    int img = (L.fp32 ? kRowsLds : L.alias ? kRowsLds + kLoRowsLds : kCoreBytes) +
+    int img = (L.alias ? kRowsLds : kCoreBytes) + side_lo_bytes(f) + kSideTailBytes + kSideSlack +
               (sc.motor_lag ? kLagBytes + kGrpBytes : 0) +
-              (c.noise == GAQ_NOISE_PHILOX ? kGrpBytes : 0) +
               ((sc.need_act_prev && (!L.alias || L.pack)) ? kGrpBytes : 0) +
               (sc.swarm.agents > 1 ? kGrpBytes : 0) +
               ((f & gaq::F_ENVX) && sc.per_env_goal ? kGrpBytes : 0) +
@@ -1089,21 +1090,20 @@
     he = hipMalloc(p, bytes);
     if (he == hipSuccess) he = hipMemset(*p, 0, bytes);
   };
+  d.side_stride = (uint32_t)((e->alias && !e->fp32 ? (e->lomix ? kMixRowsBytes : kLoRowsBytes) : 0) + kSideTailBytes);
+  alloc0((void**)&d.side, nt * (size_t)d.side_stride);
   if (e->alias) {
-    if (!e->fp32) alloc0((void**)&d.lo, nt * (e->lomix ? (size_t)kMixRowsBytes : (size_t)kLoRowsBytes));
     alloc0((void**)&e->own_obs, nt * kRowsBytes);
   } else {
     alloc0((void**)&d.core, nt * kCoreBytes);
   }
   alloc0((void**)&d.lag, nt * kLagBytes);
-  alloc0((void**)&d.ou, nt * kGrpBytes);
   alloc0((void**)&d.cmds, nt * kGrpBytes);
   alloc0((void**)&d.actp, nt * kGrpBytes);
   alloc0((void**)&d.goal, nt * kGrpBytes);
   alloc0((void**)&d.gyro, nt * kGrpBytes);
   alloc0((void**)&e->step_ctr_mem, sizeof(uint64_t) * kCtrSlots * kCtrStride);
   alloc0((void**)&e->alias_sum_dev, sizeof(uint64_t));
-  alloc0((void**)&d.ctr, nt * kTile * sizeof(uint32_t));
   alloc0((void**)&d.done_count, sizeof(uint32_t) * 2);
   alloc0((void**)&d.nan_count, sizeof(uint32_t));
   if (cfg->compact_done) alloc0((void**)&d.done_list, nt * kTile * sizeof(uint32_t));
@@ -1173,8 +1173,8 @@
   (void)hipSetDevice(e->cfg.device);
   if (e->stream) (void)hipStreamSynchronize(e->stream);
   (void)hipDeviceSynchronize();
-  (void)hipFree(e->d.core); (void)hipFree(e->d.lo); (void)hipFree(e->own_obs); (void)hipFree(e->d.lag); (void)hipFree(e->d.ou); (void)hipFree(e->d.cmds);
-  (void)hipFree(e->d.actp); (void)hipFree(e->d.goal); (void)hipFree(e->d.gyro); (void)hipFree(e->step_ctr_mem); if (e->info_pin) (void)hipHostFree(e->info_pin); (void)hipFree(e->alias_sum_dev); (void)hipFree(e->d.ctr);
+  (void)hipFree(e->d.core); (void)hipFree(e->d.side); (void)hipFree(e->own_obs); (void)hipFree(e->d.lag); (void)hipFree(e->d.cmds);
+  (void)hipFree(e->d.actp); (void)hipFree(e->d.goal); (void)hipFree(e->d.gyro); (void)hipFree(e->step_ctr_mem); if (e->info_pin) (void)hipHostFree(e->info_pin); (void)hipFree(e->alias_sum_dev);
   (void)hipFree(e->d.done_count); (void)hipFree(e->d.nan_count); (void)hipFree(e->d.done_list);
   (void)hipFree(e->d.ep_ret); (void)hipFree(e->d.ep_len); (void)hipFree(e->d.ep_acc); (void)hipFree(e->d.aux);
   (void)hipFree(const_cast<double*>(e->d.par)); (void)hipFree(const_cast<double*>(e->d.jinv));
@@ -1795,47 +1795,45 @@
   const int64_t n = e->d.n;
   const size_t nt = (size_t)e->d.ntiles;
   std::vector<double> core(nt * kCorePlanes * kTile, 0.0), lag(nt * kLagPlanes * kTile, 0.0);
-  std::vector<float> ou(nt * 4 * kTile, 0.f), cmds(nt * 4 * kTile, 0.f), actp(nt * 4 * kTile, 0.f), goal(nt * 4 * kTile, 0.f),
+  const uint32_t stride = e->d.side_stride;
+  std::vector<char> side(nt * (size_t)stride, 0);
+  std::vector<float> cmds(nt * 4 * kTile, 0.f), actp(nt * 4 * kTile, 0.f), goal(nt * 4 * kTile, 0.f),
       gyro(nt * 4 * kTile, 0.f);
-  std::vector<uint32_t> c(nt * kTile, 0u);
   for (int64_t i = n; i < (int64_t)(nt * kTile); ++i) { for (int j : {6, 10, 14}) core[tidx(i, kCorePlanes, j)] = 1.0; }
   for (int64_t i = 0; i < n; ++i) {
     for (int pl = 0; pl < kCorePlanes; ++pl) core[tidx(i, kCorePlanes, pl)] = hp[(size_t)pl * n + i];
     for (int j = 0; j < 4; ++j) {
       lag[tidx(i, kLagPlanes, j)] = hp[(size_t)(18 + j) * n + i];
       cmds[tidx(i, 4, j)] = (float)hp[(size_t)(22 + j) * n + i];
-      ou[tidx(i, 4, j)] = (float)hp[(size_t)(26 + j) * n + i];
+      side_ou(side.data(), stride, i / kTile)[j * kTile + i % kTile] = (float)hp[(size_t)(26 + j) * n + i];
       actp[tidx(i, 4, j)] = (float)hp[(size_t)(30 + j) * n + i];
     }
     for (int j = 0; j < 3; ++j) goal[tidx(i, 4, j)] = (float)hp[(size_t)(34 + j) * n + i];
     for (int j = 0; j < 3; ++j) gyro[tidx(i, 4, j)] = (float)hp[(size_t)(39 + j) * n + i];
     const double t = hp[(size_t)37 * n + i], s = hp[(size_t)38 * n + i];
     if (!(t >= 0 && t <= 65535 && s >= 0 && s <= 65535)) return fail(GAQ_ERR_INVALID, "tick / SVD counter out of range");
-    c[i] = ((uint32_t)t & 0xFFFFu) | ((uint32_t)s << 16);
+    side_ctr(side.data(), stride, i / kTile)[i % kTile] = ((uint32_t)t & 0xFFFFu) | ((uint32_t)s << 16);
   }
   if (e->alias) {
     std::vector<float> hi(nt * kTile * 18, 0.0f);
     const int mode = alias_mode(e);
-    std::vector<unsigned char> lo(nt * (size_t)(e->lomix ? kMixRowsBytes : kLoRowsBytes), 0);
     for (int64_t i = 0; i < n; ++i)
       for (int k = 0; k < 18; ++k) {
         const double v = core[tidx(i, kCorePlanes, k)] - (k < 3 ? (double)goal[tidx(i, 4, k)] : 0.0);
         hi[i * 18 + k] = e->fp32 ? (float)v : split_hi(v);
-        lo_encode(mode, lo.data(), i, k, v);
+        lo_encode(mode, side.data(), stride, i, k, v);
       }
     HIP_TRY(hipMemcpy(e->own_obs, hi.data(), hi.size() * 4, hipMemcpyHostToDevice));
-    if (!e->fp32) HIP_TRY(hipMemcpy(e->d.lo, lo.data(), lo.size(), hipMemcpyHostToDevice));
     e->last_obs = e->own_obs;
   } else {
     HIP_TRY(hipMemcpy(e->d.core, core.data(), core.size() * 8, hipMemcpyHostToDevice));
   }
   HIP_TRY(hipMemcpy(e->d.lag, lag.data(), lag.size() * 8, hipMemcpyHostToDevice));
-  HIP_TRY(hipMemcpy(e->d.ou, ou.data(), ou.size() * 4, hipMemcpyHostToDevice));
+  HIP_TRY(hipMemcpy(e->d.side, side.data(), side.size(), hipMemcpyHostToDevice));
   HIP_TRY(hipMemcpy(e->d.cmds, cmds.data(), cmds.size() * 4, hipMemcpyHostToDevice));
   HIP_TRY(hipMemcpy(e->d.actp, actp.data(), actp.size() * 4, hipMemcpyHostToDevice));
   HIP_TRY(hipMemcpy(e->d.goal, goal.data(), goal.size() * 4, hipMemcpyHostToDevice));
   HIP_TRY(hipMemcpy(e->d.gyro, gyro.data(), gyro.size() * 4, hipMemcpyHostToDevice));
-  HIP_TRY(hipMemcpy(e->d.ctr, c.data(), c.size() * 4, hipMemcpyHostToDevice));
   e->rz_refill_now = true;
   return GAQ_OK;
 }
diff --git a/gym_art_amd/csrc/gaq_kernels.hpp b/gym_art_amd/csrc/gaq_kernels.hpp
--- a/gym_art_amd/csrc/gaq_kernels.hpp
+++ b/gym_art_amd/csrc/gaq_kernels.hpp
@@ -44,11 +44,25 @@
 constexpr int kRowsLds = 5 * 1024;
 constexpr int kLoRowBytes = 18 * 2;
 constexpr int kLoRowsBytes = kTile * kLoRowBytes;
-constexpr int kLoRowsLds = 3 * 1024;
 constexpr int kMixRowWords = 11;
 constexpr int kMixRowBytes = kMixRowWords * 4;
 constexpr int kMixRowsBytes = kTile * kMixRowBytes;
 template <uint32_t F> constexpr bool kLoMix = (F & (gaq::F_PER_ENV | gaq::F_LAG)) != 0;
+constexpr int kSideCtrBytes = kTile * 4;
+constexpr int kSideTailBytes = kGrpBytes + kSideCtrBytes;
+constexpr int kSideSlack = 1024 - kSideCtrBytes;
+__host__ __device__ constexpr int side_lo_bytes(uint32_t f) {
+  return ((f & gaq::F_ALIAS) != 0 && (f & gaq::F_FP32) == 0) ? ((f & (gaq::F_PER_ENV | gaq::F_LAG)) != 0 ? kMixRowsBytes : kLoRowsBytes) : 0;
+}
+template <uint32_t F> constexpr int kSideLo = side_lo_bytes(F);
+template <uint32_t F> constexpr int kSideStride = kSideLo<F> + kSideTailBytes;
+__host__ __device__ __forceinline__ char* side_lo(char* side, uint32_t stride, int64_t tile) { return side + tile * (int64_t)stride; }
+__host__ __device__ __forceinline__ float* side_ou(char* side, uint32_t stride, int64_t tile) {
+  return reinterpret_cast<float*>(side + tile * (int64_t)stride + (stride - kSideTailBytes));
+}
+__host__ __device__ __forceinline__ uint32_t* side_ctr(char* side, uint32_t stride, int64_t tile) {
+  return reinterpret_cast<uint32_t*>(side + tile * (int64_t)stride + (stride - kSideCtrBytes));
+}
 constexpr int kPar = 45;
 constexpr int kParBytes = kPar * kTile * 8;
 constexpr int kHotPlanes = 19;
@@ -61,17 +75,15 @@
 
 struct DevPtrs {
   double* core;
-  void* lo;
+  char* side;
   const float* obs_in;
   float* obs_copy;
   float* hi_final;
   double* lag;
-  float* ou;
   float* cmds;
   float* actp;
   float* goal;
   float* gyro;
-  uint32_t* ctr;
   const double* par;
   const double* jinv;
   const float* noise_in;
@@ -94,6 +106,7 @@
   uint32_t* rz_flag;
   uint32_t* rz_overrun;
   int32_t rz_every;
+  uint32_t side_stride;
   int64_t n, ntiles;
 };
 
@@ -111,20 +124,21 @@
 typedef unsigned int u32x4 __attribute__((ext_vector_type(4)));
 typedef __attribute__((address_space(3))) void lds_void;
 
-struct TileImage { int lo, lag, ou, cmds, actp, goal, gyro, total; };
+struct TileImage { int lo, lag, ou, ctr, cmds, actp, goal, gyro, total; };
 
 template <uint32_t F>
 __host__ __device__ __forceinline__ TileImage tile_image(const StepCfg& cfg) {
   TileImage t;
-  t.lo = kRowsLds;
-  int o = (F & gaq::F_FP32) ? kRowsLds : (F & gaq::F_ALIAS) ? kRowsLds + kLoRowsLds : kCoreBytes;
+  int o = (F & gaq::F_ALIAS) ? kRowsLds : kCoreBytes;
   t.lag = o;  if (gaq::has_lag<F>(cfg)) o += kLagBytes;
-  t.ou = o;   if (gaq::noise_mode<F>(cfg) != gaq::NOISE_OFF) o += kGrpBytes;
   t.cmds = o; if (gaq::has_lag<F>(cfg)) o += kGrpBytes;
   t.actp = o; if (gaq::has_act_prev<F>(cfg)) o += kGrpBytes;
   t.goal = o; if (gaq::has_env_goal<F>(cfg)) o += kGrpBytes;
   t.gyro = o; if (gaq::has_gyro_bias<F>(cfg)) o += kGrpBytes;
-  t.total = o;
+  t.lo = o;   o += kSideLo<F>;
+  t.ou = o;   o += kGrpBytes;
+  t.ctr = o;  o += kSideCtrBytes;
+  t.total = o + kSideSlack;
   return t;
 }
 
@@ -169,9 +183,11 @@
 
 using gaq::split_decode; using gaq::split_hi; using gaq::split_lo; using gaq::split_decode32; using gaq::split_lo32;
 
-__host__ __device__ __forceinline__ double lo_decode(int mode, const float* hi, const void* lo, int64_t i, int k) {
+__host__ __device__ __forceinline__ double lo_decode(int mode, const float* hi, const char* side, uint32_t stride, int64_t i, int k) {
   const float h = hi[i * 18 + k];
   if (mode == 2) return (double)h;
+  const char* lo = side_lo(const_cast<char*>(side), stride, i / kTile);
+  i %= kTile;
   if (mode == 3) {
     const uint32_t* row = reinterpret_cast<const uint32_t*>(lo) + i * kMixRowWords;
     if (k >= 15) return split_decode32(h, row[8 + (k - 15)]);
@@ -179,7 +195,10 @@
   }
   return split_decode(h, (uint32_t)reinterpret_cast<const uint16_t*>(lo)[i * 18 + k]);
 }
-__host__ __device__ __forceinline__ void lo_encode(int mode, void* lo, int64_t i, int k, double v) {
+__host__ __device__ __forceinline__ void lo_encode(int mode, char* side, uint32_t stride, int64_t i, int k, double v) {
+  if (mode != 1 && mode != 3) return;
+  char* lo = side_lo(side, stride, i / kTile);
+  i %= kTile;
   if (mode == 3) {
     uint32_t* row = reinterpret_cast<uint32_t*>(lo) + i * kMixRowWords;
     if (k >= 15) row[8 + (k - 15)] = split_lo32(v);
@@ -207,6 +226,52 @@
       __builtin_amdgcn_raw_buffer_store_b128(v, r, off, 0, AUX);
     }
   }
+}
+
+template <int AUX>
+__device__ __forceinline__ void dma_in_span(const char* g, char* l, uint32_t lane, int nbytes) {
+  auto r = __builtin_amdgcn_make_buffer_rsrc(const_cast<char*>(g), 0, nbytes, 0x00020000);
+#pragma unroll
+  for (int o = 0; o < nbytes; o += 1024) __builtin_amdgcn_raw_ptr_buffer_load_lds(r, (lds_void*)(l + o), 16, lane * 16u, o, 0, AUX);
+}
+template <int AUX>
+__device__ __forceinline__ void copy_out_span(char* g, const char* l, uint32_t lane, int nbytes) {
+  auto r = __builtin_amdgcn_make_buffer_rsrc(g, 0, nbytes, 0x00020000);
+#pragma unroll
+  for (int o = 0; o < nbytes; o += 1024) {
+    const u32x4 v = *reinterpret_cast<const u32x4*>(l + o + lane * 16u);
+    __builtin_amdgcn_raw_buffer_store_b128(v, r, lane * 16u, o, AUX);
+  }
+}
+template <uint32_t F, int AUX>
+__device__ __forceinline__ void side_in(const DevPtrs& p, const StepCfg& cfg, int64_t tile, char* buf, uint32_t lane) {
+  constexpr int S = kSideStride<F>;
+  const char* g = side_lo(p.side, S, tile);
+  char* l = buf + tile_image<F>(cfg).lo;
+  if (gaq::noise_mode<F>(cfg) != gaq::NOISE_OFF) dma_in_span<AUX>(g, l, lane, S);
+  else {
+    if constexpr (kSideLo<F> != 0) dma_in_span<AUX>(g, l, lane, kSideLo<F>);
+    dma_in_span<AUX>(g + (S - kSideCtrBytes), l + (S - kSideCtrBytes), lane, kSideCtrBytes);
+  }
+}
+template <uint32_t F, int AUX>
+__device__ __forceinline__ void side_out(const DevPtrs& p, const StepCfg& cfg, int64_t tile, const char* buf, uint32_t lane) {
+  constexpr int S = kSideStride<F>;
+  char* g = side_lo(p.side, S, tile);
+  const char* l = buf + tile_image<F>(cfg).lo;
+  if (gaq::noise_mode<F>(cfg) != gaq::NOISE_OFF) copy_out_span<AUX>(g, l, lane, S);
+  else {
+    if constexpr (kSideLo<F> != 0) copy_out_span<AUX>(g, l, lane, kSideLo<F>);
+    copy_out_span<AUX>(g + (S - kSideCtrBytes), l + (S - kSideCtrBytes), lane, kSideCtrBytes);
+  }
+}
+template <uint32_t F>
+__device__ __forceinline__ uint32_t read_ctr_word(const StepCfg& cfg, const char* buf, uint32_t lane) {
+  return reinterpret_cast<const uint32_t*>(buf + tile_image<F>(cfg).ctr)[lane];
+}
+template <uint32_t F>
+__device__ __forceinline__ void write_ctr_word(const StepCfg& cfg, char* buf, uint32_t lane, uint32_t w) {
+  reinterpret_cast<uint32_t*>(buf + tile_image<F>(cfg).ctr)[lane] = w;
 }
 
 template <uint32_t F>
@@ -216,19 +281,14 @@
     const int64_t first = tile * kTile;
     const uint32_t live = (uint32_t)((p.n - first) < kTile ? (p.n - first) : kTile);
     dma_in_rows<5, kLdAux<F>>(p.obs_in + first * 18, buf, lane, live * kRowBytes);
-    if constexpr ((F & gaq::F_FP32) == 0)
-      {
-        if constexpr (kLoMix<F>) dma_in_rows<3, kLdAux<F>>(reinterpret_cast<const uint32_t*>(p.lo) + first * kMixRowWords, buf + kRowsLds, lane, kMixRowsBytes);
-        else dma_in_rows<3, kLdAux<F>>(reinterpret_cast<const int16_t*>(p.lo) + first * 18, buf + kRowsLds, lane, kLoRowsBytes);
-      }
   } else {
     dma_in<9, kLdAux<F>>(p.core + tile * (kCorePlanes * kTile), buf, lane);
   }
+  side_in<F, kLdAux<F>>(p, cfg, tile, buf, lane);
   if (gaq::has_lag<F>(cfg)) {
     dma_in<2, kLdAux<F>>(p.lag + tile * (kLagPlanes * kTile), buf + im.lag, lane);
     dma_in<1, kLdAux<F>>(p.cmds + tile * (4 * kTile), buf + im.cmds, lane);
   }
-  if (gaq::noise_mode<F>(cfg) != gaq::NOISE_OFF) dma_in<1, kLdAux<F>>(p.ou + tile * (4 * kTile), buf + im.ou, lane);
   if (gaq::has_act_prev<F>(cfg)) dma_in<1, kLdAux<F>>(p.actp + tile * (4 * kTile), buf + im.actp, lane);
   if (gaq::has_env_goal<F>(cfg)) dma_in<1, kLdAux<F>>(p.goal + tile * (4 * kTile), buf + im.goal, lane);
   if (gaq::has_gyro_bias<F>(cfg)) dma_in<1, kLdAux<F>>(p.gyro + tile * (4 * kTile), buf + im.gyro, lane);
@@ -259,7 +319,7 @@
     }
     double v[18];
     if constexpr (kLoMix<F>) {
-      const uint32_t* q = reinterpret_cast<const uint32_t*>(buf + kRowsLds + lane * kMixRowBytes);
+      const uint32_t* q = reinterpret_cast<const uint32_t*>(buf + im.lo + lane * kMixRowBytes);
       float hv[18];
 #pragma unroll
       for (int k = 0; k < 9; ++k) { const float2 a = h[k]; hv[2 * k] = a.x; hv[2 * k + 1] = a.y; }
@@ -272,7 +332,7 @@
 #pragma unroll
       for (int j = 0; j < 3; ++j) v[15 + j] = split_decode32(hv[15 + j], q[8 + j]);
     } else {
-      const uint32_t* q = reinterpret_cast<const uint32_t*>(buf + kRowsLds + lane * kLoRowBytes);
+      const uint32_t* q = reinterpret_cast<const uint32_t*>(buf + im.lo + lane * kLoRowBytes);
 #pragma unroll
       for (int k = 0; k < 9; ++k) {
         const float2 a = h[k];
@@ -353,7 +413,7 @@
     float hv[18];
     heads18<gaq::kHeadsAreObs<F>>(v, hv);
     if constexpr (kLoMix<F>) {
-      uint32_t* q = reinterpret_cast<uint32_t*>(buf + kRowsLds + lane * kMixRowBytes);
+      uint32_t* q = reinterpret_cast<uint32_t*>(buf + im.lo + lane * kMixRowBytes);
 #pragma unroll
       for (int k = 0; k < 9; ++k) h[k] = make_float2(hv[2 * k], hv[2 * k + 1]);
 #pragma unroll
@@ -361,7 +421,7 @@
 #pragma unroll
       for (int j = 0; j < 3; ++j) q[8 + j] = split_lo32(v[15 + j]);
     } else {
-      uint32_t* q = reinterpret_cast<uint32_t*>(buf + kRowsLds + lane * kLoRowBytes);
+      uint32_t* q = reinterpret_cast<uint32_t*>(buf + im.lo + lane * kLoRowBytes);
 #pragma unroll
       for (int k = 0; k < 9; ++k) {
         h[k] = make_float2(hv[2 * k], hv[2 * k + 1]);
@@ -418,19 +478,14 @@
     copy_out_rows<5, kRowsBytes, kStAux<F>>(obs + first * 18, buf, lane, live * kRowBytes);
     if constexpr ((F & gaq::F_PACK) == 0)
       if (p.obs_copy) copy_out_rows<5, kRowsBytes, kCopyAux<F>>(p.obs_copy + first * 18, buf, lane, live * kRowBytes);
-    if constexpr ((F & gaq::F_FP32) == 0)
-      {
-        if constexpr (kLoMix<F>) copy_out_rows<3, kMixRowsBytes, kStAux<F>>(reinterpret_cast<uint32_t*>(p.lo) + first * kMixRowWords, buf + kRowsLds, lane, kMixRowsBytes);
-        else copy_out_rows<3, kLoRowsBytes, kStAux<F>>(reinterpret_cast<int16_t*>(p.lo) + first * 18, buf + kRowsLds, lane, kLoRowsBytes);
-      }
   } else {
     copy_out<9, kStAux<F>>(p.core + tile * (kCorePlanes * kTile), buf, lane);
   }
+  side_out<F, kStAux<F>>(p, cfg, tile, buf, lane);
   if (gaq::has_lag<F>(cfg)) {
     copy_out<2, kStAux<F>>(p.lag + tile * (kLagPlanes * kTile), buf + im.lag, lane);
     copy_out<1, kStAux<F>>(p.cmds + tile * (4 * kTile), buf + im.cmds, lane);
   }
-  if (gaq::noise_mode<F>(cfg) != gaq::NOISE_OFF) copy_out<1, kStAux<F>>(p.ou + tile * (4 * kTile), buf + im.ou, lane);
   if (gaq::has_act_prev<F>(cfg)) copy_out<1, kStAux<F>>(p.actp + tile * (4 * kTile), buf + im.actp, lane);
   if (gaq::has_env_goal<F>(cfg) && (cfg.resample_goal || cfg.excite))
     copy_out<1, kStAux<F>>(p.goal + tile * (4 * kTile), buf + im.goal, lane);
@@ -653,13 +708,10 @@
   const Model<T>* mp = &m;
   if constexpr (gaq::kModelMem<F>) mp = (const Model<T>*)kernarg_model_ptr();
   float4 a4;
-  uint32_t cw;
   {
     auto ra = __builtin_amdgcn_make_buffer_rsrc(const_cast<float*>(actions), 0, (int)(p.n * 16), 0x00020000);
     const u32x4 v = __builtin_amdgcn_raw_buffer_load_b128(ra, (uint32_t)i * 16u, 0, (F & gaq::F_NT) ? 2 : GAQ_ACT_AUX);
     a4 = __builtin_bit_cast(float4, v);
-    auto rc = __builtin_amdgcn_make_buffer_rsrc(p.ctr, 0, (int)(p.ntiles * kTile * 4), 0x00020000);
-    cw = __builtin_amdgcn_raw_buffer_load_b32(rc, (uint32_t)i * 4u, 0, (F & gaq::F_NT) ? 2 : GAQ_ACT_AUX);
   }
   if constexpr ((F & gaq::F_CTR) != 0) cfg.step_index = step_counter_checkin(p, step_counter_read(p, lane), lane);
   float pre0[4] = {0.0f, 0.0f, 0.0f, 0.0f}, pre1[4] = {0.0f, 0.0f, 0.0f, 0.0f};
@@ -673,6 +725,7 @@
   }
   wait_dma();
   EnvState<T> s;
+  const uint32_t cw = ablated(cfg, 8) ? 0u : read_ctr_word<F>(cfg, buf, lane);
   read_image<F>(cfg, buf, lane, s);
   s.tick = cw & 0xFFFFu;
   s.svd_ctr = cw >> 16;
@@ -754,15 +807,11 @@
     wave_lds_fence();
   }
   write_image<F>(cfg, buf, lane, s);
+  if (!ablated(cfg, 8)) write_ctr_word<F>(cfg, buf, lane, (s.tick & 0xFFFFu) | (s.svd_ctr << 16));
   wave_lds_fence();
   stage_out<F>(p, cfg, tile, buf, lane, obs);
-  {
-    auto rc = __builtin_amdgcn_make_buffer_rsrc(p.ctr, 0, (int)(p.ntiles * kTile * 4), 0x00020000);
-    __builtin_amdgcn_raw_buffer_store_b32((s.tick & 0xFFFFu) | (s.svd_ctr << 16), rc, (uint32_t)i * 4u, 0, kStAux<F>);
-  }
   if (live) {
-    reward[i] = out.reward;
-    done[i] = out.done;
+    if (!ablated(cfg, 16)) { reward[i] = out.reward; done[i] = out.done; }
     if (!isfinite(out.reward)) atomicAdd(p.nan_count, 1u);
   }
   if constexpr (!gaq::kHeadsAreObs<F> && !kObsRowsInLds) {
@@ -955,8 +1004,6 @@
   using RT = Real<F>;
   Model<RT> m;
   load_model<F, true>(p, cfg, tile, lane, um, m);
-  auto rc = __builtin_amdgcn_make_buffer_rsrc(p.ctr, 0, (int)(p.ntiles * kTile * 4), 0x00020000);
-  const uint32_t cw = __builtin_amdgcn_raw_buffer_load_b32(rc, (uint32_t)i * 4u, 0, 0);
   auto load_action = [&](int t) {
     auto ra = __builtin_amdgcn_make_buffer_rsrc(const_cast<float*>(actions + ((int64_t)t * p.n + first) * 4), 0,
                                                 (int)(nlive * 16u), 0x00020000);
@@ -966,6 +1013,7 @@
   wait_dma();
   EnvState<RT> s;
   read_image<F>(cfg, buf, lane, s);
+  const uint32_t cw = read_ctr_word<F>(cfg, buf, lane);
   s.tick = cw & 0xFFFFu;
   s.svd_ctr = cw >> 16;
   wave_lds_fence();
@@ -1014,18 +1062,14 @@
     c.step_index += 1;
   }
   write_image<F>(cfg, buf, lane, s);
+  write_ctr_word<F>(cfg, buf, lane, (s.tick & 0xFFFFu) | (s.svd_ctr << 16));
   wave_lds_fence();
   if (p.hi_final) copy_out_rows<5, kRowsBytes>(p.hi_final + first * 18, buf, lane, nlive * kRowBytes);
-  if constexpr ((F & gaq::F_FP32) == 0) {
-    if constexpr (kLoMix<F>) copy_out_rows<3, kMixRowsBytes>(reinterpret_cast<uint32_t*>(p.lo) + first * kMixRowWords, buf + im.lo, lane, kMixRowsBytes);
-    else copy_out_rows<3, kLoRowsBytes>(reinterpret_cast<int16_t*>(p.lo) + first * 18, buf + im.lo, lane, kLoRowsBytes);
-  }
+  side_out<F, GAQ_ST_AUX>(p, cfg, tile, buf, lane);
   if (gaq::has_lag<F>(cfg)) {
     copy_out<2>(p.lag + tile * (kLagPlanes * kTile), buf + im.lag, lane);
     copy_out<1>(p.cmds + tile * (4 * kTile), buf + im.cmds, lane);
   }
-  if (gaq::noise_mode<F>(cfg) != gaq::NOISE_OFF) copy_out<1>(p.ou + tile * (4 * kTile), buf + im.ou, lane);
-  __builtin_amdgcn_raw_buffer_store_b32((s.tick & 0xFFFFu) | (s.svd_ctr << 16), rc, (uint32_t)i * 4u, 0, 0);
 }
 
 template <uint32_t F>
@@ -1042,11 +1086,10 @@
   using RT = Real<F>;
   Model<RT> m;
   load_model<F, true>(p, cfg, tile, lane, um, m);
-  auto rc = __builtin_amdgcn_make_buffer_rsrc(p.ctr, 0, (int)(p.ntiles * kTile * 4), 0x00020000);
-  const uint32_t cw = __builtin_amdgcn_raw_buffer_load_b32(rc, (uint32_t)i * 4u, 0, 0);
   wait_dma();
   EnvState<RT> s;
   read_image<F>(cfg, buf, lane, s);
+  const uint32_t cw = read_ctr_word<F>(cfg, buf, lane);
   s.tick = cw & 0xFFFFu;
   s.svd_ctr = cw >> 16;
   wave_lds_fence();
@@ -1100,18 +1143,14 @@
     c.step_index += 1;
   }
   write_image<F>(cfg, buf, lane, s);
+  write_ctr_word<F>(cfg, buf, lane, (s.tick & 0xFFFFu) | (s.svd_ctr << 16));
   wave_lds_fence();
   if (p.hi_final) copy_out_rows<5, kRowsBytes>(p.hi_final + first * 18, buf, lane, nlive * kRowBytes);
-  if constexpr ((F & gaq::F_FP32) == 0) {
-    if constexpr (kLoMix<F>) copy_out_rows<3, kMixRowsBytes>(reinterpret_cast<uint32_t*>(p.lo) + first * kMixRowWords, buf + im.lo, lane, kMixRowsBytes);
-    else copy_out_rows<3, kLoRowsBytes>(reinterpret_cast<int16_t*>(p.lo) + first * 18, buf + im.lo, lane, kLoRowsBytes);
-  }
+  side_out<F, GAQ_ST_AUX>(p, cfg, tile, buf, lane);
   if (gaq::has_lag<F>(cfg)) {
     copy_out<2>(p.lag + tile * (kLagPlanes * kTile), buf + im.lag, lane);
     copy_out<1>(p.cmds + tile * (4 * kTile), buf + im.cmds, lane);
   }
-  if (gaq::noise_mode<F>(cfg) != gaq::NOISE_OFF) copy_out<1>(p.ou + tile * (4 * kTile), buf + im.ou, lane);
-  __builtin_amdgcn_raw_buffer_store_b32((s.tick & 0xFFFFu) | (s.svd_ctr << 16), rc, (uint32_t)i * 4u, 0, 0);
 }
 
 constexpr int kPolBlock = kTile;
```

New measurement: 21.43 billion (median of 4 runs). Within noise of the previous version (-0.1%).
